# facebookresearch/Active-3D-Vision-and-Touch

Hardware: AMD Instinct MI355X
Metric: mesh-recon iters/sec (fwd+bwd, 2562-vert GCN + 10k-pt Chamfer) at bs=64 (higher is better)
Workload: dtype f32; 1 GPU; icosphere-4 template (2562 verts, 5120 faces), 3-stage GCN 20x300 cut 0.33, bs=64/GPU, 10000-pt Chamfer x3 draws, Adam, ellipsoid clouds (BASELINE.json configs[1]); global_batch=64, parallelism=dp1

## Files before the change

active-3d-vision-and-touch_amd/csrc/capi.hip:

```cpp
#include <stdarg.h>
#include <stdlib.h>
#include <string.h>

#include "../../include/a3vt.h"
#include <atomic>
#include <initializer_list>
#include <mutex>
#include <unordered_map>

#include "kernels.h"
#include "prims.h"

namespace a3vt {

static thread_local char g_err[512] = "";

void set_error(const char *fmt, ...) {
  va_list ap;
  va_start(ap, fmt);
  vsnprintf(g_err, sizeof(g_err), fmt, ap);
  va_end(ap);
}

struct PtrArg {
  const char *name;
  const void *p;
  bool required;
  unsigned align;
  const char *why;
};
static int check_ptrs(const char *who, std::initializer_list<PtrArg> ptrs) {
  for (const PtrArg &a : ptrs) {
    if (a.required && !a.p) {
      set_error("%s: %s=NULL: %s", who, a.name, a.why);
      return -1;
    }
    if (!aligned_to(a.p, a.align)) {
      set_error("%s: %s=%p is not %u-byte aligned", who, a.name, a.p, a.align);
      return -1;
    }
  }
  return 0;
}
static int check_range(const char *who, const char *name, long long v, long long lo, long long hi) {
  if (v >= lo && v <= hi) return 0;
  set_error("%s: %s=%lld outside %lld..%lld", who, name, v, lo, hi);
  return -1;
}
static int check_count(const char *who, const char *name, int v, int max) {
  if (v >= 1 && v <= max) return 0;
  set_error("%s: %s=%d (1..%d) unsupported", who, name, v, max);
  return -1;
}
static int check_grads(const char *who, const PolicyGrads &g, int n_layers) {
  for (int l = 0; l < n_layers; ++l) {
    if (!g.dw[l] || !g.db[l] || !aligned_to(g.dw[l], 4) || !aligned_to(g.db[l], 4)) {
      set_error("%s: layer %d dweight / dbias null or misaligned", who, l);
      return -1;
    }
  }
  return 0;
}
template <int N>
struct LaunchCounts {
  std::atomic<long long> n[N];
  void add(int i, long long k) { n[i].fetch_add(k, std::memory_order_relaxed); }
  int read(long long *counts, int reset) {
    for (int i = 0; i < N; ++i) {
      if (counts) counts[i] = n[i].load(std::memory_order_relaxed);
      if (reset) n[i].store(0, std::memory_order_relaxed);
    }
    return N;
  }
};

__device__ float g_zero_page[64];
static const float *zero_page() {
  static const float *ptr[64] = {};
  static std::mutex mu;
  int dev = 0;
  (void)hipGetDevice(&dev);
  std::lock_guard<std::mutex> lock(mu);
  const float *&slot = ptr[dev & 63];
  if (!slot) {
    void *p = nullptr;
    if (hipGetSymbolAddress(&p, HIP_SYMBOL(g_zero_page)) != hipSuccess) return nullptr;
    slot = static_cast<const float *>(p);
  }
  return slot;
}

static inline size_t align_up(size_t x, size_t a) { return (x + a - 1) / a * a; }

struct Arena {
  size_t off = 0;
  size_t take(size_t nfloats) {
    const size_t o = off;
    off = align_up(off + nfloats, 64);
    return o;
  }
  size_t take16(size_t nelems) { return take((nelems + 1) / 2 + 64); }
};

enum { PROF_GEMM_FWD = 0, PROF_GEMM_DX = 1, PROF_DW = 2, PROF_AGG = 3, PROF_OUT = 4, PROF_SEARCH = 5, PROF_LOSS = 6, PROF_ENC = 7,
       PROF_OPT = 8, PROF_CLASSES = 9 };
struct Prof {
  bool on = false;
  static constexpr int kMax = 8192;
  hipEvent_t ev[kMax][2];
  int cls[kMax];
  int created = 0, used = 0;
};
static Prof g_prof;

struct ProfScope {
  int slot = -1;
  hipStream_t s;
  ProfScope(int cls, hipStream_t stream, bool timed = true) : s(stream) {
    if (!timed || !g_prof.on || g_prof.used >= Prof::kMax) return;
    slot = g_prof.used++;
    if (slot >= g_prof.created) {
      (void)hipEventCreate(&g_prof.ev[slot][0]);
      (void)hipEventCreate(&g_prof.ev[slot][1]);
      g_prof.created = slot + 1;
    }
    g_prof.cls[slot] = cls;
    (void)hipEventRecord(g_prof.ev[slot][0], s);
  }
  ~ProfScope() {
    if (slot >= 0) (void)hipEventRecord(g_prof.ev[slot][1], s);
  }
};

struct StackLayout {
  size_t wt, wt_stride;
  size_t za;
  int ldza;
  size_t z3;
  size_t ping[2];
  size_t panel;
  size_t dw_slab, db_slab, thin_dw_slab, thin_db_slab;
  size_t db_layer_stride;
  size_t heavy;
  size_t gq;
  size_t ell;
  size_t total;
};

constexpr int kQuadCols = 160;
static std::atomic<long long> g_path_counts[PATH_COUNT];
void path_count(int which) { g_path_counts[which].fetch_add(1, std::memory_order_relaxed); }
static int g_csr_algo = 0;
static SplitRef split_ref(const a3vt_adj_split *sp) {
  return sp ? SplitRef{sp->rowptr, sp->col, sp->scale, sp->cls} : SplitRef{nullptr, nullptr, nullptr, nullptr};
}
static bool split_whole(const a3vt_adj_split *sp) {
  const SplitRef r = split_ref(sp);
  return !sp || (r.rowptr && r.col && r.scale && r.cls);
}
static bool split_usable(const a3vt_adj_split *sp, int n_vert, int cut_len) {
  return sp && sp->max_degree > 0 && sp->max_degree <= csrqs_max_degree() && csrqs_fits(n_vert, cut_len);
}
static bool use_csrq(int batch, int n_vert, int hidden, int cut_len, int mode, int max_degree) {
  if (mode == GEMM_BF16_OPERANDS || mode == GEMM_BF16_STORAGE) return false;
  if (g_csr_algo != 2 && (max_degree <= 0 || max_degree > csrq_max_degree())) return false;
  if (g_csr_algo == 1 || cut_len <= 0) return false;
  return hidden % 4 == 0 && hidden >= kQuadCols + 16 && csrq_fits(n_vert, cut_len) && dw_quad_major_ok(hidden, kQuadCols / 4) &&
         rowgemm_quad_major_ok(batch * n_vert, hidden, pad4(cut_len));
}
static std::mutex g_stash_mu;
static std::unordered_map<const void *, int> g_stash_layout;
static void stash_layout_record(const void *masks, bool quad) {
  if (!masks) return;
  std::lock_guard<std::mutex> lock(g_stash_mu);
  if (g_stash_layout.size() > 4096) g_stash_layout.clear();
  g_stash_layout[masks] = quad ? 1 : 0;
}
static int stash_layout_lookup(const void *masks) {
  std::lock_guard<std::mutex> lock(g_stash_mu);
  auto it = g_stash_layout.find(masks);
  return it == g_stash_layout.end() ? -1 : it->second;
}
static int reduce_bias_partials(const float *slab, size_t layer_stride, int nslab, int cpad, int cut_len, int hidden, int last,
                                float *const *grad_biases, int acc, hipStream_t s) {
  for (int i0 = 0; i0 < last; i0 += kMaxImages) {
    SlabReduceBatch b{};
    b.count = last - i0 < kMaxImages ? last - i0 : kMaxImages;
    b.slab = slab + (size_t)i0 * layer_stride;
    for (int j = 0; j < b.count; ++j) b.out[j] = grad_biases[i0 + j];
    b.layer_stride = layer_stride;
    b.stride = cpad;
    b.n = cut_len;
    b.n_out = hidden;
    b.nslab = nslab;
    b.accumulate = acc;
    if (int rc = launch_slab_reduce_batch(b, s)) return rc;
  }
  return 0;
}

static inline int mask_ld(int hidden, int cut_len) { return pad4(cut_len) / 4 + (hidden + 3) / 4; }

static int hub_rows(const int32_t *rowptr, int n_vert, int max_degree, float *slot, int32_t **heavy, hipStream_t s) {
  *heavy = nullptr;
  if (max_degree > 0 && max_degree <= csr_heavy_degree()) return 0;
  *heavy = reinterpret_cast<int32_t *>(slot);
  return launch_csr_heavy_list(rowptr, n_vert, *heavy, s);
}

static int launch_stack_images(int kind, int transpose, const float *const *weights, int i0, int i1, int in_features,
                               int hidden, int w0, int wh, float *dst, size_t stride, hipStream_t s) {
  auto ld = [&](int w) { return kind == GEMM_BF16_STORAGE ? 2 * pad16(w / 2) : pad16(w); };
  for (; i0 < i1; i0 += kMaxImages) {
    WeightImages wi{};
    wi.count = i1 - i0 < kMaxImages ? i1 - i0 : kMaxImages;
    wi.dst = dst + stride * i0;
    wi.dst_stride = stride;
    wi.n = hidden;
    wi.transpose = transpose;
    int max_rows = 0, max_ld = kind == GEMM_FP32 && transpose ? ld(wh) : 0;
    for (int j = 0; j < wi.count; ++j) {
      const int w = i0 + j == 0 ? w0 : wh;
      wi.w[j] = weights[i0 + j];
      wi.k[j] = i0 + j == 0 ? in_features : hidden;
      wi.rows[j] = rowgemm_bt_rows(transpose ? hidden : w);
      wi.ld[j] = ld(transpose ? w : wh);
      max_rows = wi.rows[j] > max_rows ? wi.rows[j] : max_rows;
      max_ld = wi.ld[j] > max_ld ? wi.ld[j] : max_ld;
    }
    const int rc = kind == GEMM_FP32X3 ? launch_weight_images3(wi, s)
                   : kind == GEMM_BF16_STORAGE ? launch_weight_images16(wi, max_rows, max_ld, s)
                                               : launch_weight_images(wi, max_rows, max_ld, s);
    if (rc) return rc;
  }
  return 0;
}

static int reduce_output_grads(const float *dw_slab, const float *db_slab, int k, float *grad_w, float *grad_b, int acc,
                               hipStream_t s) {
  const size_t n = (size_t)k * 3;
  if (int rc = launch_slab_reduce_za(dw_slab, thin_num_slabs(), n, n, n, grad_w, acc, s)) return rc;
  return launch_slab_reduce_za(db_slab, thin_num_slabs(), 3, 3, 3, grad_b, acc, s);
}

struct StackPlan {
  bool x3;
  int omode;
  bool quad;
  bool qsplit;
  int qcols;
  int rm_ld;
  size_t rm_off;
};
static StackPlan stack_plan(int mode, int batch, int n_vert, int hidden, int num_layers, int cut_len, int max_degree,
                            const a3vt_adj_split *split, int rec) {
  StackPlan p{};
  const size_t m = (size_t)batch * n_vert;
  p.x3 = mode == GEMM_FP32X3 && num_layers > 2 && rowgemm3_stack_ok((long long)m, hidden, mask_ld(hidden, cut_len));
  p.omode = mode == GEMM_BF16_OPERANDS ? GEMM_BF16_OPERANDS : GEMM_FP32;
  const bool split_ok = split_usable(split, n_vert, cut_len);
  p.quad = num_layers > 1 &&
           (rec >= 0 ? rec == 1 : use_csrq(batch, n_vert, hidden, cut_len, mode, split_ok ? csrq_max_degree() : max_degree));
  p.qsplit = p.quad && split_ok;
  p.qcols = p.quad ? kQuadCols : 0;
  p.rm_ld = hidden - p.qcols;
  p.rm_off = m * p.qcols;
  return p;
}

static int launch_stack_ell(const StackPlan &p, const a3vt_adj_split *split, const int32_t *rowptr, const int32_t *col,
                            const float *val, int n_vert, int32_t *ell, hipStream_t s) {
  if (p.qsplit) {
    const SplitRef r = split_ref(split);
    return launch_csrqs_image(r.rowptr, r.col, r.scale, r.cls, n_vert, ell, s);
  }
  return p.quad ? launch_csrq_ell(rowptr, col, val, n_vert, ell, s) : 0;
}

static StackLayout stack_layout(int batch, int n_vert, int in_features, int hidden, int num_layers, int cut_len,
                                int need_backward, int gemm_mode = 0) {
  StackLayout L{};
  const size_t m = (size_t)batch * n_vert;
  const int cpad = pad4(cut_len);
  Arena a;
  const int kmax = hidden > pad4(in_features) ? hidden : pad4(in_features);
  L.wt_stride = align_up((size_t)rowgemm_bt_rows(kmax) * pad16(kmax), 64);
  if (gemm_mode == GEMM_FP32X3 && L.wt_stride < 3 * (size_t)kX3ImageFloats) L.wt_stride = 3 * (size_t)kX3ImageFloats;
  L.wt = a.take(L.wt_stride * (num_layers > 1 ? num_layers - 1 : 1));
  L.ldza = cpad > 4 ? cpad : 4;
  L.za = a.take(m * L.ldza);
  L.z3 = a.take(2 * m * 4);
  L.ping[0] = a.take(m * hidden);
  L.ping[1] = a.take(m * hidden);
  L.heavy = a.take(csr_heavy_scratch_ints(n_vert));
  L.ell = a.take(csrq_ell_ints(n_vert));
  if (need_backward) {
    const size_t kin = kmax;
    L.panel = a.take(pad4(in_features) > 304 ? m * 300 : 0);
    L.dw_slab = a.take((size_t)dw_slab_capacity(hidden) * kin * hidden);
    const size_t nslab = (size_t)csr_bwd_num_slabs(batch, n_vert) > (size_t)batch ? csr_bwd_num_slabs(batch, n_vert) : batch;
    L.db_layer_stride = align_up(nslab * cpad, 64);
    L.db_slab = a.take(L.db_layer_stride * (num_layers > 1 ? num_layers - 1 : 1));
    L.gq = a.take(m * L.ldza);
    L.thin_dw_slab = a.take((size_t)thin_num_slabs() * kin * 3);
    L.thin_db_slab = a.take((size_t)thin_num_slabs() * 3);
  }
  L.total = a.off;
  return L;
}

static int dw_panels(DwArgs d, const float *x, int ldx, int kin, float *panel, float *grad, int acc, bool timed, hipStream_t s) {
  const int cblk = kin > 304 ? 300 : kin;
  for (int c0 = 0; c0 < kin; c0 += cblk) {
    const int w = kin - c0 < cblk ? kin - c0 : cblk;
    d.x = x;
    d.ldx = ldx;
    if (kin > 304) {
      if (pad4(w) != w) { set_error("gcn_stack: in_features=%d needs a multiple of 4 past 300", kin); return -1; }
      if (int rc = launch_copy_cols(x, ldx, c0, w, panel, (long long)d.m, s)) return rc;
      d.x = panel;
      d.ldx = w;
    }
    d.k_in = w;
    {
      ProfScope ps(PROF_DW, s, timed);
      if (int rc = launch_dw(d, s)) return rc;
    }
    const size_t n = (size_t)w * d.n_out;
    if (int rc = launch_slab_reduce_za(d.slab, dw_images(d), n, n, n, grad + (size_t)c0 * d.n_out, acc, s)) return rc;
  }
  return 0;
}

static int check_stack_dims(int ld_feats, int in_features, int num_layers, int hidden, int cut_len) {
  if (num_layers < 1) { set_error("gcn_stack: num_layers=%d", num_layers); return -1; }
  if (ld_feats != pad4(in_features)) {
    set_error("gcn_stack: ld_feats=%d must be in_features=%d rounded up to a multiple of 4", ld_feats, in_features);
    return -1;
  }
  if (num_layers > 1 && (hidden % 4 != 0 || hidden > 304 || cut_len < 0 || cut_len > hidden)) {
    set_error("gcn_stack: hidden=%d (must be a multiple of 4, <= 304) cut_len=%d unsupported", hidden, cut_len);
    return -1;
  }
  if (ld_feats > 600) { set_error("gcn_stack: in_features=%d > 600 unsupported", in_features); return -1; }
  if (num_layers == 1 && ld_feats > 320) { set_error("gcn_stack: single-layer stack with %d inputs unsupported", in_features); return -1; }
  return 0;
}


static inline int mask_ld16(int hidden, int cut_len) { return (pad8(cut_len) / 4 + (hidden + 3) / 4 + 1) & ~1; }

constexpr int kStashInputLd = 608;

struct StackStash {
  size_t act_stride;
  size_t input16;
  int mld;
  size_t sign_stride;
  size_t signq0, signq_stride;
  size_t acts_bytes, mask_bytes;
  size_t act(int i) const { return (size_t)i * act_stride; }
  size_t signs(int i) const { return (size_t)i * sign_stride; }
  size_t signq(int i) const { return signq0 + (size_t)i * signq_stride; }
};
static StackStash stack_stash(int batch, int n_vert, int hidden, int num_layers, int cut_len, int gemm_mode) {
  StackStash S{};
  const bool s16 = gemm_mode == GEMM_BF16_STORAGE;
  const size_t m = (size_t)batch * n_vert, mpad = (m + 31) / 32 * 32, nh = num_layers > 1 ? num_layers - 1 : 0;
  S.act_stride = m * (s16 ? pad8(hidden) : hidden);
  S.input16 = nh * S.act_stride;
  S.mld = s16 ? mask_ld16(hidden, cut_len) : mask_ld(hidden, cut_len);
  S.sign_stride = mpad * S.mld;
  S.signq0 = nh * S.sign_stride;
  S.signq_stride = s16 ? 0 : align_up(m * (size_t)(pad4(cut_len) / 4), 256);
  S.acts_bytes = s16 ? (S.input16 + m * (size_t)kStashInputLd) * 2 + 256 : nh * S.act_stride * sizeof(float);
  S.mask_bytes = nh * (S.sign_stride + S.signq_stride);
  return S;
}
struct Stack16Layout {
  size_t wt, wt_stride;
  size_t feats16;
  size_t za;
  size_t z3;
  size_t ping[2];
  size_t dw_slab, db_slab, thin_dw_slab, thin_db_slab, heavy, total;
  size_t db_layer_stride;
  size_t tplan;
  int ld0, ldh, cpad;
  int ldza;
};

static Stack16Layout stack16_layout(int batch, int n_vert, int in_features, int hidden, int num_layers, int cut_len,
                                    int need_backward) {
  Stack16Layout L{};
  const size_t m = (size_t)batch * n_vert;
  L.ld0 = pad8(in_features);
  L.ldh = pad8(hidden);
  L.cpad = pad8(cut_len);
  L.ldza = L.cpad > 8 ? L.cpad : 8;
  Arena a;
  const int kmax = L.ld0 > L.ldh ? L.ld0 : L.ldh;
  const int rows_f = rowgemm_bt_rows(hidden), rows_b = rowgemm_bt_rows(kmax);
  const size_t img_f = (size_t)rows_f * pad16(kmax / 2), img_b = (size_t)rows_b * pad16(L.ldh / 2);
  L.wt_stride = align_up(img_f > img_b ? img_f : img_b, 64);
  L.wt = a.take(L.wt_stride * (num_layers > 1 ? num_layers - 1 : 1));
  L.feats16 = a.take16(m * L.ld0);
  L.za = a.take16(m * L.ldza);
  L.z3 = a.take(2 * m * 4);
  L.ping[0] = a.take16(m * L.ldh);
  L.ping[1] = a.take16(m * L.ldh);
  L.heavy = a.take(csr_heavy_scratch_ints(n_vert));
  L.tplan = a.take(csr16t_plan_ints(n_vert));
  if (need_backward) {
    const size_t kin = in_features > hidden ? in_features : hidden;
    L.dw_slab = a.take((size_t)dw16_num_slabs(hidden) * (kin > 304 ? 304 : kin) * hidden);
    L.db_layer_stride = align_up((size_t)csr_bwd_num_slabs(batch, n_vert) * L.ldza, 64);
    L.db_slab = a.take(L.db_layer_stride * (num_layers > 1 ? num_layers - 1 : 1));
    L.thin_dw_slab = a.take((size_t)thin_num_slabs() * hidden * 3);
    L.thin_db_slab = a.take((size_t)thin_num_slabs() * 3);
  }
  L.total = a.off;
  return L;
}

static int check_stack16_dims(int num_layers, int hidden, int in_features) {
  if (num_layers < 2) { set_error("gcn_stack: the bf16 storage mode needs at least one hidden layer"); return -1; }
  if (num_layers - 1 > kMaxImages) { set_error("gcn_stack: bf16 storage mode supports up to %d hidden layers", kMaxImages); return -1; }
  if (hidden > 304 || hidden % 4 != 0 || hidden < 16) { set_error("gcn_stack: bf16 storage mode: hidden=%d unsupported", hidden); return -1; }
  if (in_features > 600) { set_error("gcn_stack: in_features=%d > 600 unsupported", in_features); return -1; }
  if (in_features > 304 && in_features % 8 != 0) {
    set_error("gcn_stack: bf16 storage mode: in_features=%d > 304 must be a multiple of 8", in_features);
    return -1;
  }
  return 0;
}

static int stack_fwd16(const float *feats, int ld_feats, int in_features, const float *const *weights,
                       const float *const *biases, int num_layers, int hidden, int cut_len, const int32_t *rowptr,
                       const int32_t *col, const float *val, int max_degree, const a3vt_adj_split *split, int n_vert,
                       int batch, void *acts, uint8_t *masks, float *scratch, float *update, hipStream_t s) {
  if (int rc = check_stack16_dims(num_layers, hidden, in_features)) return rc;
  const float *zeros = zero_page();
  A3VT_CHECK_ARG(zeros != nullptr);
  const Stack16Layout L = stack16_layout(batch, n_vert, in_features, hidden, num_layers, cut_len, 0);
  const StackStash S = stack_stash(batch, n_vert, hidden, num_layers, cut_len, GEMM_BF16_STORAGE);
  const size_t m = (size_t)batch * n_vert;
  int32_t *heavy;
  if (int rc = hub_rows(rowptr, n_vert, max_degree, scratch + L.heavy, &heavy, s)) return rc;
  if (int rc = launch_stack_images(GEMM_BF16_STORAGE, 1, weights, 0, num_layers - 1, in_features, hidden, L.ld0, L.ldh,
                                   scratch + L.wt, L.wt_stride, s))
    return rc;
  u16 *f16 = acts ? static_cast<u16 *>(acts) + S.input16 : reinterpret_cast<u16 *>(scratch + L.feats16);
  if (int rc = launch_cvt_rows(feats, ld_feats, in_features, f16, L.ld0, (long long)m, s)) return rc;
  const bool tiled = heavy == nullptr && cut_len > 0 && g_csr_algo != 1 && csr16t_ok(n_vert, cut_len, max_degree, (long long)m);
  int32_t *tplan = reinterpret_cast<int32_t *>(scratch + L.tplan);
  if (tiled)
    if (int rc = launch_csr16t_build(rowptr, col, val, n_vert, tplan, s)) return rc;

  const u16 *x = f16;
  int ldx = L.ld0;
  u16 *za = reinterpret_cast<u16 *>(scratch + L.za);
  for (int i = 0; i + 1 < num_layers; ++i) {
    u16 *y = acts ? static_cast<u16 *>(acts) + S.act(i) : reinterpret_cast<u16 *>(scratch + L.ping[i & 1]);
    RowGemmArgs g{};
    g.a0 = g.a1 = reinterpret_cast<const float *>(x);
    g.lda0 = g.lda1 = ldx / 2;
    g.ksplit = g.k = ldx / 2;
    g.bt = scratch + L.wt + L.wt_stride * i;
    g.ldb = pad16(ldx / 2);
    g.zeros = zeros;
    g.m = (int)m;
    g.n_store = hidden;
    g.c = reinterpret_cast<float *>(y);
    g.ldc = L.ldh;
    g.c2 = reinterpret_cast<float *>(za);
    g.ldc2 = L.ldza;
    g.csplit = cut_len;
    uint8_t *mk = masks ? masks + S.signs(i) : nullptr;
    g.maskb = mk;
    g.mld = S.mld;
    g.moff = L.cpad / 4;
    g.mode = GEMM_BF16_STORAGE;
// ... 170 lines not shown
  return 0;
}

int a3vt_adj_split_validate(const int32_t *rowptr, const int32_t *col, const float *val, int n_vert,
                            const int32_t *p_rowptr, const int32_t *p_col, const float *scale, const uint8_t *cls) {
  A3VT_CHECK_ARG(rowptr && col && val && p_rowptr && p_col && scale && cls && n_vert > 0);
  if (p_rowptr[0] != 0 || p_rowptr[n_vert] > rowptr[n_vert]) {
    set_error("adj_split: p_rowptr[0]=%d p_rowptr[n]=%d (the matrix has %d entries)", p_rowptr[0], p_rowptr[n_vert], rowptr[n_vert]);
    return -1;
  }
  for (int i = 0; i < n_vert; ++i)
    if (p_rowptr[i + 1] < p_rowptr[i]) { set_error("adj_split: p_rowptr not monotone at %d", i); return -1; }
  int ns = 0, nc = 0;
  for (int i = 0; i < n_vert; ++i) {
    if (cls[i] > 2) { set_error("adj_split: cls[%d]=%d", i, (int)cls[i]); return -1; }
    ns += cls[i] == 1;
    nc += cls[i] == 2;
  }
  if ((ns == 0) != (nc == 0)) { set_error("adj_split: %d seam vertices but %d centres", ns, nc); return -1; }
  int32_t *members = static_cast<int32_t *>(malloc(sizeof(int32_t) * (size_t)(ns + nc + 1)));
  A3VT_CHECK_ARG(members != nullptr);
  int32_t *seam = members, *centre = members + ns;
  for (int i = 0, a = 0, b = 0; i < n_vert; ++i) {
    if (cls[i] == 1) seam[a++] = i;
    if (cls[i] == 2) centre[b++] = i;
  }
  int rc = 0;
  for (int i = 0; i < n_vert && rc == 0; ++i) {
    const int e0 = rowptr[i], e1 = rowptr[i + 1], p0 = p_rowptr[i], p1 = p_rowptr[i + 1];
    const int32_t *other = cls[i] == 1 ? centre : cls[i] == 2 ? seam : nullptr;
    const int no = cls[i] == 1 ? nc : cls[i] == 2 ? ns : 0;
    if (p1 < p0 || e1 - e0 != (p1 - p0) + no) {
      set_error("adj_split: row %d has %d entries, the split gives %d + %d", i, e1 - e0, p1 - p0, no);
      rc = -1;
      break;
    }
    int a = p0, b = 0;
    for (int e = e0; e < e1; ++e) {
      const bool has_a = a < p1, has_b = b < no;
      int next;
      if (has_a && has_b && p_col[a] == other[b]) {
        set_error("adj_split: row %d: column %d is in P and in the bipartite block", i, p_col[a]);
        rc = -1;
        break;
      }
      if (has_a && (!has_b || p_col[a] < other[b])) {
        next = p_col[a++];
        if (next < 0 || next >= n_vert || (a - 1 > p0 && p_col[a - 2] >= next)) {
          set_error("adj_split: row %d of P is not ascending / in range at column %d", i, next);
          rc = -1;
          break;
        }
        int lo = p_rowptr[next], hi = p_rowptr[next + 1] - 1;
        bool found = false;
        while (lo <= hi) {
          const int mid = (lo + hi) / 2;
          if (p_col[mid] == i) { found = true; break; }
          if (p_col[mid] < i) lo = mid + 1;
          else hi = mid - 1;
        }
        if (!found) { set_error("adj_split: P has (%d, %d) but not (%d, %d)", i, next, next, i); rc = -1; break; }
      } else {
        next = other[b++];
      }
      if (col[e] != next) {
        set_error("adj_split: row %d entry %d: column %d, the split gives %d", i, e - e0, col[e], next);
        rc = -1;
        break;
      }
      if (memcmp(&val[e], &scale[i], sizeof(float)) != 0) {
        set_error("adj_split: row %d entry %d: value %.9g != scale %.9g", i, e - e0, (double)val[e], (double)scale[i]);
        rc = -1;
        break;
      }
    }
  }
  free(members);
  return rc;
}

size_t a3vt_gcn_stack_mask_bytes(int batch, int n_vert, int hidden, int num_layers, int cut_len) {
  if (num_layers < 2 || batch <= 0 || n_vert <= 0 || hidden <= 0 || cut_len < 0) return 0;
  return stack_stash(batch, n_vert, hidden, num_layers, cut_len, GEMM_FP32).mask_bytes;
}

size_t a3vt_gcn_stack_scratch_bytes(int batch, int n_vert, int in_features, int hidden, int num_layers, int cut_len,
                                    int need_backward) {
  size_t most = 0;
  for (int mode = 0; mode <= 3; ++mode) {
    if (mode == GEMM_BF16_STORAGE && num_layers < 2) continue;
    const size_t b = a3vt_gcn_stack_scratch_bytes_mode(batch, n_vert, in_features, hidden, num_layers, cut_len, need_backward, mode);
    most = b > most ? b : most;
  }
  return most;
}

size_t a3vt_gcn_stack_scratch_bytes_mode(int batch, int n_vert, int in_features, int hidden, int num_layers,
                                         int cut_len, int need_backward, int gemm_bf16) {
  if (batch <= 0 || n_vert <= 0 || in_features <= 0 || hidden <= 0 || num_layers <= 0 || cut_len < 0 || gemm_bf16 < 0 || gemm_bf16 > 3)
    return 0;
  if (gemm_bf16 == GEMM_BF16_STORAGE)
    return stack16_layout(batch, n_vert, in_features, hidden, num_layers, cut_len, need_backward).total * sizeof(float);
  return stack_layout(batch, n_vert, in_features, hidden, num_layers, cut_len, need_backward, gemm_bf16).total * sizeof(float);
}

int a3vt_gcn_stack_stash_bytes(int batch, int n_vert, int hidden, int num_layers, int cut_len, int gemm_bf16,
                               size_t *acts_bytes, size_t *mask_bytes) {
  A3VT_CHECK_ARG(acts_bytes && mask_bytes && batch > 0 && n_vert > 0 && hidden > 0 && cut_len >= 0);
  *acts_bytes = *mask_bytes = 0;
  if (num_layers < 2) return 0;
  const StackStash S = stack_stash(batch, n_vert, hidden, num_layers, cut_len, gemm_bf16);
  *acts_bytes = S.acts_bytes;
  *mask_bytes = S.mask_bytes;
  return 0;
}

int a3vt_gcn_stack_fwd(const float *feats, int ld_feats, int in_features, const float *const *weights,
                       const float *const *biases, int num_layers, int hidden, int cut_len,
                       const int32_t *rowptr, const int32_t *col, const float *val, int max_degree, int n_vert,
                       int batch, int gemm_bf16, void *acts_v, uint8_t *masks, float *scratch, float *update,
                       void *stream) {
  return a3vt_gcn_stack_fwd_adj(feats, ld_feats, in_features, weights, biases, num_layers, hidden, cut_len, rowptr, col, val,
                                max_degree, nullptr, n_vert, batch, gemm_bf16, acts_v, masks, scratch, update, stream);
}

int a3vt_gcn_stack_fwd_adj(const float *feats, int ld_feats, int in_features, const float *const *weights,
                           const float *const *biases, int num_layers, int hidden, int cut_len,
                           const int32_t *rowptr, const int32_t *col, const float *val, int max_degree,
                           const a3vt_adj_split *split, int n_vert,
                           int batch, int gemm_bf16, void *acts_v, uint8_t *masks, float *scratch, float *update,
                           void *stream) {
  float *acts = static_cast<float *>(acts_v);
  A3VT_CHECK_ARG(feats && weights && biases && rowptr && col && val && scratch && update);
  A3VT_CHECK_ARG((acts == nullptr) == (masks == nullptr) || num_layers < 2);
  A3VT_CHECK_ARG(n_vert > 0 && batch > 0 && split_whole(split));
  A3VT_CHECK_ARG(gemm_bf16 >= GEMM_FP32 && gemm_bf16 <= GEMM_FP32X3);
  if (int rc = check_stack_dims(ld_feats, in_features, num_layers, hidden, cut_len)) return rc;
  hipStream_t s = static_cast<hipStream_t>(stream);
  if (gemm_bf16 == GEMM_BF16_STORAGE)
    return stack_fwd16(feats, ld_feats, in_features, weights, biases, num_layers, hidden, cut_len, rowptr, col, val,
                       max_degree, split, n_vert, batch, acts, masks, scratch, update, s);
  const float *zeros = zero_page();
  A3VT_CHECK_ARG(zeros != nullptr);
  const StackLayout L = stack_layout(batch, n_vert, in_features, hidden, num_layers, cut_len, 0, gemm_bf16);
  const StackStash S = stack_stash(batch, n_vert, hidden, num_layers, cut_len, gemm_bf16);
  const size_t m = (size_t)batch * n_vert;
  const int cpad = pad4(cut_len);

  int32_t *heavy;
  if (int rc = hub_rows(rowptr, n_vert, max_degree, scratch + L.heavy, &heavy, s)) return rc;
  const StackPlan P = stack_plan(gemm_bf16, batch, n_vert, hidden, num_layers, cut_len, max_degree, split, -1);
  const int qcols = P.qcols, rm_ld = P.rm_ld;
  const size_t rm_off = P.rm_off;
  if (P.x3)
    if (int rc = launch_stack_images(GEMM_FP32X3, 1, weights, 1, num_layers - 1, in_features, hidden, ld_feats, hidden,
                                     scratch + L.wt, L.wt_stride, s))
      return rc;
  if (int rc = launch_stack_images(GEMM_FP32, 1, weights, 0, P.x3 ? 1 : num_layers - 1, in_features, hidden, ld_feats, hidden,
                                   scratch + L.wt, L.wt_stride, s))
    return rc;
  if (num_layers > 1) path_count(P.quad ? PATH_STACK_QUAD : PATH_STACK_ROWS);
  if (P.qsplit) path_count(PATH_STACK_SPLIT);
  if (num_layers > 1) stash_layout_record(masks, P.quad);
  int32_t *ell = reinterpret_cast<int32_t *>(scratch + L.ell);
  if (int rc = launch_stack_ell(P, split, rowptr, col, val, n_vert, ell, s)) return rc;
  const float *x = feats, *xq = nullptr;
  int ldx = ld_feats;
  for (int i = 0; i + 1 < num_layers; ++i) {
    const int k = i == 0 ? ld_feats : hidden;
    const bool l3 = P.x3 && i > 0;
    float *y = acts ? acts + S.act(i) : scratch + L.ping[i & 1];
    RowGemmArgs g{};
    g.a0 = g.a1 = x;
    g.lda0 = g.lda1 = ldx;
    g.ksplit = k;
    if (xq) {
      g.a0 = xq;
      g.ksplit = qcols;
      g.a0q_nvert = n_vert;
      g.a0q_quads = qcols / 4;
    }
    g.bt = scratch + L.wt + L.wt_stride * i;
    g.ldb = pad16(k);
    g.zeros = zeros;
    g.m = (int)m;
    g.k = k;
    g.n_store = hidden;
    g.c = y + rm_off - qcols;
    g.ldc = rm_ld;
    g.c2 = scratch + L.za;
    g.ldc2 = cpad;
    g.csplit = cut_len;
    uint8_t *mk = masks ? masks + S.signs(i) : nullptr;
    g.maskb = mk;
    g.mld = S.mld;
    g.moff = cpad / 4;
    g.mode = l3 ? GEMM_FP32X3 : P.omode;
    if (P.quad) {
      g.zq_nvert = n_vert;
      g.zq_quads = cpad / 4;
      g.yq = y;
      g.yq_quads = qcols / 4;
      g.trash = scratch + L.z3;
    }
    {
      ProfScope ps(PROF_GEMM_FWD, s);
      if (int rc = launch_rowgemm(g, EPI_FWD_HIDDEN, s)) return rc;
    }
    if (P.quad) {
      uint8_t *sq = masks ? masks + S.signq(i) : nullptr;
      ProfScope psa(PROF_AGG, s);
      if (P.qsplit) {
        if (int rc = launch_csrqs_fwd(scratch + L.za, biases[i], cut_len, ell, n_vert, batch, y, qcols / 4, sq, 1, s)) return rc;
      } else if (int rc = launch_csrq_fwd(scratch + L.za, biases[i], cut_len, rowptr, col, val, heavy, ell, n_vert, batch, y, qcols / 4, sq, 1, s)) {
        return rc;
      }
      xq = y;
    } else if (cut_len > 0) {
      ProfScope psa(PROF_AGG, s);
      if (int rc = launch_csr_fwd(scratch + L.za, L.ldza, biases[i], cut_len, rowptr, col, val, heavy, n_vert, batch, y, hidden, mk, S.mld, 1, s))
        return rc;
    }
    x = y + rm_off - qcols;
    ldx = rm_ld;
  }
  const int klast = num_layers == 1 ? in_features : hidden;
  ProfScope pso(PROF_OUT, s);
  const SplitRef sref = split_ref(split);
  return launch_thin_fwd(x, ldx, klast, weights[num_layers - 1], biases[num_layers - 1], rowptr, col, val, heavy, n_vert,
                         batch, scratch + L.z3, update, xq, qcols / 4, s, split ? &sref : nullptr);
}

int a3vt_gcn_stack_bwd(const float *feats, int ld_feats, int in_features, const float *const *weights,
                       const float *const *biases, int num_layers, int hidden, int cut_len,
                       const int32_t *rowptr, const int32_t *col, const float *val, const int32_t *rowptrT,
                       const int32_t *colT, const float *valT, int max_degreeT, int n_vert, int batch, int gemm_bf16,
                       const void *acts_v,
                       const uint8_t *masks, const float *grad_update, float *const *grad_weights, float *const *grad_biases,
                       float *grad_feats, float *scratch, void *stream) {
  return a3vt_gcn_stack_bwd_adj(feats, ld_feats, in_features, weights, biases, num_layers, hidden, cut_len, rowptr, col, val,
                                rowptrT, colT, valT, max_degreeT, nullptr, n_vert, batch, gemm_bf16, acts_v, masks, grad_update,
                                grad_weights, grad_biases, grad_feats, scratch, 0, stream);
}

int a3vt_gcn_stack_bwd_acc(const float *feats, int ld_feats, int in_features, const float *const *weights,
                           const float *const *biases, int num_layers, int hidden, int cut_len,
                           const int32_t *rowptr, const int32_t *col, const float *val, const int32_t *rowptrT,
                           const int32_t *colT, const float *valT, int max_degreeT, int n_vert, int batch, int gemm_bf16,
                           const void *acts_v,
                           const uint8_t *masks, const float *grad_update, float *const *grad_weights,
                           float *const *grad_biases, float *grad_feats, float *scratch, int accumulate, void *stream) {
  return a3vt_gcn_stack_bwd_adj(feats, ld_feats, in_features, weights, biases, num_layers, hidden, cut_len, rowptr, col, val,
                                rowptrT, colT, valT, max_degreeT, nullptr, n_vert, batch, gemm_bf16, acts_v, masks, grad_update,
                                grad_weights, grad_biases, grad_feats, scratch, accumulate, stream);
}

int a3vt_gcn_stack_bwd_adj(const float *feats, int ld_feats, int in_features, const float *const *weights,
                           const float *const *biases, int num_layers, int hidden, int cut_len,
                           const int32_t *rowptr, const int32_t *col, const float *val, const int32_t *rowptrT,
                           const int32_t *colT, const float *valT, int max_degreeT, const a3vt_adj_split *split,
                           int n_vert, int batch, int gemm_bf16, const void *acts_v,
                           const uint8_t *masks, const float *grad_update, float *const *grad_weights,
                           float *const *grad_biases, float *grad_feats, float *scratch, int accumulate, void *stream) {
  const int acc = accumulate ? 1 : 0;
  const float *acts = static_cast<const float *>(acts_v);
  (void)biases; (void)rowptr; (void)col; (void)val;
  A3VT_CHECK_ARG(feats && weights && rowptrT && colT && valT && grad_update && grad_weights && grad_biases);
  A3VT_CHECK_ARG(grad_feats && scratch && n_vert > 0 && batch > 0 && split_whole(split));
  A3VT_CHECK_ARG(gemm_bf16 >= GEMM_FP32 && gemm_bf16 <= GEMM_FP32X3);
  A3VT_CHECK_ARG(num_layers == 1 || acts != nullptr);
  A3VT_CHECK_ARG(num_layers <= 2 || masks != nullptr);
  if (int rc = check_stack_dims(ld_feats, in_features, num_layers, hidden, cut_len)) return rc;
  hipStream_t s = static_cast<hipStream_t>(stream);
  if (gemm_bf16 == GEMM_BF16_STORAGE)
    return stack_bwd16(feats, ld_feats, in_features, weights, num_layers, hidden, cut_len, rowptrT, colT, valT,
                       max_degreeT, split, n_vert, batch, acts, masks, grad_update, grad_weights, grad_biases, grad_feats,
                       scratch, acc, s);
  const float *zeros = zero_page();
  A3VT_CHECK_ARG(zeros != nullptr);
  const StackLayout L = stack_layout(batch, n_vert, in_features, hidden, num_layers, cut_len, 1, gemm_bf16);
  const StackStash S = stack_stash(batch, n_vert, hidden, num_layers, cut_len, gemm_bf16);
  const size_t m = (size_t)batch * n_vert;
  const int cpad = pad4(cut_len);
  const int last = num_layers - 1;

  const SplitRef sref = split_ref(split);
  int32_t *heavyT;
  if (int rc = hub_rows(rowptrT, n_vert, max_degreeT, scratch + L.heavy, &heavyT, s)) return rc;
  const StackPlan P = stack_plan(gemm_bf16, batch, n_vert, hidden, num_layers, cut_len, max_degreeT, split,
                                 masks ? stash_layout_lookup(masks) : 0);
  const bool quad = P.quad;
  const int qcols = P.qcols, rm_ld = P.rm_ld;
  const size_t rm_off = P.rm_off;
  int32_t *ellT = reinterpret_cast<int32_t *>(scratch + L.ell);
  if (int rc = launch_stack_ell(P, split, rowptrT, colT, valT, n_vert, ellT, s)) return rc;
  {
    const float *xl = num_layers == 1 ? feats : acts + S.act(last - 1);
    const float *x = xl + rm_off - qcols;
    const int ldx = num_layers == 1 ? ld_feats : rm_ld;
    const int k = num_layers == 1 ? in_features : hidden;
    float *gprev = num_layers == 1 ? grad_feats : scratch + L.ping[0];
    const int ldg = num_layers == 1 ? ld_feats : hidden;
    ProfScope pso(PROF_OUT, s);
    if (int rc = launch_thin_bwd(x, ldx, k, weights[last], rowptrT, colT, valT, heavyT, n_vert, batch, grad_update,
                                 scratch + L.z3, num_layers > 1, gprev, ldg, ldg, scratch + L.thin_dw_slab,
                                 scratch + L.thin_db_slab, quad ? scratch + L.gq : nullptr, cpad / 4, quad ? xl : nullptr,
                                 qcols / 4, s, split ? &sref : nullptr))
      return rc;
    if (int rc = reduce_output_grads(scratch + L.thin_dw_slab, scratch + L.thin_db_slab, k, grad_weights[last], grad_biases[last],
                                     acc, s))
      return rc;
  }

  if (P.x3)
    if (int rc = launch_stack_images(GEMM_FP32X3, 0, weights, 1, last, in_features, hidden, ld_feats, hidden, scratch + L.wt,
                                     L.wt_stride, s))
      return rc;
  if (int rc = launch_stack_images(GEMM_FP32, 0, weights, 0, P.x3 ? 1 : last, in_features, hidden, ld_feats, hidden,
                                   scratch + L.wt, L.wt_stride, s))
    return rc;

  const int db_rows = quad ? batch : csr_bwd_num_slabs(batch, n_vert);
  int cur = 0;
  for (int i = last - 1; i >= 0; --i) {
    float *g = scratch + L.ping[cur];
    float *dza = scratch + L.za;
    const float *xl = i == 0 ? feats : acts + S.act(i - 1);
    const bool xhyb = quad && i > 0;
    const float *x = xhyb ? xl + rm_off - qcols : xl;
    const int ldx = i == 0 ? ld_feats : (xhyb ? rm_ld : hidden);
    const int kin = i == 0 ? in_features : hidden;

    if (cut_len > 0 && quad) {
      const uint8_t *sq = masks + S.signq(i);
      ProfScope psa(PROF_AGG, s);
      if (P.qsplit) {
        if (int rc = launch_csrqs_bwd(scratch + L.gq, cut_len, ellT, n_vert, batch, dza, sq,
                                      scratch + L.db_slab + (size_t)i * L.db_layer_stride, s))
          return rc;
      } else if (int rc = launch_csrq_bwd(scratch + L.gq, cut_len, rowptrT, colT, valT, heavyT, ellT, n_vert, batch, dza, sq,
                                          scratch + L.db_slab + (size_t)i * L.db_layer_stride, s)) {
        return rc;
      }
    } else if (cut_len > 0) {
      ProfScope psa(PROF_AGG, s);
      if (int rc = launch_csr_bwd(g, hidden, cut_len, rowptrT, colT, valT, heavyT, n_vert, batch, dza, L.ldza,
                                  scratch + L.db_slab + (size_t)i * L.db_layer_stride, s))
        return rc;
    } else if (!acc) {
      if (int rc = launch_fill_zero(grad_biases[i], hidden, s)) return rc;
    }

    DwArgs d{};
    if (xhyb) {
      d.ldx_src = rm_ld;
      d.xq = xl;
      d.xq_nvert = n_vert;
      d.xq_quads = qcols / 4;
    }
    if (quad) {
      d.z0q_nvert = n_vert;
      d.z0q_quads = cpad / 4;
    }
    d.z0 = dza;
    d.ldz0 = L.ldza;
    d.z1 = g;
    d.ldz1 = hidden;
    d.zsplit = cpad;
    d.zeros = zeros;
    d.slab = scratch + L.dw_slab;
    d.m = (int)m;
    d.n_out = hidden;
    d.mode = P.omode;
    const int ldxw = xhyb ? hidden : ldx;
    if (P.x3 && i > 0) {
      d.mode = GEMM_FP32X3;
      d.x = x;
      d.ldx = ldxw;
      d.k_in = kin;
      if (!dw3_ok(d)) d.mode = P.omode;
    }
    if (int rc = dw_panels(d, x, ldxw, kin, scratch + L.panel, grad_weights[i], acc, true, s)) return rc;

    RowGemmArgs r{};
    r.a0 = dza;
    r.lda0 = L.ldza;
    if (quad) {
      r.a0q_nvert = n_vert;
      r.a0q_quads = cpad / 4;
    }
    r.a1 = g;
    r.lda1 = hidden;
    r.ksplit = cpad;
    r.bt = scratch + L.wt + L.wt_stride * i;
    r.ldb = pad16(hidden);
    r.zeros = zeros;
    r.m = (int)m;
    r.k = hidden;
    r.n_store = i == 0 ? ld_feats : hidden;
    r.mode = P.x3 && i > 0 ? GEMM_FP32X3 : P.omode;
    if (i == 0) {
      r.c = grad_feats;
      r.ldc = ld_feats;
      if (int rc = launch_rowgemm(r, EPI_PLAIN, s)) return rc;
    } else {
      r.c = scratch + L.ping[cur ^ 1];
      r.ldc = hidden;
      r.maskb = const_cast<uint8_t *>(masks) + S.signs(i - 1);
      r.mld = S.mld;
      r.moff = cpad / 4;
      r.csplit = cut_len;
      if (quad) {
        r.c2 = scratch + L.gq;
        r.zq_nvert = n_vert;
        r.zq_quads = cpad / 4;
        r.trash = scratch + L.z3;
      }
      {
        ProfScope ps(PROF_GEMM_DX, s);
        if (int rc = launch_rowgemm(r, EPI_DX_MASK, s)) return rc;
      }
      cur ^= 1;
    }
  }
  if (cut_len > 0)
    if (int rc = reduce_bias_partials(scratch + L.db_slab, L.db_layer_stride, db_rows, cpad, cut_len, hidden, last, grad_biases, acc, s))
      return rc;
  return 0;
}

namespace {
struct LayerLayout {
  size_t wt, za, ga, dz, panel, dw_slab, db_slab, heavy, total;
  int ldza;
};
LayerLayout layer_layout(int batch, int n_vert, int ld_x, int n_out, int cut_len, int need_backward) {
  LayerLayout L{};
  const size_t m = (size_t)batch * n_vert;
  const int cpad = pad4(cut_len), npad = pad4(n_out);
  L.ldza = cpad > 4 ? cpad : 4;
  Arena a;
  const size_t wt_fwd = (size_t)rowgemm_bt_rows(n_out) * pad16(ld_x);
  const size_t wt_bwd = (size_t)rowgemm_bt_rows(ld_x) * pad16(npad);
  L.wt = a.take(wt_fwd > wt_bwd ? wt_fwd : wt_bwd);
  L.za = a.take(m * L.ldza);
  L.heavy = a.take(csr_heavy_scratch_ints(n_vert));
  if (need_backward) {
    L.ga = a.take(m * L.ldza);
    L.dz = a.take(m * npad);
    L.panel = a.take(ld_x > 304 ? m * 300 : 0);
    const int kin = ld_x > 304 ? 300 : ld_x;
    L.dw_slab = a.take((size_t)dw_num_slabs(n_out) * kin * n_out);
    L.db_slab = a.take((size_t)csr_bwd_num_slabs(batch, n_vert) * L.ldza);
  }
  L.total = a.off;
  return L;
}
int check_layer_dims(int ld_x, int in_features, int n_out, int cut_len) {
  if (ld_x % 4 != 0 || ld_x < in_features || ld_x > 600 || in_features < 1) {
    set_error("gcn_layer: ld_x=%d must be a multiple of 4, >= in_features=%d and <= 600", ld_x, in_features);
    return -1;
  }
  if (n_out < 1 || n_out > 304 || cut_len < 0 || cut_len > n_out) {
    set_error("gcn_layer: out_features=%d (1..304) cut_len=%d unsupported", n_out, cut_len);
    return -1;
  }
  if (in_features > 304 && in_features % 4 != 0) {
    set_error("gcn_layer: in_features=%d > 304 must be a multiple of 4", in_features);
    return -1;
  }
  return 0;
}
int layer_fwd_tail(const float *za, int ldza, const float *bias, int cut_len, int relu, const int32_t *rowptr, const int32_t *col,
                   const float *val, int max_degree, int n_vert, int batch, float *y, int ld_y, float *heavy_slot, hipStream_t s) {
  if (cut_len <= 0) return 0;
  int32_t *heavy;
  if (int rc = hub_rows(rowptr, n_vert, max_degree, heavy_slot, &heavy, s)) return rc;
  return launch_csr_fwd(za, ldza, bias, cut_len, rowptr, col, val, heavy, n_vert, batch, y, ld_y, nullptr, 0, relu, s);
}
int layer_bwd_tail(const float *grad_y, int ld_gy, const float *y, int ld_y, int relu, int n_out, int cut_len,
                   const int32_t *rowptrT, const int32_t *colT, const float *valT, int max_degreeT, int n_vert, int batch, float *ga,
                   float *dz, float *db_slab, float *heavy_slot, float *grad_bias, hipStream_t s) {
  const int cpad = pad4(cut_len), npad = pad4(n_out);
  if (int rc = launch_relu_split(grad_y, ld_gy, y, ld_y, relu, n_out, cpad, npad, (long long)batch * n_vert, ga, dz, s)) return rc;
  if (int rc = launch_fill_zero(grad_bias, n_out, s)) return rc;
  if (cut_len <= 0) return 0;
  int32_t *heavyT;
  if (int rc = hub_rows(rowptrT, n_vert, max_degreeT, heavy_slot, &heavyT, s)) return rc;
  if (int rc = launch_csr_bwd(ga, cpad, cut_len, rowptrT, colT, valT, heavyT, n_vert, batch, dz, npad, db_slab, s)) return rc;
  return launch_slab_reduce(db_slab, csr_bwd_num_slabs(batch, n_vert), cpad, cut_len, grad_bias, s);
}
}

size_t a3vt_gcn_layer_scratch_bytes(int batch, int n_vert, int ld_x, int out_features, int cut_len, int need_backward) {
  return layer_layout(batch, n_vert, ld_x, out_features, cut_len, need_backward).total * sizeof(float);
}

int a3vt_gcn_layer_fwd(const float *x, int ld_x, int in_features, const float *weight, const float *bias,
                       int out_features, int cut_len, int relu, const int32_t *rowptr, const int32_t *col,
                       const float *val, int max_degree, int n_vert, int batch, int gemm_bf16, float *y, int ld_y,
                       float *scratch, void *stream) {
  A3VT_CHECK_ARG(x && weight && bias && rowptr && col && val && y && scratch && n_vert > 0 && batch > 0);
  if (int rc = check_layer_dims(ld_x, in_features, out_features, cut_len)) return rc;
  A3VT_CHECK_ARG(ld_y % 4 == 0 && ld_y >= out_features);
  hipStream_t s = static_cast<hipStream_t>(stream);
  const float *zeros = zero_page();
  A3VT_CHECK_ARG(zeros != nullptr);
  const LayerLayout L = layer_layout(batch, n_vert, ld_x, out_features, cut_len, 0);
  const size_t m = (size_t)batch * n_vert;
  float *wt = scratch + L.wt;
  if (int rc = launch_transpose_pad(weight, in_features, out_features, wt, rowgemm_bt_rows(out_features), pad16(ld_x), s))
    return rc;
  RowGemmArgs g{};
  g.a0 = g.a1 = x;
  g.lda0 = g.lda1 = ld_x;
  g.ksplit = ld_x;
  g.bt = wt;
  g.ldb = pad16(ld_x);
  g.zeros = zeros;
  g.m = (int)m;
  g.k = ld_x;
  g.n_store = out_features;
  g.c = y;
  g.ldc = ld_y;
  g.c2 = scratch + L.za;
  g.ldc2 = L.ldza;
  g.csplit = cut_len;
  g.no_relu = relu ? 0 : 1;
  g.mode = gemm_bf16 == GEMM_BF16_OPERANDS ? GEMM_BF16_OPERANDS : GEMM_FP32;
  if (int rc = launch_rowgemm(g, EPI_FWD_HIDDEN, s)) return rc;
  return layer_fwd_tail(scratch + L.za, L.ldza, bias, cut_len, relu ? 1 : 0, rowptr, col, val, max_degree, n_vert, batch, y, ld_y,
                        scratch + L.heavy, s);
}

int a3vt_gcn_layer_bwd(const float *x, int ld_x, int in_features, const float *weight, int out_features, int cut_len,
                       int relu, const int32_t *rowptrT, const int32_t *colT, const float *valT, int max_degreeT,
                       int n_vert, int batch, int gemm_bf16, const float *y, int ld_y, const float *grad_y, int ld_gy,
                       float *grad_weight, float *grad_bias, float *grad_x, float *scratch, void *stream) {
  A3VT_CHECK_ARG(x && weight && rowptrT && colT && valT && grad_y && grad_weight && grad_bias && grad_x && scratch);
  A3VT_CHECK_ARG(n_vert > 0 && batch > 0 && ld_gy >= out_features && (!relu || (y && ld_y >= out_features)));
  if (int rc = check_layer_dims(ld_x, in_features, out_features, cut_len)) return rc;
  hipStream_t s = static_cast<hipStream_t>(stream);
  const float *zeros = zero_page();
  A3VT_CHECK_ARG(zeros != nullptr);
  const LayerLayout L = layer_layout(batch, n_vert, ld_x, out_features, cut_len, 1);
  const size_t m = (size_t)batch * n_vert;
  const int npad = pad4(out_features);
  float *dz = scratch + L.dz;
  if (int rc = layer_bwd_tail(grad_y, ld_gy, y, ld_y, relu ? 1 : 0, out_features, cut_len, rowptrT, colT, valT, max_degreeT, n_vert,
                              batch, scratch + L.ga, dz, scratch + L.db_slab, scratch + L.heavy, grad_bias, s))
    return rc;
  DwArgs d{};
  d.z0 = scratch + L.za;
  d.ldz0 = 4;
  d.z1 = dz;
  d.ldz1 = npad;
  d.zsplit = 0;
  d.zeros = zeros;
  d.slab = scratch + L.dw_slab;
  d.m = (int)m;
  d.n_out = out_features;
  d.mode = gemm_bf16 == GEMM_BF16_OPERANDS ? GEMM_BF16_OPERANDS : GEMM_FP32;
  if (int rc = dw_panels(d, x, ld_x, in_features, scratch + L.panel, grad_weight, 0, false, s)) return rc;
  float *wp = scratch + L.wt;
  if (int rc = launch_copy_pad(weight, in_features, out_features, wp, rowgemm_bt_rows(ld_x), pad16(npad), s)) return rc;
  RowGemmArgs r{};
  r.a0 = scratch + L.za;
  r.lda0 = 4;
  r.ksplit = 0;
  r.a1 = dz;
  r.lda1 = npad;
  r.bt = wp;
  r.ldb = pad16(npad);
  r.zeros = zeros;
  r.m = (int)m;
// ... 760 lines not shown
  for (int k = 0; k < n; ++k) {
    A3VT_CHECK_ARG(src[k] && dst[k] && outer[k] > 0 && inner[k] > 0 && hw[k] > 0);
    A3VT_CHECK_ARG(outer[k] <= (1ll << 31) / inner[k] / hw[k]);
    b.src[k] = src[k];
    b.dst[k] = static_cast<uint16_t *>(dst[k]);
    b.inner[k] = inner[k];
    b.hw[k] = hw[k];
    b.start[k + 1] = b.start[k] + outer[k] * inner[k] * hw[k];
  }
  ProfScope psc(PROF_ENC, static_cast<hipStream_t>(stream));
  return launch_cast_weights(b, static_cast<hipStream_t>(stream));
}

int a3vt_conv5_supported(int cin, int cout, int stride) { return conv5_shape_ok(cin, cout, stride) ? 1 : 0; }

size_t a3vt_conv5_image_bytes(int cout, int cin, int flip) {
  if (cin == 3 && flip) return cout == 16 ? conv5_weight_image_bytes(16, 16) : 0;
  if (cin == 3) return cout == 3 || cout == 16 ? conv5_weight_image_bytes(cout, 3) : 0;
  if ((cin != 16 && cin != 32) || (cout != 16 && cout != 32)) return 0;
  return flip ? conv5_weight_image_bytes(cin, cout) : conv5_weight_image_bytes(cout, cin);
}

int a3vt_conv5_weight_image(const float *weight, int cout, int cin, int flip, void *image, void *stream) {
  A3VT_CHECK_ARG(weight && image && (flip == 0 || flip == 1));
  A3VT_CHECK_ARG(((cin == 16 || cin == 32) && (cout == 16 || cout == 32)) || (cin == 3 && flip == 0 && (cout == 3 || cout == 16)) ||
                 (cin == 3 && flip == 1 && cout == 16));
  A3VT_CHECK_ARG(aligned_to(image, 16));
  return launch_conv5_weight_image(weight, flip, cout, cin, image, static_cast<hipStream_t>(stream));
}

int a3vt_conv5_nhwc(const void *x, int batch, int height, int width, int cin, int cout, int stride, int pad, const void *image,
                    const float *bias, void *y, void *stream) {
  A3VT_CHECK_ARG(x && image && y);
  A3VT_CHECK_ARG(conv5_shape_ok(cin, cout, stride));
  A3VT_CHECK_ARG(batch > 0 && height > 0 && width > 0 && pad >= 0 && pad <= 4);
  A3VT_CHECK_ARG(height + 2 * pad >= 5 && width + 2 * pad >= 5);
  A3VT_CHECK_ARG((long long)batch * height * width <= (1ll << 31) / 32);
  A3VT_CHECK_ARG(aligned_to(x, cin == 3 ? 2 : 16) && aligned_to(y, cin == 3 ? 2 : 16));
  A3VT_CHECK_ARG(aligned_to(image, 16) && (cout == 3 || aligned_to(y, 16)));
  A3VT_CHECK_ARG(aligned_to(bias, cout == 3 ? 4 : 16));
  ProfScope psc(PROF_ENC, static_cast<hipStream_t>(stream));
  return launch_conv5(x, batch, height, width, cin, cout, stride, pad, image, bias, y, static_cast<hipStream_t>(stream));
}

int a3vt_conv5_input_grad_3x16s2(const void *grad_out, int batch, int out_height, int out_width, const void *image, void *grad_in,
                                 void *stream) {
  A3VT_CHECK_ARG(grad_out && image && grad_in && batch > 0 && out_height > 0 && out_width > 0);
  A3VT_CHECK_ARG((long long)batch * (2 * out_height + 2) * (2 * out_width + 2) <= (1ll << 31) / 16);
  A3VT_CHECK_ARG(aligned_to(grad_out, 16) && aligned_to(image, 16));
  A3VT_CHECK_ARG(aligned_to(grad_in, 2));
  ProfScope psc(PROF_ENC, static_cast<hipStream_t>(stream));
  return launch_conv5_up3(grad_out, batch, out_height, out_width, image, grad_in, static_cast<hipStream_t>(stream));
}

size_t a3vt_conv5_wrw_scratch_bytes(int cin, int cout) {
  return ((cin == 16 || cin == 32) && (cout == 16 || cout == 32)) || (cin == 3 && (cout == 3 || cout == 16)) ? conv5_wrw_scratch_bytes(cin, cout) : 0;
}

int a3vt_conv5_weight_grad(const void *x, const void *grad_out, int batch, int height, int width, int cin, int cout, int stride,
                           float *grad_weight, void *scratch, size_t scratch_bytes, void *stream) {
  A3VT_CHECK_ARG(x && grad_out && grad_weight && scratch);
  A3VT_CHECK_ARG(conv5_shape_ok(cin, cout, stride));
  A3VT_CHECK_ARG(batch > 0 && height >= 3 && width >= 3 && (long long)batch * height * width <= (1ll << 31) / 32);
  A3VT_CHECK_ARG(aligned_to(scratch, 16));
  A3VT_CHECK_ARG(aligned_to(x, cin == 3 ? 2 : 16) && aligned_to(grad_out, cout == 3 ? 2 : 16));
  A3VT_CHECK_ARG(scratch_bytes >= conv5_wrw_scratch_bytes(cin, cout));
  ProfScope psc(PROF_ENC, static_cast<hipStream_t>(stream));
  return launch_conv5_wrw(x, grad_out, batch, height, width, cin, cout, stride, grad_weight, scratch, static_cast<hipStream_t>(stream));
}

int a3vt_conv5f_supported(int cin, int cout, int stride) { return conv5f_shape_ok(cin, cout, stride) ? 1 : 0; }

size_t a3vt_conv5f_image_bytes(int cin, int cout) { return conv5f_weight_image_bytes(cin, cout); }

int a3vt_conv5f_weight_image(const float *weight, int cout, int cin, void *image, void *stream) {
  A3VT_CHECK_ARG(weight && image);
  A3VT_CHECK_ARG(conv5f_weight_image_bytes(cin, cout) != 0);
  A3VT_CHECK_ARG(aligned_to(weight, 4) && aligned_to(image, 16));
  return launch_conv5f_weight_image(weight, cout, cin, image, static_cast<hipStream_t>(stream));
}

int a3vt_conv5f_nhwc(const float *x, int batch, int height, int width, int cin, int cout, int stride, int pad, const void *image,
                     const float *scale, const float *shift, int relu, float *y, void *stream) {
  A3VT_CHECK_ARG(x && image && y);
  A3VT_CHECK_ARG(conv5f_shape_ok(cin, cout, stride));
  A3VT_CHECK_ARG(batch >= 1 && height >= 1 && width >= 1 && pad >= 0 && pad <= 4 && (relu == 0 || relu == 1));
  A3VT_CHECK_ARG(height + 2 * pad >= 5 && width + 2 * pad >= 5);
  A3VT_CHECK_ARG((long long)batch * height * width <= (1ll << 31) / 32);
  A3VT_CHECK_ARG(aligned_to(x, cin == 3 ? 4 : 16));
  A3VT_CHECK_ARG(aligned_to(y, 16) && aligned_to(image, 16));
  A3VT_CHECK_ARG(aligned_to(scale, 4) && aligned_to(shift, 4));
  ProfScope psc(PROF_ENC, static_cast<hipStream_t>(stream));
  return launch_conv5f(x, batch, height, width, cin, cout, stride, pad, image, scale, shift, relu, y, static_cast<hipStream_t>(stream));
}

int a3vt_adam_chunk_elems(void) { return adam_chunk_elems(); }

int a3vt_adam_step(void *const *param, const void *const *grad, void *const *exp_avg, void *const *exp_avg_sq,
                   const long long *numel, const int *chunk_tensor, const long long *chunk_off, int n_chunks, double lr, double beta1,
                   double beta2, double eps, double weight_decay, long long step, void *stream) {
  A3VT_CHECK_ARG(n_chunks >= 0 && step >= 1);
  A3VT_CHECK_ARG(n_chunks == 0 || (param && grad && exp_avg && exp_avg_sq && numel && chunk_tensor && chunk_off));
  A3VT_CHECK_ARG(lr >= 0.0 && beta1 >= 0.0 && beta1 < 1.0 && beta2 >= 0.0 && beta2 < 1.0 && eps >= 0.0 && weight_decay >= 0.0);
  ProfScope psc(PROF_OPT, static_cast<hipStream_t>(stream));
  return launch_adam(param, grad, exp_avg, exp_avg_sq, numel, chunk_tensor, chunk_off, n_chunks, lr, beta1, beta2, eps, weight_decay, step,
                     static_cast<hipStream_t>(stream));
}

int a3vt_adam_step_clamp(void *const *param, void *const *grad, void *const *exp_avg, void *const *exp_avg_sq, const long long *numel,
                         const int *chunk_tensor, const long long *chunk_off, int n_chunks, double lr, double beta1, double beta2,
                         double eps, double weight_decay, long long step, double grad_clamp, void *stream) {
  A3VT_CHECK_ARG(n_chunks >= 0 && step >= 1 && grad_clamp > 0.0);
  A3VT_CHECK_ARG(n_chunks == 0 || (param && grad && exp_avg && exp_avg_sq && numel && chunk_tensor && chunk_off));
  A3VT_CHECK_ARG(lr >= 0.0 && beta1 >= 0.0 && beta1 < 1.0 && beta2 >= 0.0 && beta2 < 1.0 && eps >= 0.0 && weight_decay >= 0.0);
  ProfScope psc(PROF_OPT, static_cast<hipStream_t>(stream));
  return launch_adam(param, const_cast<const void *const *>(grad), exp_avg, exp_avg_sq, numel, chunk_tensor, chunk_off, n_chunks, lr, beta1,
                     beta2, eps, weight_decay, step, static_cast<hipStream_t>(stream), grad_clamp);
}

int a3vt_profile_enable(int on) {
  g_prof.on = on != 0;
  g_prof.used = 0;
  return 0;
}

int a3vt_profile_read_classes(double *total_ms, int *count, int n) {
  A3VT_CHECK_ARG(total_ms && count && n >= 0);
  for (int c = 0; c < n; ++c) { total_ms[c] = 0.0; count[c] = 0; }
  for (int i = 0; i < g_prof.used; ++i) {
    if (hipEventSynchronize(g_prof.ev[i][1]) != hipSuccess) { set_error("profile_read: event sync failed"); return -2; }
    float ms = 0.f;
    if (hipEventElapsedTime(&ms, g_prof.ev[i][0], g_prof.ev[i][1]) != hipSuccess) continue;
    if (g_prof.cls[i] >= n) continue;
    total_ms[g_prof.cls[i]] += ms;
    count[g_prof.cls[i]] += 1;
  }
  g_prof.used = 0;
  return PROF_CLASSES;
}

int a3vt_profile_read(double *total_ms, int *count) {
  const int rc = a3vt_profile_read_classes(total_ms, count, 3);
  return rc < 0 ? rc : 0;
}

int a3vt_dbg_path_counts(long long *counts, int n, int reset) {
  A3VT_CHECK_ARG(n >= 0 && (counts != nullptr || n == 0));
  for (int i = 0; i < n; ++i) counts[i] = i < PATH_COUNT ? g_path_counts[i].load(std::memory_order_relaxed) : 0;
  if (reset)
    for (auto &c : g_path_counts) c.store(0, std::memory_order_relaxed);
  return PATH_COUNT;
}

int a3vt_dbg_csr_algo(int algo) {
  A3VT_CHECK_ARG(algo >= 0 && algo <= 2);
  g_csr_algo = algo;
  return 0;
}

int a3vt_split3_bf16(const float *x, size_t n, uint16_t *hi, uint16_t *mid, uint16_t *lo, void *stream) {
  A3VT_CHECK_ARG(n == 0 || (x && hi && mid && lo));
  return launch_split3(x, n, hi, mid, lo, static_cast<hipStream_t>(stream));
}

int a3vt_check_finite(const float *data, size_t n, int32_t *flag, void *stream) {
  A3VT_CHECK_ARG(data && flag);
  return launch_check_finite(data, n, flag, static_cast<hipStream_t>(stream));
}

}
```

active-3d-vision-and-touch_amd/csrc/gcn_dww.hip:

```cpp
#include <type_traits>

#include "gemm_tile.h"

namespace a3vt {

constexpr int kDK = 300, kDN = 300, kDXQ = 40, kDZQ = 25, kDXRW = 140, kDLdz = 300;
constexpr int kDStageRows = 16;
constexpr int kDwwGroupsA = 135, kDwwGroupsB = 121;
constexpr int kDXQ_off = 0, kDXR_off = 2560, kDZ_off = 2560 + 2304;
constexpr int kDZRa_off = kDZ_off + 1792;
constexpr int kDStage = kDZ_off + 2816;
constexpr int kDStages = 4;
constexpr int kDLdsFloats = kDStages * kDStage;

__device__ __forceinline__ void d_mfma(f32x4 &acc, float a, float b) {
  asm volatile("v_mfma_f32_16x16x4_f32 %0, %1, %2, %0" : "+a"(acc) : "v"(a), "v"(b));
}
__device__ __forceinline__ void d_lds(float &dst, unsigned base, int imm) {
  asm volatile("ds_read_b32 %0, %1 offset:%2" : "=v"(dst) : "v"(base), "n"(imm));
}
template <int N, int NX, int NZ>
__device__ __forceinline__ void d_wait(float (&x)[NX], float (&z)[NZ]) {
  static_assert(NX <= 5 && NZ <= 10, "operand list");
  if constexpr (NX == 5 && NZ == 10)
// ... 19 lines not shown
  const int nvert = p.xq_nvert;
  const unsigned lds0 = (unsigned)(size_t)(__attribute__((address_space(3))) float *)lds;

  const unsigned xq_lane = kDXQ_off * 4 + (unsigned)((l16 >> 2) * 256 + q * 16 + (l16 & 3) * 4);
  const unsigned xr_lane = kDXR_off * 4 + (unsigned)((q * kDXRW + l16) * 4);
  const unsigned zq_lane = kDZ_off * 4 + (unsigned)((l16 >> 2) * 256 + q * 16 + (l16 & 3) * 4);
  const unsigned zra_lane = kDZRa_off * 4 + (unsigned)((q * 60 + l16) * 4);
  const unsigned zrb_lane = kDZ_off * 4 + (unsigned)((q * kDXRW + l16) * 4);
  const bool t6q = l16 < 4;
  const unsigned z6_lane = t6q ? kDZ_off * 4 + (unsigned)(24 * 256 + q * 16 + l16 * 4) : kDZRa_off * 4 + (unsigned)((q * 60 + l16 - 4) * 4);
  const unsigned z6_step = t6q ? 64u : 960u;

  unsigned xr_off[9], zr_off[9];
  int d_bq = 0, d_vq = 0;
  unsigned xq_off = 0, zq_off = 0;
  auto locate = [&](int tile) {
    const int row = tile * kDStageRows + l16;
    d_bq = row / nvert;
    d_vq = row - d_bq * nvert;
  };
  auto refresh = [&]() {
    xq_off = ((unsigned)(d_bq * kDXQ + q) * (unsigned)nvert + (unsigned)d_vq) * 16u;
    zq_off = ((unsigned)(d_bq * kDZQ + q) * (unsigned)nvert + (unsigned)d_vq) * 16u;
  };
  auto advance = [&]() {
    d_vq += kDStageRows;
    const bool wrap = d_vq >= nvert;
    d_vq = wrap ? d_vq - nvert : d_vq;
    d_bq = wrap ? d_bq + 1 : d_bq;
  };
  if (SERVICE) {
#pragma unroll
    for (int j = 0; j < 9; ++j) {
      const int i = 64 * j + lane;
      const int rx = i / 35, px = i - rx * 35;
      xr_off[j] = i < 16 * 35 ? (unsigned)((rx * p.ldx_src + px * 4) * 4) : 0u;
      if (HALF == 0) {
        const int rz = i / 15, pz = i - rz * 15;
        zr_off[j] = (j < 4 && i < 16 * 15) ? (unsigned)((rz * kDLdz + pz * 4) * 4) : 0u;
      } else {
        zr_off[j] = i < 16 * 35 ? (unsigned)((rx * kDLdz + px * 4) * 4) : 0u;
      }
    }
  }
  constexpr int NDMA = HALF == 0 ? 10 + 9 + 7 + 4 : 10 + 9 + 9;
  auto dma = [&](int idx, int tile, int st) {
    float *sbase = lds + st * kDStage;
    const size_t row0 = (size_t)tile * kDStageRows;
    if (idx < 10) {
      glds16(reinterpret_cast<const float *>(w_at(p.xq + (size_t)idx * 4 * nvert * 4, xq_off)), sbase + kDXQ_off + idx * 256);
    } else if (idx < 19) {
      const int j = idx - 10;
      glds16(reinterpret_cast<const float *>(w_at(p.x + row0 * p.ldx_src + 160, xr_off[j])), sbase + kDXR_off + j * 256);
    } else if (HALF == 0 && idx < 26) {
      const int j = idx - 19;
      const unsigned off = j < 6 ? zq_off : zq_off - (unsigned)q * (unsigned)nvert * 16u;
      glds16(reinterpret_cast<const float *>(w_at(p.z0 + (size_t)(j < 6 ? j * 4 : 24) * nvert * 4, off)), sbase + kDZ_off + j * 256);
    } else if (HALF == 0) {
      const int j = idx - 26;
      glds16(reinterpret_cast<const float *>(w_at(p.z1 + row0 * kDLdz + 100, zr_off[j])), sbase + kDZRa_off + j * 256);
    } else {
      const int j = idx - 19;
      glds16(reinterpret_cast<const float *>(w_at(p.z1 + row0 * kDLdz + 160, zr_off[j])), sbase + kDZ_off + j * 256);
    }
  };

  if (SERVICE) {
#pragma unroll
    for (int d = 0; d < 3; ++d) {
      const int tsrc = tile0 + d < tile1 ? tile0 + d : tile1 - 1;
      locate(tsrc);
      refresh();
#pragma unroll
      for (int idx = 0; idx < NDMA; ++idx) dma(idx, tsrc, d);
    }
    locate(tile0 + 2 < tile1 ? tile0 + 2 : tile1 - 1);
    refresh();
  }
  wait_vmcnt<0>();
  wait_lgkm0();
  __builtin_amdgcn_s_barrier();

  f32x4 acc[NKT][NNT];
#pragma unroll
  for (int t = 0; t < NKT; ++t)
#pragma unroll
    for (int n = 0; n < NNT; ++n) acc[t][n] = f32x4{0.f, 0.f, 0.f, 0.f};
  int st = 0;
  auto frag = [&](int stg, auto sc, auto kc, float (&xf)[NKT], float (&zf)[NNT]) {
    constexpr int s = decltype(sc)::value, k = decltype(kc)::value;
    const unsigned sb = lds0 + (unsigned)(stg * kDStage * 4);
    if constexpr (k < NKT) {
      const unsigned xb = sb + (XROW ? xr_lane : xq_lane);
      if (XROW) d_lds(xf[k], xb, (kt0x + k) * 64 + s * 4 * kDXRW * 4);
      else d_lds(xf[k], xb, (kt0x + k) * 1024 + s * 64);
    } else if constexpr (k < NKT + NNT) {
      constexpr int n = k - NKT, T = NT0 + n;
      if (HALF == 0 && T < 6) d_lds(zf[n], sb + zq_lane, T * 1024 + s * 64);
      else if (HALF == 0 && T == 6) d_lds(zf[n], sb + z6_lane + (unsigned)s * z6_step, 0);
      else if (HALF == 0) d_lds(zf[n], sb + zra_lane, (T * 16 - 100) * 4 + s * 4 * 60 * 4);
      else d_lds(zf[n], sb + zrb_lane, (T * 16 - 160) * 4 + s * 4 * kDXRW * 4);
    }
  };
  auto dma_part = [&](int part, int dtile, int dst) {
    constexpr int PER = (NDMA + 3) / 4;
#pragma unroll
    for (int u = 0; u < PER; ++u)
      if (part * PER + u < NDMA) dma(part * PER + u, dtile < tile1 ? dtile : tile1 - 1, dst);
  };
  float xc[NKT], zc[NNT];
  [&]<int... K>(std::integer_sequence<int, K...>) {
    (frag(0, std::integral_constant<int, 0>{}, std::integral_constant<int, K>{}, xc, zc), ...);
  }(std::make_integer_sequence<int, NKT + NNT>{});
  d_wait<0>(xc, zc);
  for (int tile = tile0; tile < tile1; ++tile) {
    auto step = [&](auto sc) {
      constexpr int s = decltype(sc)::value;
      float xn[NKT], zn[NNT];
      constexpr int EVERY = (NKT * NNT) / (NKT + NNT);
      [&]<int... I>(std::integer_sequence<int, I...>) {
        ((d_mfma(acc[I / NNT][I % NNT], zc[I % NNT], xc[I / NNT]),
          (I % EVERY == 0 ? frag(s < 3 ? st : ((st + 1) & 3), std::integral_constant<int, (s + 1) & 3>{}, std::integral_constant<int, I / EVERY>{}, xn, zn)
                          : (void)0)),
         ...);
      }(std::make_integer_sequence<int, NKT * NNT>{});
      d_wait<0>(xn, zn);
#pragma unroll
      for (int t = 0; t < NKT; ++t) xc[t] = xn[t];
#pragma unroll
      for (int n = 0; n < NNT; ++n) zc[n] = zn[n];
    };
    step(std::integral_constant<int, 0>{});
    if (SERVICE && tile > tile0) dma_part(1, tile + 2, (st + 2) & 3);
    step(std::integral_constant<int, 1>{});
    if (SERVICE && tile > tile0) dma_part(2, tile + 2, (st + 2) & 3);
    step(std::integral_constant<int, 2>{});
    if (SERVICE) {
      if (tile > tile0) dma_part(3, tile + 2, (st + 2) & 3);
      wait_vmcnt<NDMA>();
    }
    wait_lgkm0();
    __builtin_amdgcn_s_barrier();
    step(std::integral_constant<int, 3>{});
    if (SERVICE) {
      if (tile + 3 < tile1) {
        advance();
        refresh();
      }
      dma_part(0, tile + 3, (st + 3) & 3);
    }
    st = (st + 1) & 3;
  }
  asm volatile("s_nop 15\n\ts_nop 3" ::: "memory");
  float *img = p.slab + (size_t)image * kDK * kDN;
#pragma unroll
  for (int t = 0; t < NKT; ++t) {
    const int k = (kt0 + t) * 16 + l16;
#pragma unroll
    for (int n = 0; n < NNT; ++n) {
      const int col = (NT0 + n) * 16 + q * 4;
      if (k < kDK && col < kDN) *reinterpret_cast<f32x4 *>(img + (size_t)k * kDN + col) = acc[t][n];
    }
  }
}

__global__ __launch_bounds__(256) __attribute__((amdgpu_waves_per_eu(1, 1))) void dww_kernel(DwArgs p) {
  extern __shared__ __attribute__((aligned(16))) float lds[];
  const int lane = threadIdx.x & 63;
  const int wave = __builtin_amdgcn_readfirstlane(threadIdx.x >> 6);
  const int half = blockIdx.x < kDwwGroupsA ? 0 : 1;
  const int group = half == 0 ? blockIdx.x : blockIdx.x - kDwwGroupsA, ngroups = half == 0 ? kDwwGroupsA : kDwwGroupsB;
  const int tiles = p.m / kDStageRows;
  const int t0 = (int)((long long)group * tiles / ngroups), t1 = (int)((long long)(group + 1) * tiles / ngroups);
  if (half == 1 && group < kDwwGroupsA - kDwwGroupsB) {
    float *img = p.slab + (size_t)(kDwwGroupsB + group) * kDK * kDN;
    for (int i = threadIdx.x; i < kDK * 35; i += 256) {
      const int k = i / 35, c = i - k * 35;
      *reinterpret_cast<f32x4 *>(img + (size_t)k * kDN + 160 + c * 4) = f32x4{0.f, 0.f, 0.f, 0.f};
    }
  }
  if (half == 0) {
    if (wave == 0) dww_wave<0, false, 5, false, 0>(p, lds, lane, t0, t1, group);
    else if (wave == 1) dww_wave<0, false, 5, false, 5>(p, lds, lane, t0, t1, group);
    else if (wave == 2) dww_wave<0, true, 5, false, 10>(p, lds, lane, t0, t1, group);
    else dww_wave<0, true, 4, true, 15>(p, lds, lane, t0, t1, group);
  } else {
    if (wave == 0) dww_wave<1, false, 5, false, 0>(p, lds, lane, t0, t1, group);
    else if (wave == 1) dww_wave<1, false, 5, false, 5>(p, lds, lane, t0, t1, group);
    else if (wave == 2) dww_wave<1, true, 5, false, 10>(p, lds, lane, t0, t1, group);
    else dww_wave<1, true, 4, true, 15>(p, lds, lane, t0, t1, group);
  }
}

bool dww_ok(const DwArgs &a) {
  if (a.mode != GEMM_FP32 || a.xq_nvert <= 0 || a.z0q_nvert != a.xq_nvert || a.xq == nullptr) return false;
  if (a.k_in != kDK || a.n_out != kDN || a.xq_quads != kDXQ || a.z0q_quads != kDZQ || a.zsplit != 4 * kDZQ) return false;
  if (a.ldx_src != kDXRW || a.ldz1 != kDLdz || a.m % a.xq_nvert != 0 || a.m % kDStageRows != 0 || a.xq_nvert < 16) return false;
  if (a.m > 3000000) return false;
  return a.m / kDStageRows >= kDwwGroupsA * 5;
}

int dww_images() { return kDwwGroupsA; }

int launch_dww(const DwArgs &a, hipStream_t s) {
  if (!dww_ok(a)) {
    set_error("dww: shape not taken (m=%d k_in=%d n_out=%d)", a.m, a.k_in, a.n_out);
    return -1;
  }
  static OncePerDevice once;
  once.run([] {
    (void)hipFuncSetAttribute((const void *)dww_kernel, hipFuncAttributeMaxDynamicSharedMemorySize, (int)(kDLdsFloats * sizeof(float)));
  });
  path_count(PATH_DWW);
  A3VT_LAUNCH(dww_kernel, dim3(kDwwGroupsA + kDwwGroupsB), dim3(256), kDLdsFloats * sizeof(float), s, a);
  A3VT_CHECK_LAUNCH();
  return 0;
}

}
```

active-3d-vision-and-touch_amd/csrc/gcn_gemm.hip:

```cpp
#include <type_traits>

#include "common.h"
#include "kernels.h"
#include "gemm_tile.h"

namespace a3vt {

template <int V>
using RgIdx = std::integral_constant<int, V>;

template <int NT, int EPI, int NSTAGE, int WAVES, int MODE, bool ADIRECT = false>
__global__ __launch_bounds__(64 * WAVES, 2) void rowgemm_kernel(RowGemmArgs p) {
  constexpr bool BF16 = MODE == 1;
  constexpr bool ST16 = MODE == 2;
  constexpr int MT = 2;
  constexpr int BROWS = ((NT * 16 + 16 * WAVES - 1) / (16 * WAVES)) * (16 * WAVES);
  constexpr int A_INSTR = MT;
  constexpr int B_INSTR = BROWS / (16 * WAVES);
  constexpr int A_FLOATS = WAVES * MT * 16 * 16;
  constexpr int STAGE = A_FLOATS + BROWS * 16;
  constexpr int PER = A_INSTR + B_INSTR;
  constexpr int DIST = NSTAGE - 1;
  constexpr int MSLOT = 1024;
  static_assert((DIST - 1) * PER <= 63, "vmcnt immediate");
// ... 401 lines not shown
              const int ur = i * 16 + rl;
              const unsigned ba = mslot[ur * p.mld + (col >> 2)];
              const unsigned bb = mslot[ur * p.mld + p.moff + (col >> 2)];
              float *dst = p.c + (size_t)row * p.ldc + col;
#pragma unroll
              for (int t = 0; t < 4; ++t) {
                const unsigned bit = ((col + t < p.csplit ? ba : bb) >> t) & 1u;
                v[t] = bit ? v[t] : 0.f;
              }
              if (full) {
                *reinterpret_cast<f32x4 *>(dst) = v;
              } else {
                for (int t = 0; t < 4; ++t)
                  if (col + t < p.n_store) dst[t] = v[t];
              }
            }
          }
        }
      }
      if (mask_rows) {
        wait_lgkm0();
        __builtin_amdgcn_wave_barrier();
        const int nbytes = 16 * nm * p.mld;
        uint8_t *dstm = p.maskb + (size_t)row0 * p.mld;
        for (int o = le * 16; o < nbytes; o += 1024)
          *reinterpret_cast<f32x4 *>(dstm + o) = *reinterpret_cast<const f32x4 *>(mslot + o);
      }
    }
    wait_lgkm0();
    __builtin_amdgcn_s_barrier();
  }
  if (p.rem_rows > 0) {
    const int ntl = min(NT, (p.n_store - col0 + 15) >> 4);
    const int units = ((p.rem_rows + 15) >> 4) * ntl;
    for (int u = wave * gridDim.x + blockIdx.x; u < units; u += WAVES * gridDim.x)
      rowtile_unit<EPI, MODE>(p, p.rem_row0, p.rem_row0 + p.rem_rows, u / ntl, col0 + (u % ntl) * 16, lane);
  }
}

template <int NT>
struct RowGemmCfg {
  static constexpr int WAVES = 8;
  static constexpr int NSTAGE = NT == 1 ? 5 : 3;
  static constexpr int WG_PER_CU = 1;
  static constexpr int BROWS = ((NT * 16 + 16 * WAVES - 1) / (16 * WAVES)) * (16 * WAVES);
};

template <int NT, int EPI>
static int launch_rowgemm_nt(const RowGemmArgs &a, int grid_y, hipStream_t s) {
  using C = RowGemmCfg<NT>;
  constexpr size_t shmem = (C::NSTAGE * (size_t)(C::WAVES * 2 * 256 + C::BROWS * 16) +
                            (EPI != EPI_PLAIN ? C::WAVES * 1024 : 0)) * sizeof(float);
  static_assert(shmem * C::WG_PER_CU <= 160 * 1024, "LDS budget");
  static OncePerDevice once;
  once.run([] {
    (void)hipFuncSetAttribute((const void *)rowgemm_kernel<NT, EPI, C::NSTAGE, C::WAVES, 0>,
                              hipFuncAttributeMaxDynamicSharedMemorySize, (int)shmem);
    (void)hipFuncSetAttribute((const void *)rowgemm_kernel<NT, EPI, C::NSTAGE, C::WAVES, 1>,
                              hipFuncAttributeMaxDynamicSharedMemorySize, (int)shmem);
    (void)hipFuncSetAttribute((const void *)rowgemm_kernel<NT, EPI, C::NSTAGE, C::WAVES, 2>,
                              hipFuncAttributeMaxDynamicSharedMemorySize, (int)shmem);
    if (NT == 19)
      (void)hipFuncSetAttribute((const void *)rowgemm_kernel<NT, EPI, C::NSTAGE, C::WAVES, 0, NT == 19>,
                                hipFuncAttributeMaxDynamicSharedMemorySize, (int)shmem);
  });
  const int tiles = cdiv(a.m, 16);
  const int max_wg = 256 * C::WG_PER_CU;
  const int grid = cdiv(tiles, C::WAVES) < max_wg ? cdiv(tiles, C::WAVES) : max_wg;
  if (a.mode == GEMM_BF16_STORAGE)
    A3VT_LAUNCH((rowgemm_kernel<NT, EPI, C::NSTAGE, C::WAVES, 2>), dim3(grid, grid_y), dim3(64 * C::WAVES), shmem, s, a);
  else if (a.mode == GEMM_BF16_OPERANDS)
    A3VT_LAUNCH((rowgemm_kernel<NT, EPI, C::NSTAGE, C::WAVES, 1>), dim3(grid, grid_y), dim3(64 * C::WAVES), shmem, s, a);
  else {
    if (NT == 19) path_count(PATH_RG_ADIRECT);
    if (NT == 19)
      A3VT_LAUNCH((rowgemm_kernel<NT, EPI, C::NSTAGE, C::WAVES, 0, NT == 19>), dim3(grid, grid_y), dim3(64 * C::WAVES), shmem, s, a);
    else
      A3VT_LAUNCH((rowgemm_kernel<NT, EPI, C::NSTAGE, C::WAVES, 0>), dim3(grid, grid_y), dim3(64 * C::WAVES), shmem, s, a);
  }
  A3VT_CHECK_LAUNCH();
  return 0;
}

template <int EPI>
static int launch_rowgemm_cols(const RowGemmArgs &a, hipStream_t s) {
  const int nt = cdiv(a.n_store, 16);
  const int row_wgs = cdiv(cdiv(a.m, 16), 8);
  if (row_wgs < 96 && nt > 4) {
    if (row_wgs * cdiv(nt, 4) >= 96) return launch_rowgemm_nt<4, EPI>(a, cdiv(nt, 4), s);
    return launch_rowgemm_nt<1, EPI>(a, nt, s);
  }
  if (nt <= 1) return launch_rowgemm_nt<1, EPI>(a, 1, s);
  if (nt <= 4) return launch_rowgemm_nt<4, EPI>(a, 1, s);
  if (nt <= 8) return launch_rowgemm_nt<8, EPI>(a, 1, s);
  if (nt <= 13) return launch_rowgemm_nt<13, EPI>(a, 1, s);
  return launch_rowgemm_nt<19, EPI>(a, cdiv(nt, 19), s);
}

static int rowgemm_main_rows(int m, int nt) {
  const int tiles = cdiv(m, 16), full = tiles / 2048 * 2048, rem = tiles - full;
  return full == 0 || rem == 0 || rem * nt > 1024 || nt < 2 ? m : full * 16;
}
template <int EPI>
static int launch_rowgemm_epi(const RowGemmArgs &a0, hipStream_t s) {
  RowGemmArgs a = a0;
  a.bt_rows = rowgemm_bt_rows(a.n_store);
  a.col0 = 0;
  const int main_m = rowgemm_main_rows(a.m, cdiv(a.n_store, 16));
  if (main_m == a.m) return launch_rowgemm_cols<EPI>(a, s);
  RowGemmArgs m = a;
  m.m = main_m;
  m.rem_row0 = main_m;
  m.rem_rows = a.m - main_m;
  return launch_rowgemm_cols<EPI>(m, s);
}

int rowgemm_bt_rows(int n_store) {
  const int nt = cdiv(n_store, 16);
  if (nt > 19) return ((n_store + 127) / 128) * 128;
  const int tnt = nt <= 1 ? 1 : nt <= 4 ? 4 : nt <= 8 ? 8 : nt <= 13 ? 13 : 19;
  return ((tnt * 16 + 127) / 128) * 128;
}

bool rowgemm_quad_major_ok(int m, int n_store, int cpad) {
  const int nt = cdiv(n_store, 16);
  if (nt < 14 || nt > 19 || cpad <= 0 || cpad > 160 || cpad % 4 != 0) return false;
  return cdiv(cdiv(rowgemm_main_rows(m, nt), 16), 8) >= 96;
}

int launch_rowgemm(const RowGemmArgs &a, int epi, hipStream_t s) {
  if (a.mode == GEMM_FP32X3) return launch_rowgemm3(a, epi, s);
  if (a.a0q_nvert > 0 && (a.mode == GEMM_BF16_STORAGE || a.m % a.a0q_nvert != 0 || a.ksplit != a.a0q_quads * 4)) {
    set_error("rowgemm: quad-major a0 needs ksplit = 4 * quads (ksplit=%d quads=%d) and whole meshes (m=%d)", a.ksplit, a.a0q_quads, a.m);
    return -1;
  }
  if (a.yq_quads > 0 && (a.zq_nvert <= 0 || a.yq == nullptr || epi != EPI_FWD_HIDDEN || a.yq_quads < a.zq_quads || a.yq_quads * 4 > 160 ||
                         a.yq_quads * 4 > a.n_store)) {
    set_error("rowgemm: quad-major activations need the quad-major forward epilogue and at most 160 columns (yq_quads=%d)", a.yq_quads);
    return -1;
  }
  if (a.zq_nvert > 0 && (epi == EPI_PLAIN || a.mode == GEMM_BF16_STORAGE || a.c2 == nullptr || a.m % a.zq_nvert != 0 ||
                         a.zq_quads * 4 != pad4(a.csplit) || !rowgemm_quad_major_ok(a.m, a.n_store, a.zq_quads * 4))) {
    set_error("rowgemm: quad-major output unsupported for m=%d n=%d csplit=%d epi=%d mode=%d", a.m, a.n_store, a.csplit, epi, a.mode);
    return -1;
  }
  if (epi == EPI_DX_MASK && (a.maskb == nullptr || 32 * a.mld > 4096)) {
    set_error("rowgemm: EPI_DX_MASK needs sign bytes with 32*mld <= 4096 (mld=%d)", a.mld);
    return -1;
  }
  if (a.k % 4 != 0 || a.ksplit % 4 != 0 || a.ldb < pad16(a.k)) {
    set_error("rowgemm: k=%d ksplit=%d ldb=%d violate alignment rules", a.k, a.ksplit, a.ldb);
    return -1;
  }
  if (rowgemmw_ok(a, epi)) return launch_rowgemmw(a, epi, s);
  if (rowgemm16_ok(a, epi)) return launch_rowgemm16(a, epi, s);
  switch (epi) {
    case EPI_PLAIN: return launch_rowgemm_epi<EPI_PLAIN>(a, s);
    case EPI_FWD_HIDDEN: return launch_rowgemm_epi<EPI_FWD_HIDDEN>(a, s);
    case EPI_DX_MASK: return launch_rowgemm_epi<EPI_DX_MASK>(a, s);
  }
  set_error("rowgemm: bad epilogue %d", epi);
  return -1;
}

__global__ void transpose_pad_kernel(const float *__restrict__ w, int k, int n, float *__restrict__ wt,
                                     int rows, int ld) {
  __shared__ float tile[32][33];
  const int bx = blockIdx.x * 32, by = blockIdx.y * 32;
  for (int i = threadIdx.y; i < 32; i += 8) {
    const int kk = bx + i, nn = by + threadIdx.x;
    tile[i][threadIdx.x] = (kk < k && nn < n) ? w[(size_t)kk * n + nn] : 0.f;
  }
  __syncthreads();
  for (int i = threadIdx.y; i < 32; i += 8) {
    const int nn = by + i, kk = bx + threadIdx.x;
    if (nn < rows && kk < ld) wt[(size_t)nn * ld + kk] = tile[threadIdx.x][i];
  }
}

int launch_transpose_pad(const float *w, int k, int n, float *wt, int rows, int ld, hipStream_t s) {
  dim3 grid(cdiv(ld, 32), cdiv(rows, 32));
  A3VT_LAUNCH(transpose_pad_kernel, grid, dim3(32, 8), 0, s, w, k, n, wt, rows, ld);
  A3VT_CHECK_LAUNCH();
  return 0;
}

__global__ void weight_images_kernel(WeightImages w) {
  const int l = blockIdx.z;
  const float *src = w.w[l];
  float *dst = w.dst + (size_t)l * w.dst_stride;
  const int k = w.k[l], n = w.n, rows = w.rows[l], ld = w.ld[l];
  if (w.transpose) {
    __shared__ float tile[32][33];
    const int bx = blockIdx.x * 32, by = blockIdx.y * 32;
    if (bx >= ld || by >= rows) return;
    for (int i = threadIdx.y; i < 32; i += 8) {
      const int kk = bx + i, nn = by + threadIdx.x;
      tile[i][threadIdx.x] = (kk < k && nn < n) ? src[(size_t)kk * n + nn] : 0.f;
    }
    __syncthreads();
    for (int i = threadIdx.y; i < 32; i += 8) {
      const int nn = by + i, kk = bx + threadIdx.x;
      if (nn < rows && kk < ld) dst[(size_t)nn * ld + kk] = tile[threadIdx.x][i];
    }
  } else {
    const int tid = threadIdx.y * 32 + threadIdx.x;
    const int nblk = gridDim.x * gridDim.y, blk = blockIdx.y * gridDim.x + blockIdx.x;
    for (int idx = blk * 256 + tid; idx < rows * ld; idx += nblk * 256) {
      const int r = idx / ld, c = idx % ld;
      dst[idx] = (r < k && c < n) ? src[(size_t)r * n + c] : 0.f;
    }
  }
}

int launch_weight_images(const WeightImages &w, int max_rows, int max_ld, hipStream_t s) {
  A3VT_LAUNCH(weight_images_kernel, dim3(cdiv(max_ld, 32), cdiv(max_rows, 32), w.count), dim3(32, 8), 0, s, w);
  A3VT_CHECK_LAUNCH();
  return 0;
}

__global__ void copy_pad_kernel(const float *__restrict__ w, int rows_in, int cols_in, float *__restrict__ out,
                                int rows, int ld) {
  const int idx = blockIdx.x * blockDim.x + threadIdx.x;
  if (idx >= rows * ld) return;
  const int r = idx / ld, c = idx % ld;
  out[idx] = (r < rows_in && c < cols_in) ? w[(size_t)r * cols_in + c] : 0.f;
}

int launch_copy_pad(const float *w, int rows_in, int cols_in, float *out, int rows, int ld, hipStream_t s) {
  A3VT_LAUNCH(copy_pad_kernel, dim3(cdiv((long long)rows * ld, 256)), dim3(256), 0, s, w, rows_in, cols_in, out,
                     rows, ld);
  A3VT_CHECK_LAUNCH();
  return 0;
}

__global__ void copy_cols_kernel(const float *__restrict__ src, int ld_src, int c0, int w, float *__restrict__ dst,
                                 long long m) {
  const long long i = (long long)blockIdx.x * blockDim.x + threadIdx.x;
  const int w4 = w >> 2;
  if (i >= m * w4) return;
  const long long r = i / w4;
  const int c = (int)(i - r * w4) * 4;
  *reinterpret_cast<f32x4 *>(dst + r * w + c) = *reinterpret_cast<const f32x4 *>(src + r * ld_src + c0 + c);
}

int launch_copy_cols(const float *src, int ld_src, int c0, int w, float *dst, long long m, hipStream_t s) {
  A3VT_LAUNCH(copy_cols_kernel, dim3(cdiv(m * (w >> 2), 256)), dim3(256), 0, s, src, ld_src, c0, w, dst, m);
  A3VT_CHECK_LAUNCH();
  return 0;
}

constexpr int DW_MAXI = 5;
constexpr int DW_MAXO = 3;

template <int NI, int NO>
__device__ __forceinline__ void dw_stage(const float *__restrict__ sb, int ldx, int ldz0, int ldz1, int offG,
                                         int xoff, const int (&zoff)[DW_MAXO], int q, int ni, int no, bool z0q, int rot,
                                         f32x4 (&acc)[DW_MAXI][DW_MAXO]) {
#pragma unroll 1
  for (int ks = 0; ks < 4; ++ks) {
    const int r = q * 4 + ks;
    const float *xr = sb + r * ldx + xoff;
    const int ra = z0q ? ((r + rot) & 15) * 4 : r * ldz0, rg = r * ldz1;
    float a[DW_MAXI], b[DW_MAXO];
#pragma unroll
    for (int i = 0; i < DW_MAXI; ++i) a[i] = xr[i * 16];
#pragma unroll
    for (int j = 0; j < DW_MAXO; ++j) b[j] = sb[zoff[j] + (zoff[j] < offG ? ra : rg)];
#pragma unroll
    for (int i = 0; i < DW_MAXI; ++i) {
      if (NI >= 0 ? i < NI : i < ni) {
#pragma unroll
        for (int j = 0; j < DW_MAXO; ++j)
          if (NO >= 0 ? j < NO : j < no)
            acc[i][j] = __builtin_amdgcn_mfma_f32_16x16x4f32(a[i], b[j], acc[i][j], 0, 0, 0);
      }
    }
  }
}

template <bool HYB, bool BLK>
__device__ __forceinline__ void dw_stage_fast(const float *__restrict__ sb, int ldx, int ldz0, int ldz1, int offG,
                                              int xoff, const int (&zoff)[DW_MAXO], int q, bool row5, bool col3,
                                              int xo, bool z0q, int rot, f32x4 (&acc)[DW_MAXI][DW_MAXO]) {
  float a[DW_MAXI], b[DW_MAXO], an[DW_MAXI], bn[DW_MAXO];
  auto load = [&](int ks, float (&av)[DW_MAXI], float (&bv)[DW_MAXO]) {
    const int r = q * 4 + ks;
    const float *xr = sb + r * ldx + xoff;
    const int rq = ((r + rot) & 15) * 4;
    const int ra = HYB && z0q ? rq : r * ldz0, rg = r * ldz1;
    (void)row5; (void)col3;
    if (HYB && BLK) {
      const float *xb = sb + xo + rq;
#pragma unroll
      for (int i = 0; i < DW_MAXI; ++i) av[i] = xb[i * 256];
    } else {
#pragma unroll
      for (int i = 0; i < DW_MAXI; ++i) av[i] = xr[i * 16];
    }
#pragma unroll
    for (int j = 0; j < DW_MAXO; ++j) bv[j] = sb[zoff[j] + (zoff[j] < offG ? ra : rg)];
  };
  load(0, a, b);
#pragma unroll
  for (int ks = 0; ks < 4; ++ks) {
    if (ks < 3) load(ks + 1, an, bn);
    __builtin_amdgcn_sched_barrier(0);
#pragma unroll
    for (int i = 0; i < 4; ++i)
#pragma unroll
      for (int j = 0; j < 2; ++j) acc[i][j] = __builtin_amdgcn_mfma_f32_16x16x4f32(a[i], b[j], acc[i][j], 0, 0, 0);
    if (row5) {
#pragma unroll
      for (int j = 0; j < 2; ++j) acc[4][j] = __builtin_amdgcn_mfma_f32_16x16x4f32(a[4], b[j], acc[4][j], 0, 0, 0);
    }
    if (col3) {
#pragma unroll
      for (int i = 0; i < 4; ++i) acc[i][2] = __builtin_amdgcn_mfma_f32_16x16x4f32(a[i], b[2], acc[i][2], 0, 0, 0);
      if (row5) acc[4][2] = __builtin_amdgcn_mfma_f32_16x16x4f32(a[4], b[2], acc[4][2], 0, 0, 0);
    }
    __builtin_amdgcn_sched_barrier(0);
#pragma unroll
    for (int i = 0; i < DW_MAXI; ++i) a[i] = an[i];
#pragma unroll
    for (int j = 0; j < DW_MAXO; ++j) b[j] = bn[j];
  }
}

__device__ __forceinline__ void dw_stage_bf16(const float *__restrict__ sb, int ldx, int ldz0, int ldz1, int offG,
                                              int xoff, const int (&zoff)[DW_MAXO], int q, int ni, int no,
                                              f32x4 (&acc)[DW_MAXI][DW_MAXO]) {
  s16x4 a[DW_MAXI], b[DW_MAXO];
#pragma unroll
  for (int i = 0; i < DW_MAXI; ++i) {
    f32x4 v = {0.f, 0.f, 0.f, 0.f};
    if (i < ni) {
#pragma unroll
      for (int ks = 0; ks < 4; ++ks) v[ks] = sb[(q * 4 + ks) * ldx + xoff + i * 16];
    }
    a[i] = cvt_bf16x4(v);
  }
#pragma unroll
  for (int j = 0; j < DW_MAXO; ++j) {
    f32x4 v = {0.f, 0.f, 0.f, 0.f};
    if (j < no) {
      const int ld = zoff[j] < offG ? ldz0 : ldz1;
#pragma unroll
      for (int ks = 0; ks < 4; ++ks) v[ks] = sb[zoff[j] + (q * 4 + ks) * ld];
    }
    b[j] = cvt_bf16x4(v);
  }
#pragma unroll
  for (int i = 0; i < DW_MAXI; ++i) {
    if (i < ni) {
#pragma unroll
      for (int j = 0; j < DW_MAXO; ++j)
// ... 68 lines not shown
  const int stage = offD + 256;

  const int units = (p.m + 15) >> 4;
  const int ubase = units / gridDim.x, urem = units % gridDim.x;
  const int u0 = blockIdx.x * ubase + (blockIdx.x < urem ? blockIdx.x : urem);
  const int nu = ubase + (blockIdx.x < urem ? 1 : 0);

  const float *sp[3];
  int sstep[3];
  int sdst[3];
  int srow[3];
  const int qn = p.xq_nvert > 0 ? p.xq_nvert : p.z0q_nvert;
  int sjq[3];
#pragma unroll
  for (int j = 0; j < 3; ++j) {
    const int s = wave * 3 + j;
    const float *img = nullptr, *imgq = nullptr;
    int ld = 0, w = 4, c0 = 0, li = 0, nquad = 0, cend = 0;
    bool blocked = false;
    sdst[j] = offD;
    if (s < nbq) {
      img = p.x; ld = p.ldx_src; c0 = 0; cend = p.ldx; li = s; sdst[j] = li * 256;
      imgq = p.xq; nquad = p.xq_quads; blocked = true;
    } else if (s < xin) {
      img = p.x; ld = p.ldx_src; w = wrm; c0 = nbq * 16; li = s - nbq; sdst[j] = s * 256;
    } else if (s < xin + ain) {
      li = s - xin; sdst[j] = offA + li * 256;
      if (z0q) { imgq = p.z0; nquad = p.z0q_quads; c0 = a0; cend = a0 + wa; blocked = true; }
      else { img = p.z0; ld = p.ldz0; w = wa; c0 = a0; }
    } else if (s < xin + ain + gin) {
      img = p.z1; ld = p.ldz1; w = wg; c0 = g0; li = s - xin - ain; sdst[j] = offG + li * 256;
    }
    int row, col;
    bool valid;
    if (blocked) {
      const int qd = lane >> 4;
      row = ((lane & 15) - qd) & 15;
      col = c0 + li * 16 + qd * 4;
      valid = col < cend && (img != nullptr || col < nquad * 4);
    } else {
      const int wq = w >> 2, f4 = li * 64 + lane;
      row = f4 / wq;
      col = c0 + (f4 - row * wq) * 4;
      valid = img != nullptr && row < 16;
    }
    const size_t grow = (size_t)u0 * 16 + row;
    sp[j] = valid && img != nullptr ? img + grow * ld + col : p.zeros;
    sstep[j] = valid ? 16 * ld : 0;
    srow[j] = valid ? row : 0x7fffffff;
    sjq[j] = (nquad - 1) * qn * 4;
    if (valid && imgq != nullptr && col < nquad * 4) {
      const int bq = (int)(grow / qn), vq = (int)(grow - (size_t)bq * qn);
      sp[j] = imgq + (((size_t)bq * nquad + (col >> 2)) * qn + vq) * 4;
      sstep[j] = 64;
    }
  }

  int next_mesh = qn > 0 ? (int)((((size_t)u0 * 16) / qn + 1) * qn) : 0x7fffffff;
  auto advance = [&](int unit) {
#pragma unroll
    for (int j = 0; j < 3; ++j) sp[j] += sstep[j];
    if (HYB && unit * 16 + 31 >= next_mesh) {
#pragma unroll
      for (int j = 0; j < 3; ++j) {
        const int g = unit * 16 + (srow[j] & 15);
        if (sstep[j] == 64 && g < next_mesh && g + 16 >= next_mesh) sp[j] += sjq[j];
      }
      if (unit * 16 + 16 >= next_mesh) next_mesh += qn;
    }
  };
  auto issue = [&](int unit, int buf) {
    float *base = lds + buf * stage;
    const int rows_left = p.m - unit * 16;
    if (rows_left >= 16) {
#pragma unroll
      for (int j = 0; j < 3; ++j) glds16(sp[j], base + sdst[j]);
    } else {
#pragma unroll
      for (int j = 0; j < 3; ++j) glds16(srow[j] < rows_left ? sp[j] : p.zeros, base + sdst[j]);
    }
    advance(unit);
  };

  f32x4 acc[MAXI][DW_MAXO];
#pragma unroll
  for (int i = 0; i < MAXI; ++i)
#pragma unroll
    for (int j = 0; j < DW_MAXO; ++j) acc[i][j] = f32x4{0.f, 0.f, 0.f, 0.f};

  int zoff[DW_MAXO];
#pragma unroll
  for (int j = 0; j < DW_MAXO; ++j) {
    const int col = (o0 + j) * 16 + l16;
    const int ca = col - a0;
    zoff[j] = col < p.zsplit ? offA + (z0q ? (ca >> 4) * 256 + ((ca & 15) >> 2) * 64 + (ca & 3) : ca) : offG + (col - g0);
  }
  const int xo = i0 < nbq ? i0 * 256 + (l16 >> 2) * 64 + (l16 & 3) : -1;
  const int rot = l16 >> 2;

  const int xoff = HYB ? nbq * 256 + (i0 - nbq) * 16 + l16 : i0 * 16 + l16;
  const int nst = p.nstage;
  for (int d = 0; d < nst - 1; ++d)
    if (d < nu) issue(u0 + d, d);
  int buf = 0;
  for (int t = 0; t < nu; ++t) {
    const int younger = min(nu - 1 - t, nst - 2);
    if (younger >= 3) wait_vmcnt<9>();
    else if (younger == 2) wait_vmcnt<6>();
    else if (younger == 1) wait_vmcnt<3>();
    else wait_vmcnt<0>();
    __builtin_amdgcn_s_barrier();
    if (t + nst - 1 < nu) issue(u0 + t + nst - 1, buf >= 1 ? buf - 1 : nst - 1);
    const float *sb = lds + buf * stage;
    if constexpr (NARROW) {
      dw_stage_narrow<HYB>(sb, p.ldx, wa, wg, offG, xoff, zoff, q, no == 3, z0q, rot, acc);
    } else {
    if (BF16) dw_stage_bf16(sb, p.ldx, wa, wg, offG, xoff, zoff, q, ni, no, acc);
    else if (FAST && HYB) {
      if (xo >= 0) dw_stage_fast<true, true>(sb, wrm, wa, wg, offG, xoff, zoff, q, true, no == 3, xo, z0q, rot, acc);
      else dw_stage_fast<true, false>(sb, wrm, wa, wg, offG, xoff, zoff, q, true, no == 3, xo, z0q, rot, acc);
    } else if (FAST) dw_stage_fast<false, false>(sb, p.ldx, wa, wg, offG, xoff, zoff, q, true, no == 3, xo, z0q, rot, acc);
    else dw_stage<-1, -1>(sb, p.ldx, wa, wg, offG, xoff, zoff, q, ni, no, z0q, rot, acc);
    }
    buf = buf == nst - 1 ? 0 : buf + 1;
  }
  wait_lgkm0();

  float *slab = p.slab + (size_t)blockIdx.x * p.k_in * p.n_out;
#pragma unroll
  for (int i = 0; i < MAXI; ++i) {
    if (i >= ni) continue;
#pragma unroll
    for (int r = 0; r < 4; ++r) {
      const int kin = (i0 + i) * 16 + q * 4 + r;
      if (kin >= p.k_in) continue;
#pragma unroll
      for (int j = 0; j < DW_MAXO; ++j) {
        if (j >= no) continue;
        const int col = (o0 + j) * 16 + l16;
        if (col < p.n_out) slab[(size_t)kin * p.n_out + col] = acc[i][j][r];
      }
    }
  }
}

bool dw_quad_major_ok(int k_in, int quads) { return quads % 4 == 0 && dw_blocked_tiles(k_in, quads) == quads / 4; }

static int dw_col_groups(int n_out) { return cdiv(cdiv(n_out, 16), 4 * DW_MAXO); }
int dw_num_slabs(int n_out) {
  const int g = dw_col_groups(n_out);
  return 256 / g > 0 ? 256 / g : 1;
}

int dw_images(const DwArgs &a) { return a.mode != GEMM_FP32X3 && dww_ok(a) ? dww_images() : dw_num_slabs(a.n_out); }
int dw_slab_capacity(int n_out) { return dw_num_slabs(n_out) > dww_images() ? dw_num_slabs(n_out) : dww_images(); }

constexpr int kDwStageUnits = 48;
bool dw_rows_fit(int ldx, int ldz0, int ldz1) {
  return (16 * ldx + 255) / 256 + (16 * ldz0 + 255) / 256 + (16 * ldz1 + 255) / 256 <= kDwStageUnits;
}

int launch_dw(const DwArgs &a0, hipStream_t s) {
  if (a0.mode == GEMM_FP32X3) return launch_dw3(a0, s);
  DwArgs a = a0;
  if (a.ldx_src == 0) a.ldx_src = a.ldx;
  if ((a.xq_nvert > 0 && (a.xq == nullptr || a.xq_quads * 4 > a.k_in || a.m % a.xq_nvert != 0)) ||
      (a.z0q_nvert > 0 && (a.z0q_quads * 4 != a.zsplit || a.m % a.z0q_nvert != 0)) ||
      (a.xq_nvert > 0 && a.z0q_nvert > 0 && a.xq_nvert != a.z0q_nvert) || a.mode == GEMM_BF16_STORAGE ||
      (a.xq_nvert > 0 && a.xq_nvert < 32) || (a.z0q_nvert > 0 && a.z0q_nvert < 32) ||
      ((a.xq_nvert > 0 || a.z0q_nvert > 0) && (a.ldx_src == 4 || a.ldz1 == 4 || a.ldz0 == 4))) {
    set_error("dw: quad-major operands unsupported (xq %d x %d, z0q %d x %d, m=%d)", a.xq_nvert, a.xq_quads, a.z0q_nvert,
              a.z0q_quads, a.m);
    return -1;
  }
  if (a.ldx % 4 || a.ldz0 % 4 || a.ldz1 % 4 || a.k_in > DW_MAXI * 64 || a.k_in > a.ldx ||
      a.n_out > a.ldz1 || a.zsplit > a.ldz0) {
    set_error("dw: unsupported dims k_in=%d n_out=%d ldx=%d ldz0=%d ldz1=%d", a.k_in, a.n_out, a.ldx, a.ldz0, a.ldz1);
    return -1;
  }
  if (dww_ok(a)) return launch_dww(a, s);
  const bool hyb = a.xq_nvert > 0 || a.z0q_nvert > 0;
  if (hyb) path_count(PATH_DW_HYBRID);
  const int nbq = a.xq_nvert > 0 ? a.xq_quads / 4 : 0, wrm = a.ldx - nbq * 16;
  if (a.xq_nvert > 0 && (a.xq_quads % 4 != 0 || dw_blocked_tiles(a.k_in, a.xq_quads) != nbq)) {
    set_error("dw: quad-major X columns (%d) must end where a wave's input tiles end (k_in=%d)", a.xq_quads * 4, a.k_in);
    return -1;
  }
  const int xin = nbq + (16 * wrm + 255) / 256, ain = (16 * a.ldz0 + 255) / 256, gin = (16 * a.ldz1 + 255) / 256;
  if (xin + ain + gin > kDwStageUnits) {
    set_error("dw: rows too wide (%d + %d + %d floats)", a.ldx, a.ldz0, a.ldz1);
    return -1;
  }
  const int tout_all = cdiv(a.n_out, 16), ngrp = dw_col_groups(a.n_out);
  int worst = 0;
  for (int gy = 0; gy < ngrp; ++gy) {
    const int gbase = tout_all / ngrp, grem = tout_all % ngrp;
    const int gt0 = gy * gbase + (gy < grem ? gy : grem), gtn = gbase + (gy < grem ? 1 : 0);
    const int c0 = gt0 * 16, c1 = (gt0 + gtn) * 16 < a.n_out ? (gt0 + gtn) * 16 : a.n_out;
    const int a0 = (c0 < a.zsplit ? c0 : a.zsplit) & ~3, a1 = ((c1 < a.zsplit ? c1 : a.zsplit) + 3) & ~3;
    const int g0 = (c0 > a.zsplit ? c0 : a.zsplit) & ~3;
    int g1 = ((c1 > a.zsplit ? c1 : a.zsplit) + 3) & ~3;
    g1 = g1 < a.ldz1 ? g1 : a.ldz1;
    const int wa = a1 > a0 ? a1 - a0 : 0, wg = g1 > g0 ? g1 - g0 : 0;
    const int units = xin + (a.z0q_nvert > 0 ? (wa + 15) / 16 : (16 * wa + 255) / 256) + (16 * wg + 255) / 256 + 1;
    worst = units > worst ? units : worst;
  }
  DwArgs args = a;
  args.nstage = (int)((160 * 1024) / ((size_t)worst * 1024));
  args.nstage = args.nstage > 5 ? 5 : args.nstage;
  if (args.nstage < 3) {
    set_error("dw: rows too wide for a 3-stage ring (%d KB per stage)", worst);
    return -1;
  }
  const size_t shmem = (size_t)args.nstage * worst * 1024;
  static OncePerDevice once;
  once.run([] {
    (void)hipFuncSetAttribute((const void *)dw_kernel<true, false, false>, hipFuncAttributeMaxDynamicSharedMemorySize, 160 * 1024);
    (void)hipFuncSetAttribute((const void *)dw_kernel<false, false, false>, hipFuncAttributeMaxDynamicSharedMemorySize, 160 * 1024);
    (void)hipFuncSetAttribute((const void *)dw_kernel<false, true, false>, hipFuncAttributeMaxDynamicSharedMemorySize, 160 * 1024);
    (void)hipFuncSetAttribute((const void *)dw_kernel<true, false, true>, hipFuncAttributeMaxDynamicSharedMemorySize, 160 * 1024);
    (void)hipFuncSetAttribute((const void *)dw_kernel<false, false, true>, hipFuncAttributeMaxDynamicSharedMemorySize, 160 * 1024);
    (void)hipFuncSetAttribute((const void *)dw_kernel<false, false, true, true>, hipFuncAttributeMaxDynamicSharedMemorySize, 160 * 1024);
    (void)hipFuncSetAttribute((const void *)dw_kernel<false, false, false, true>, hipFuncAttributeMaxDynamicSharedMemorySize, 160 * 1024);
  });
  const int tin = cdiv(a.k_in, 16), tout = cdiv(a.n_out, 16), groups = dw_col_groups(a.n_out);
  const bool fast = tin / 4 >= 4 && tin <= 20 && (tout / groups) / 4 >= 2 && cdiv(tout, groups) <= 12;
  if (hyb && (a.mode != GEMM_FP32 || (a.xq_nvert > 0 && !fast))) {
    set_error("dw: quad-major operands need the fp32 kernels (and quad-major X the 300-wide shape): k_in=%d n_out=%d mode=%d",
              a.k_in, a.n_out, a.mode);
    return -1;
  }
  const dim3 grid(dw_num_slabs(a.n_out), groups);
  const bool narrow = a.mode == GEMM_FP32 && tin <= 4 && a.xq_nvert == 0 && (tout / groups) / 4 >= 2 && cdiv(tout, groups) <= 12;
  if (narrow && hyb) A3VT_LAUNCH((dw_kernel<false, false, true, true>), grid, dim3(1024), shmem, s, args);
  else if (narrow) A3VT_LAUNCH((dw_kernel<false, false, false, true>), grid, dim3(1024), shmem, s, args);
  else if (a.mode == GEMM_BF16_OPERANDS) A3VT_LAUNCH((dw_kernel<false, true, false>), grid, dim3(1024), shmem, s, args);
  else if (fast && hyb) A3VT_LAUNCH((dw_kernel<true, false, true>), grid, dim3(1024), shmem, s, args);
  else if (fast) A3VT_LAUNCH((dw_kernel<true, false, false>), grid, dim3(1024), shmem, s, args);
  else if (hyb) A3VT_LAUNCH((dw_kernel<false, false, true>), grid, dim3(1024), shmem, s, args);
  else A3VT_LAUNCH((dw_kernel<false, false, false>), grid, dim3(1024), shmem, s, args);
  A3VT_CHECK_LAUNCH();
  return 0;
}

__global__ __launch_bounds__(1024) void slab_reduce_kernel(const float *__restrict__ slab, int nslab, size_t stride,
                                                           size_t n, size_t n_out, float *__restrict__ out, int accumulate) {
  __shared__ float part[16][64];
  const int lane = threadIdx.x & 63, grp = threadIdx.x >> 6;
  const size_t i = (size_t)blockIdx.x * 64 + lane;
  const int per = (nslab + 15) / 16;
  const int s0 = grp * per, s1 = min(s0 + per, nslab);
  float a[8] = {0.f, 0.f, 0.f, 0.f, 0.f, 0.f, 0.f, 0.f};
  if (i < n) {
    int s = s0;
    for (; s + 7 < s1; s += 8) {
#pragma unroll
      for (int u = 0; u < 8; ++u) a[u] += slab[(size_t)(s + u) * stride + i];
    }
    for (; s < s1; ++s) a[0] += slab[(size_t)s * stride + i];
  }
  part[grp][lane] = ((a[0] + a[1]) + (a[2] + a[3])) + ((a[4] + a[5]) + (a[6] + a[7]));
  __syncthreads();
  if (grp == 0 && i < n_out) {
    float t = 0.f;
#pragma unroll
    for (int g = 0; g < 16; ++g) t += part[g][lane];
    t = i < n ? t : 0.f;
    out[i] = accumulate ? out[i] + t : t;
  }
}

__global__ __launch_bounds__(1024) void slab_reduce_tall_kernel(const float *__restrict__ slab, int nslab, size_t stride,
                                                                size_t n, size_t n_out, float *__restrict__ out, int accumulate) {
  __shared__ float part[64][17];
  const int o = threadIdx.x & 15, grp = threadIdx.x >> 4;
  const size_t i = (size_t)blockIdx.x * 16 + o;
  float a[8] = {0.f, 0.f, 0.f, 0.f, 0.f, 0.f, 0.f, 0.f};
  if (i < n) {
    int sl = grp;
    for (; sl + 7 * 64 < nslab; sl += 8 * 64) {
#pragma unroll
      for (int u = 0; u < 8; ++u) a[u] += slab[(size_t)(sl + u * 64) * stride + i];
    }
    for (; sl < nslab; sl += 64) a[0] += slab[(size_t)sl * stride + i];
  }
  part[grp][o] = ((a[0] + a[1]) + (a[2] + a[3])) + ((a[4] + a[5]) + (a[6] + a[7]));
  __syncthreads();
  if (grp == 0 && i < n_out) {
    float t = 0.f;
#pragma unroll
    for (int g = 0; g < 64; ++g) t += part[g][o];
    t = i < n ? t : 0.f;
    out[i] = accumulate ? out[i] + t : t;
  }
}

__global__ __launch_bounds__(1024) void slab_reduce_batch_kernel(SlabReduceBatch b) {
  __shared__ float part[16][64];
  const int lane = threadIdx.x & 63, grp = threadIdx.x >> 6;
  const size_t i = (size_t)blockIdx.x * 64 + lane;
  const float *__restrict__ slab = b.slab + (size_t)blockIdx.y * b.layer_stride;
  const int per = (b.nslab + 15) / 16;
  const int s0 = grp * per, s1 = min(s0 + per, b.nslab);
  float a[8] = {0.f, 0.f, 0.f, 0.f, 0.f, 0.f, 0.f, 0.f};
  if (i < b.n) {
    int s = s0;
    for (; s + 7 < s1; s += 8) {
#pragma unroll
      for (int u = 0; u < 8; ++u) a[u] += slab[(size_t)(s + u) * b.stride + i];
    }
    for (; s < s1; ++s) a[0] += slab[(size_t)s * b.stride + i];
  }
  part[grp][lane] = ((a[0] + a[1]) + (a[2] + a[3])) + ((a[4] + a[5]) + (a[6] + a[7]));
  __syncthreads();
  if (grp == 0 && i < b.n_out) {
    float t = 0.f;
#pragma unroll
    for (int g = 0; g < 16; ++g) t += part[g][lane];
    t = i < b.n ? t : 0.f;
    float *out = b.out[blockIdx.y];
    out[i] = b.accumulate ? out[i] + t : t;
  }
}
__global__ __launch_bounds__(1024) void slab_reduce_tall_batch_kernel(SlabReduceBatch b) {
  __shared__ float part[64][17];
  const int o = threadIdx.x & 15, grp = threadIdx.x >> 4;
  const size_t i = (size_t)blockIdx.x * 16 + o;
  const float *__restrict__ slab = b.slab + (size_t)blockIdx.y * b.layer_stride;
  float a[8] = {0.f, 0.f, 0.f, 0.f, 0.f, 0.f, 0.f, 0.f};
  if (i < b.n) {
    int sl = grp;
    for (; sl + 7 * 64 < b.nslab; sl += 8 * 64) {
#pragma unroll
      for (int u = 0; u < 8; ++u) a[u] += slab[(size_t)(sl + u * 64) * b.stride + i];
    }
    for (; sl < b.nslab; sl += 64) a[0] += slab[(size_t)sl * b.stride + i];
  }
  part[grp][o] = ((a[0] + a[1]) + (a[2] + a[3])) + ((a[4] + a[5]) + (a[6] + a[7]));
  __syncthreads();
  if (grp == 0 && i < b.n_out) {
    float t = 0.f;
#pragma unroll
    for (int g = 0; g < 64; ++g) t += part[g][o];
    t = i < b.n ? t : 0.f;
    float *out = b.out[blockIdx.y];
    out[i] = b.accumulate ? out[i] + t : t;
  }
}
int launch_slab_reduce_batch(const SlabReduceBatch &b, hipStream_t s) {
  if (b.count <= 0) return 0;
  if (b.nslab >= 512 && b.n_out <= 1024)
    A3VT_LAUNCH(slab_reduce_tall_batch_kernel, dim3(cdiv((long long)b.n_out, 16), b.count), dim3(1024), 0, s, b);
  else
    A3VT_LAUNCH(slab_reduce_batch_kernel, dim3(cdiv((long long)b.n_out, 64), b.count), dim3(1024), 0, s, b);
  A3VT_CHECK_LAUNCH();
  return 0;
}

int launch_slab_reduce_za(const float *slab, int nslab, size_t stride, size_t n, size_t n_out, float *out, int accumulate,
                          hipStream_t s) {
  if (nslab >= 512 && n_out <= 1024)
    A3VT_LAUNCH(slab_reduce_tall_kernel, dim3(cdiv((long long)n_out, 16)), dim3(1024), 0, s, slab, nslab, stride, n, n_out, out,
                accumulate);
  else
    A3VT_LAUNCH(slab_reduce_kernel, dim3(cdiv((long long)n_out, 64)), dim3(1024), 0, s, slab, nslab, stride, n, n_out, out,
                accumulate);
  A3VT_CHECK_LAUNCH();
  return 0;
}
int launch_slab_reduce(const float *slab, int nslab, size_t stride, size_t n, float *out, hipStream_t s) {
  return launch_slab_reduce_za(slab, nslab, stride, n, n, out, 0, s);
}

}
```

active-3d-vision-and-touch_amd/csrc/gcn_gemmw.hip:

```cpp
#include <type_traits>

#include "gemm_tile.h"

namespace a3vt {

constexpr int kWChunks = 19;
constexpr int kWStage = kWChunks * 256;
constexpr int kWStages = 3;
constexpr int kWMaskSlot = 512;
constexpr int kWLdsFloats = (kWStages + 2) * kWStage + (3 + 5) * kWMaskSlot;

template <int V>
using WIdx = std::integral_constant<int, V>;

template <int EPI>
struct WShape {
  static constexpr int K = 300, N = 300, ZQ = 25;
  static constexpr int YQ = EPI == EPI_FWD_HIDDEN ? 40 : 25;
  static constexpr int KSPLIT = EPI == EPI_FWD_HIDDEN ? 160 : 100;
};

__device__ __forceinline__ void w_mfma(bool first, bool a_in_agpr, f32x4 &acc, float a, float b) {
  if (first) {
    if (a_in_agpr) asm("v_mfma_f32_16x16x4_f32 %0, %1, %2, 0" : "=a"(acc) : "a"(a), "v"(b));
    else asm("v_mfma_f32_16x16x4_f32 %0, %1, %2, 0" : "=a"(acc) : "v"(a), "v"(b));
  } else {
    if (a_in_agpr) asm("v_mfma_f32_16x16x4_f32 %0, %1, %2, %0" : "+a"(acc) : "a"(a), "v"(b));
    else asm("v_mfma_f32_16x16x4_f32 %0, %1, %2, %0" : "+a"(acc) : "v"(a), "v"(b));
  }
}
__device__ __forceinline__ void w_mfma_done() { asm volatile("s_nop 15\n\ts_nop 3" ::: "memory"); }


template <int EPI>
__device__ __forceinline__ void rowgemmw_compute(const RowGemmArgs &p, float *lds, int wave, int lane, int t0, int t1) {
  constexpr int NT = 5;
  const int l16 = lane & 15, q = lane >> 4;
  float *sA = lds, *sE = lds + kWStages * kWStage;
  constexpr int NV = 3;
  float bv[kWChunks][4][NV], ba[kWChunks][4][NT - NV];
#pragma unroll
  for (int t = 0; t < NT; ++t) {
    const float *br = p.bt + (size_t)((wave + 3 * t) * 16 + l16) * p.ldb + q * 4;
#pragma unroll
    for (int c = 0; c < kWChunks; ++c) {
      const f32x4 v = *reinterpret_cast<const f32x4 *>(br + c * 16);
#pragma unroll
      for (int sidx = 0; sidx < 4; ++sidx) {
        if (t < NV) bv[c][sidx][t] = v[sidx];
        else ba[c][sidx][t - NV] = v[sidx];
      }
    }
  }
  wait_vmcnt<0>();
  wait_lgkm0();
  __builtin_amdgcn_s_barrier();
  int st = 0;
  for (int tile = t0; tile < t1; ++tile) {
    const float *sa = sA + st * kWStage + lane * 4;
    float *se = sE + ((tile - t0) & 1) * kWStage + lane * 4;
    f32x4 acc[NT];
    f32x4 af = *reinterpret_cast<const f32x4 *>(sa);
#pragma unroll
    for (int c = 0; c < kWChunks; ++c) {
      f32x4 an = af;
      if (c + 1 < kWChunks) an = *reinterpret_cast<const f32x4 *>(sa + (c + 1) * 256);
#pragma unroll
      for (int sidx = 0; sidx < 4; ++sidx) {
#pragma unroll
        for (int t = 0; t < NT; ++t) {
          if (t < NV) w_mfma(c == 0 && sidx == 0, false, acc[t], bv[c][sidx][t], af[sidx]);
          else w_mfma(c == 0 && sidx == 0, true, acc[t], ba[c][sidx][t - NV], af[sidx]);
        }
      }
      af = an;
    }
    w_mfma_done();
#pragma unroll
    for (int t = 0; t < NT; ++t) *reinterpret_cast<f32x4 *>(se + (wave + 3 * t) * 256) = acc[t];
    wait_lgkm0();
    __builtin_amdgcn_s_barrier();
    st = st == 2 ? 0 : st + 1;
  }
  __builtin_amdgcn_s_barrier();
}

template <int EPI>
__device__ __forceinline__ void rowgemmw_service(const RowGemmArgs &p, float *lds, int lane, int t0, int t1) {
  constexpr int NT = 4, T0 = 15;
  using S = WShape<EPI>;
  const int l16 = lane & 15, q = lane >> 4;
  const int nvert = p.zq_nvert;
  const unsigned nv16 = (unsigned)nvert * 16u;
  float *sA = lds, *sE = lds + kWStages * kWStage;
  uint8_t *msout = reinterpret_cast<uint8_t *>(lds + (kWStages + 2) * kWStage);
  uint8_t *msin = reinterpret_cast<uint8_t *>(lds + (kWStages + 2) * kWStage + 3 * kWMaskSlot);
  constexpr int NV = 2;
  float bv[kWChunks][4][NV], ba[kWChunks][4][NT - NV];
#pragma unroll
  for (int t = 0; t < NT; ++t) {
    const float *br = p.bt + (size_t)((T0 + t) * 16 + l16) * p.ldb + q * 4;
#pragma unroll
    for (int c = 0; c < kWChunks; ++c) {
      const f32x4 v = *reinterpret_cast<const f32x4 *>(br + c * 16);
#pragma unroll
      for (int sidx = 0; sidx < 4; ++sidx) {
        if (t < NV) bv[c][sidx][t] = v[sidx];
        else ba[c][sidx][t - NV] = v[sidx];
      }
    }
  }
  if (EPI == EPI_FWD_HIDDEN) {
    for (int i = lane; i < 2 * kWMaskSlot; i += 64) reinterpret_cast<float *>(msout)[i] = 0.f;
  }

  int d_bq, d_vq, e_bq, e_vq;
  auto locate = [&](int tile, int &bq, int &vq) {
    const int row = tile * 16 + l16;
    bq = row / nvert;
    vq = row - bq * nvert;
  };
  auto advance = [&](int &bq, int &vq) {
    vq += 16;
    const bool wrap = vq >= nvert;
    vq = wrap ? vq - nvert : vq;
    bq = wrap ? bq + 1 : bq;
  };
  unsigned d_off0, d_off1;
  auto refresh_d = [&](int tile, bool on) {
    d_off0 = on ? ((unsigned)(d_bq * (S::KSPLIT / 4) + q) * (unsigned)nvert + (unsigned)d_vq) * 16u : 0u;
    d_off1 = on ? ((unsigned)(tile * 16 + l16) * (unsigned)p.lda1 + (unsigned)q * 4u) * 4u : 0u;
  };
  unsigned e_off0, e_off1, e_off2, e_mrow;
  auto refresh_e = [&](int tile, int mslot) {
    e_off0 = ((unsigned)(e_bq * S::ZQ + q) * (unsigned)nvert + (unsigned)e_vq) * 16u;
    e_off1 = ((unsigned)(e_bq * S::YQ + q) * (unsigned)nvert + (unsigned)e_vq) * 16u;
    e_off2 = ((unsigned)(tile * 16 + l16) * (unsigned)p.ldc + (unsigned)q * 4u) * 4u;
    e_mrow = (unsigned)((EPI == EPI_FWD_HIDDEN && p.maskb == nullptr ? 2 : mslot) * 2048 + l16 * p.mld + p.moff + q);
  };
  int sz = 0;
  auto a_issue = [&](auto cc, int stage, bool on) {
    constexpr int c = decltype(cc)::value;
    float *dst = sA + stage * kWStage + c * 256;
    const float *b0 = on ? p.a0 + (size_t)c * 4 * nvert * 4 + sz : p.zeros;
    const float *b1 = on ? p.a1 + c * 16 + sz : p.zeros;
    const char *src;
    if (c * 16 + 16 <= S::KSPLIT) {
      src = w_at(b0, d_off0);
    } else if (c * 16 >= S::KSPLIT && c * 16 + 16 <= S::K) {
      src = w_at(b1, d_off1);
    } else {
      const int k0 = c * 16 + q * 4;
      src = k0 >= S::K ? reinterpret_cast<const char *>(p.zeros) : (k0 < S::KSPLIT ? w_at(b0, d_off0) : w_at(b1, d_off1));
    }
    glds16(reinterpret_cast<const float *>(src), dst);
  };
  auto m_issue = [&](int tile, int slot, bool on) {
    const uint8_t *src0 = p.maskb + (size_t)tile * 16 * p.mld;
    const int nbytes = on ? 16 * p.mld : 0;
#pragma unroll
    for (int o = 0; o < 2048; o += 1024) {
      const int b = o + lane * 16;
      const void *src = b < nbytes ? (const void *)(src0 + b) : (const void *)p.zeros;
      glds16(reinterpret_cast<const float *>(src), reinterpret_cast<float *>(msin + (on ? slot : 4) * 2048 + o));
    }
  };
  auto m_flush = [&](int tile, int mslot) {
    const int nbytes = 16 * p.mld;
    uint8_t *dstm = p.maskb + (size_t)tile * 16 * p.mld;
#pragma unroll
    for (int o = 0; o < 2048; o += 1024) {
      const int b = o + lane * 16;
      if (b < nbytes) *reinterpret_cast<f32x4 *>(dstm + b) = *reinterpret_cast<const f32x4 *>(msout + mslot * 2048 + b);
    }
  };
  auto relu_bits = [](f32x4 &v) {
    float o0, o1, o2, o3;
    unsigned b0, b1, b2, b3;
    asm("v_max_f32 %0, 0, %8\n\tv_max_f32 %1, 0, %9\n\tv_max_f32 %2, 0, %10\n\tv_max_f32 %3, 0, %11\n\t"
        "v_min_u32 %4, 1, %0\n\tv_min_u32 %5, 1, %1\n\tv_min_u32 %6, 1, %2\n\tv_min_u32 %7, 1, %3\n\t"
        "v_lshl_or_b32 %4, %5, 1, %4\n\tv_lshl_or_b32 %4, %6, 2, %4\n\tv_lshl_or_b32 %4, %7, 3, %4"
        : "=&v"(o0), "=&v"(o1), "=&v"(o2), "=&v"(o3), "=&v"(b0), "=&v"(b1), "=&v"(b2), "=&v"(b3)
        : "v"(v[0]), "v"(v[1]), "v"(v[2]), "v"(v[3]));
    v = f32x4{o0, o1, o2, o3};
    return b0;
  };
  auto mask4 = [](f32x4 &v, unsigned byte) {
    float o0, o1, o2, o3;
    asm("v_bfe_i32 %0, %8, 0, 1\n\tv_bfe_i32 %1, %8, 1, 1\n\tv_bfe_i32 %2, %8, 2, 1\n\tv_bfe_i32 %3, %8, 3, 1\n\t"
        "v_and_b32 %0, %0, %4\n\tv_and_b32 %1, %1, %5\n\tv_and_b32 %2, %2, %6\n\tv_and_b32 %3, %3, %7"
        : "=&v"(o0), "=&v"(o1), "=&v"(o2), "=&v"(o3)
        : "v"(v[0]), "v"(v[1]), "v"(v[2]), "v"(v[3]), "v"(byte));
    v = f32x4{o0, o1, o2, o3};
  };
  auto epi_fetch = [&](auto tc, int eslot, int mslot_in, f32x4 &v, unsigned &byte) {
    constexpr int T = decltype(tc)::value;
    v = *reinterpret_cast<const f32x4 *>(sE + eslot * kWStage + T * 256 + lane * 4);
    byte = EPI == EPI_DX_MASK ? msin[mslot_in * 2048 + (e_mrow & 2047u) + 4 * T] : 0u;
  };
  auto epi = [&](auto tc, f32x4 v, unsigned byte) {
    constexpr int T = decltype(tc)::value;
    const int lo = 4 * T, hi = 4 * T + 3;
    if (hi < S::ZQ) {
      *reinterpret_cast<f32x4 *>(const_cast<char *>(w_at(p.c2 + (size_t)T * 4 * nvert * 4 + sz, e_off0))) = v;
    } else if (EPI == EPI_FWD_HIDDEN && lo >= S::ZQ && hi < S::YQ) {
      const unsigned bits = relu_bits(v);
      *reinterpret_cast<f32x4 *>(const_cast<char *>(w_at(p.yq + (size_t)T * 4 * nvert * 4 + sz, e_off1))) = v;
      msout[e_mrow + 4 * T] = (uint8_t)bits;
    } else if (lo >= S::YQ && hi * 4 + 3 < S::N) {
      if (EPI == EPI_FWD_HIDDEN) {
        const unsigned bits = relu_bits(v);
        msout[e_mrow + 4 * T] = (uint8_t)bits;
      } else {
        mask4(v, byte);
      }
      *reinterpret_cast<f32x4 *>(const_cast<char *>(w_at(p.c + T * 16 + sz, e_off2))) = v;
    } else {
      const int c4 = lo + q;
      const bool valid = c4 * 4 < S::N, act = c4 >= S::ZQ;
      if (valid && !act) {
        *reinterpret_cast<f32x4 *>(const_cast<char *>(w_at(p.c2 + (size_t)T * 4 * nvert * 4 + sz, e_off0))) = v;
      } else if (valid) {
        if (EPI == EPI_FWD_HIDDEN) {
          const unsigned bits = relu_bits(v);
          msout[e_mrow + 4 * T] = (uint8_t)bits;
          if (c4 < S::YQ) *reinterpret_cast<f32x4 *>(const_cast<char *>(w_at(p.yq + (size_t)T * 4 * nvert * 4 + sz, e_off1))) = v;
          else *reinterpret_cast<f32x4 *>(const_cast<char *>(w_at(p.c + T * 16 + sz, e_off2))) = v;
        } else {
          mask4(v, byte);
          *reinterpret_cast<f32x4 *>(const_cast<char *>(w_at(p.c + T * 16 + sz, e_off2))) = v;
        }
      }
    }
  };

#pragma unroll
  for (int d = 0; d < 2; ++d) {
    locate(t0 + d, d_bq, d_vq);
    refresh_d(t0 + d, t0 + d < t1);
    if (EPI == EPI_DX_MASK) m_issue(t0 + d, (t0 + d) & 3, t0 + d < t1);
    [&]<int... C>(std::integer_sequence<int, C...>) { (a_issue(WIdx<C>{}, d, t0 + d < t1), ...); }(std::make_integer_sequence<int, kWChunks>{});
  }
  locate(t0 + 2, d_bq, d_vq);
  refresh_d(t0 + 2, t0 + 2 < t1);
  locate(t0, e_bq, e_vq);
  wait_vmcnt<0>();
  wait_lgkm0();
  __builtin_amdgcn_s_barrier();

  int st = 0;
  auto tile_body = [&](int tile, auto firstc) {
    constexpr bool have_prev = !decltype(firstc)::value;
    const int par = (tile - t0) & 1;
    const bool have_next = tile + 2 < t1;
    const int nst = st == 0 ? 2 : st - 1;
    const float *sa = sA + st * kWStage + lane * 4;
    asm volatile("s_mov_b32 %0, 0" : "=s"(sz));
    if (have_prev) refresh_e(tile - 1, EPI == EPI_FWD_HIDDEN ? (par ^ 1) : 0);
    if (EPI == EPI_DX_MASK) m_issue(tile + 2, (tile + 2) & 3, have_next);
    if (EPI == EPI_FWD_HIDDEN && p.maskb && tile - 2 >= t0) m_flush(tile - 2, par);
    f32x4 acc[NT];
    f32x4 af = *reinterpret_cast<const f32x4 *>(sa);
    auto chunk = [&](auto cc) {
      constexpr int c = decltype(cc)::value;
      f32x4 an = af, ev = {0.f, 0.f, 0.f, 0.f};
      unsigned eb = 0;
      if (c + 1 < kWChunks) an = *reinterpret_cast<const f32x4 *>(sa + (c + 1) * 256);
      if (have_prev) epi_fetch(cc, par ^ 1, (tile - 1) & 3, ev, eb);
      __builtin_amdgcn_sched_barrier(0);
#pragma unroll
      for (int sidx = 0; sidx < 4; ++sidx) {
#pragma unroll
        for (int t = 0; t < NT; ++t) {
          if (t < NV) w_mfma(c == 0 && sidx == 0, false, acc[t], bv[c][sidx][t], af[sidx]);
          else w_mfma(c == 0 && sidx == 0, true, acc[t], ba[c][sidx][t - NV], af[sidx]);
        }
      }
      __builtin_amdgcn_sched_barrier(0);
      asm volatile("s_mov_b32 %0, 0" : "=s"(sz));
      a_issue(cc, nst, have_next);
      if (have_prev) epi(cc, ev, eb);
      __builtin_amdgcn_sched_barrier(0);
      af = an;
    };
    [&]<int... C>(std::integer_sequence<int, C...>) { (chunk(WIdx<C>{}), ...); }(std::make_integer_sequence<int, kWChunks>{});
    {
      float *se = sE + par * kWStage + lane * 4;
      w_mfma_done();
#pragma unroll
      for (int t = 0; t < NT; ++t) *reinterpret_cast<f32x4 *>(se + (T0 + t) * 256) = acc[t];
    }
    advance(d_bq, d_vq);
    refresh_d(tile + 3, tile + 3 < t1);
    if (have_prev) advance(e_bq, e_vq);
    wait_vmcnt<24>();
    wait_lgkm0();
    __builtin_amdgcn_s_barrier();
    st = st == 2 ? 0 : st + 1;
  };
  if (t1 > t0) tile_body(t0, std::true_type{});
  for (int tile = t0 + 1; tile < t1; ++tile) tile_body(tile, std::false_type{});
  if (t1 > t0) {
    const int last = t1 - 1, lpar = (last - t0) & 1;
    asm volatile("s_mov_b32 %0, 0" : "=s"(sz));
    refresh_e(last, EPI == EPI_FWD_HIDDEN ? lpar : 0);
    [&]<int... C>(std::integer_sequence<int, C...>) {
      ((void)[&] {
        f32x4 ev;
        unsigned eb;
        epi_fetch(WIdx<C>{}, lpar, last & 3, ev, eb);
        epi(WIdx<C>{}, ev, eb);
      }(), ...);
    }(std::make_integer_sequence<int, kWChunks>{});
    wait_lgkm0();
    if (EPI == EPI_FWD_HIDDEN && p.maskb) {
      if (last - 1 >= t0) m_flush(last - 1, lpar ^ 1);
      m_flush(last, lpar);
    }
  }
  __builtin_amdgcn_s_barrier();
}

template <int EPI>
__global__ __launch_bounds__(256) __attribute__((amdgpu_waves_per_eu(1, 1))) void rowgemmw_kernel(RowGemmArgs p) {
  extern __shared__ __attribute__((aligned(16))) float lds[];
  const int lane = threadIdx.x & 63;
  const int wave = __builtin_amdgcn_readfirstlane(threadIdx.x >> 6);
  const int per = (p.m >> 4) / (int)gridDim.x;
  const int t0 = blockIdx.x * per, t1 = t0 + per;
  if (wave < 3) rowgemmw_compute<EPI>(p, lds, wave, lane, t0, t1);
  else rowgemmw_service<EPI>(p, lds, lane, t0, t1);
  if (p.rem_rows > 0) {
    const int ntl = (p.n_store + 15) >> 4;
    const int units = ((p.rem_rows + 15) >> 4) * ntl;
    for (int u = wave * gridDim.x + blockIdx.x; u < units; u += 4 * gridDim.x)
      rowtile_unit<EPI, 0>(p, p.rem_row0, p.rem_row0 + p.rem_rows, u / ntl, (u % ntl) * 16, lane);
  }
}

bool rowgemmw_ok(const RowGemmArgs &a, int epi) {
  if (a.mode != GEMM_FP32 || (epi != EPI_FWD_HIDDEN && epi != EPI_DX_MASK)) return false;
  if (a.zq_nvert <= 0 || a.a0q_nvert != a.zq_nvert || a.c2 == nullptr || a.m % a.zq_nvert != 0 || a.m % 16 != 0) return false;
  if (a.k <= 288 || a.k > 304 || a.n_store <= 288 || a.n_store > 304 || a.n_store % 4 != 0 || a.k % 4 != 0) return false;
  if (a.ksplit != a.a0q_quads * 4 || a.ldc % 4 != 0 || a.lda1 % 4 != 0 || a.ldb < 304) return false;
  if (a.mld > 128 || a.mld % 4 != 0 || a.zq_quads * 4 > a.n_store) return false;
  if (epi == EPI_FWD_HIDDEN && (a.yq_quads < a.zq_quads || (a.yq_quads > a.zq_quads && a.yq == nullptr))) return false;
  if (epi == EPI_DX_MASK && a.maskb == nullptr) return false;
  if (a.trash == nullptr || a.zq_nvert < 16 || a.m > 3000000) return false;
  if (a.k != 300 || a.n_store != 300 || a.zq_quads != 25 || a.no_relu) return false;
  if (epi == EPI_FWD_HIDDEN && (a.yq_quads != 40 || a.ksplit != 160)) return false;
  if (epi == EPI_DX_MASK && a.ksplit != 100) return false;
  return (a.m >> 4) >= 768;
}

template <int EPI>
static int launch_rowgemmw_epi(const RowGemmArgs &a0, hipStream_t s) {
  RowGemmArgs a = a0;
  a.bt_rows = rowgemm_bt_rows(a.n_store);
  a.col0 = 0;
  const int ncu = (a.m >> 4) >= 4 * 256 ? 256 : (a.m >> 4) / 4;
  static OncePerDevice once;
  once.run([] {
    (void)hipFuncSetAttribute((const void *)rowgemmw_kernel<EPI>, hipFuncAttributeMaxDynamicSharedMemorySize,
                              (int)(kWLdsFloats * sizeof(float)));
  });
  const int tiles = a.m >> 4, per = tiles / ncu;
  a.rem_row0 = per * ncu * 16;
  a.rem_rows = a.m - a.rem_row0;
  path_count(PATH_RGW);
  A3VT_LAUNCH((rowgemmw_kernel<EPI>), dim3(ncu), dim3(256), kWLdsFloats * sizeof(float), s, a);
  A3VT_CHECK_LAUNCH();
  return 0;
}

int launch_rowgemmw(const RowGemmArgs &a, int epi, hipStream_t s) {
  if (!rowgemmw_ok(a, epi)) {
    set_error("rowgemmw: shape not taken (m=%d k=%d n=%d epi=%d)", a.m, a.k, a.n_store, epi);
    return -1;
  }
  return epi == EPI_FWD_HIDDEN ? launch_rowgemmw_epi<EPI_FWD_HIDDEN>(a, s) : launch_rowgemmw_epi<EPI_DX_MASK>(a, s);
}

}
```

active-3d-vision-and-touch_amd/csrc/gemm_tile.h:

```cpp
#pragma once
#include "kernels.h"
#include "prims.h"

namespace a3vt {

template <int EPI, int MODE>
__device__ __forceinline__ void rowtile_unit(const RowGemmArgs &p, int row_base, int row_end, int mt, int n0, int lane) {
  constexpr int KB = 19;
  const int l16 = lane & 15, q = lane >> 4;
  const int ar = min(row_base + mt * 16 + l16, row_end - 1);
  const int br = min(n0 + l16, p.bt_rows - 1);
  const float *a1r = p.a1 + (size_t)ar * p.lda1;
  const float *a0r = p.a0 + (size_t)ar * p.lda0;
  size_t a0mul = 1;
  if (p.a0q_nvert > 0) {
    const int bq = ar / p.a0q_nvert;
    a0r = p.a0 + ((size_t)bq * p.a0q_quads * p.a0q_nvert + (size_t)(ar - bq * p.a0q_nvert)) * 4;
    a0mul = (size_t)p.a0q_nvert;
  }
  const float *btr = p.bt + (size_t)br * p.ldb;
  const int nch = (p.k + 15) >> 4;
  f32x4 acc = {0.f, 0.f, 0.f, 0.f};
  for (int c0 = 0; c0 < nch; c0 += KB) {
    f32x4 af[KB], bf[KB];
#pragma unroll
    for (int c = 0; c < KB; ++c) {
      const int kk = (c0 + c) * 16 + q * 4;
      const bool on = c0 + c < nch && kk < p.k;
      af[c] = on ? *reinterpret_cast<const f32x4 *>(kk < p.ksplit ? a0r + (size_t)kk * a0mul : a1r + kk) : f32x4{0.f, 0.f, 0.f, 0.f};
      bf[c] = on ? *reinterpret_cast<const f32x4 *>(btr + kk) : f32x4{0.f, 0.f, 0.f, 0.f};
    }
#pragma unroll
    for (int c = 0; c < KB; ++c) {
      if (MODE == 2) {
        acc = mfma_bf16x32(af[c], bf[c], acc);
      } else if (MODE == 1) {
        acc = __builtin_amdgcn_mfma_f32_16x16x16bf16_1k(cvt_bf16x4(af[c]), cvt_bf16x4(bf[c]), acc, 0, 0, 0);
      } else {
#pragma unroll
        for (int t = 0; t < 4; ++t) acc = __builtin_amdgcn_mfma_f32_16x16x4f32(af[c][t], bf[c][t], acc, 0, 0, 0);
      }
    }
  }
  const int col = n0 + l16;
  const bool col_ok = col < p.n_store;
#pragma unroll
  for (int r = 0; r < 4; ++r) {
    const int row = row_base + mt * 16 + q * 4 + r;
    const bool row_ok = row < row_end;
    float v = acc[r];
    if (EPI == EPI_PLAIN) {
      if (p.plain_relu) v = v > 0.f ? v : 0.f;
      if (row_ok && col_ok) p.c[(size_t)row * p.ldc + col] = v;
    } else if (EPI == EPI_FWD_HIDDEN) {
      const unsigned mybit = (col_ok && col >= p.csplit && v > 0.f) ? 1u << (l16 & 3) : 0u;
      unsigned bits = mybit;
      bits |= __shfl_xor(bits, 1, 64);
      bits |= __shfl_xor(bits, 2, 64);
      if (row_ok && p.maskb && (l16 & 3) == 0 && (col | 3) >= p.csplit && col < ((p.n_store + 3) & ~3))
        p.maskb[(size_t)row * p.mld + p.moff + (col >> 2)] = (uint8_t)bits;
      if (MODE == 2) {
        if (row_ok && col < p.ldc) {
          if (col < p.csplit) reinterpret_cast<u16 *>(p.c2)[(size_t)row * p.ldc2 + col] = bf16_round(v);
          else reinterpret_cast<u16 *>(p.c)[(size_t)row * p.ldc + col] = bf16_round((v > 0.f || p.no_relu) ? v : 0.f);
        }
      } else if (row_ok && col_ok) {
        if (p.zq_nvert > 0 && col < p.zq_quads * 4) {
          const int bq = row / p.zq_nvert;
          p.c2[(((size_t)bq * p.zq_quads + (col >> 2)) * p.zq_nvert + (row - bq * p.zq_nvert)) * 4 + (col & 3)] = v;
        } else if (p.zq_nvert > 0 && col < p.yq_quads * 4) {
          const int bq = row / p.zq_nvert;
          p.yq[(((size_t)bq * p.yq_quads + (col >> 2)) * p.zq_nvert + (row - bq * p.zq_nvert)) * 4 + (col & 3)] =
              (v > 0.f || p.no_relu) ? v : 0.f;
        } else if (p.zq_nvert == 0 && col < p.csplit) {
          p.c2[(size_t)row * p.ldc2 + col] = v;
        } else {
          p.c[(size_t)row * p.ldc + col] = (v > 0.f || p.no_relu) ? v : 0.f;
        }
      }
    } else {
      if (MODE == 2) {
        if (row_ok && col < p.ldc) {
          const unsigned byte = col_ok ? p.maskb[(size_t)row * p.mld + (col < p.csplit ? 0 : p.moff) + (col >> 2)] : 0u;
          reinterpret_cast<u16 *>(p.c)[(size_t)row * p.ldc + col] = bf16_round(((byte >> (col & 3)) & 1u) ? v : 0.f);
        }
      } else if (row_ok && col_ok) {
        if (p.zq_nvert > 0 && col < p.zq_quads * 4) {
          const int bq = row / p.zq_nvert;
          p.c2[(((size_t)bq * p.zq_quads + (col >> 2)) * p.zq_nvert + (row - bq * p.zq_nvert)) * 4 + (col & 3)] = v;
        } else {
          const unsigned byte = p.maskb[(size_t)row * p.mld + (col < p.csplit ? 0 : p.moff) + (col >> 2)];
          p.c[(size_t)row * p.ldc + col] = ((byte >> (col & 3)) & 1u) ? v : 0.f;
        }
      }
    }
  }
}

__device__ __forceinline__ const char *w_at(const void *base, unsigned off) { return reinterpret_cast<const char *>(base) + (size_t)off; }

}
```

active-3d-vision-and-touch_amd/csrc/kernels.h:

```cpp
#pragma once
#include <hip/hip_runtime.h>
#include <stddef.h>
#include <stdint.h>

namespace a3vt {

enum { EPI_PLAIN = 0, EPI_FWD_HIDDEN = 1, EPI_DX_MASK = 2 };
enum GemmMode { GEMM_FP32 = 0, GEMM_BF16_OPERANDS = 1, GEMM_BF16_STORAGE = 2, GEMM_FP32X3 = 3 };

struct RowGemmArgs {
  const float *a0;
  const float *a1;
  const float *bt;
  const float *zeros;
  uint8_t *maskb;
  float *c;
  float *c2;
  int lda0, lda1, ksplit, ldb;
  int bt_rows;
  int col0;
  int m, k, n_store;
  int ldc, ldc2, csplit, mld, moff;
  int no_relu;
  int plain_relu;
  int mode;
  int rem_row0, rem_rows;
  int zq_nvert, zq_quads;
  float *yq;
  int yq_quads;
  int a0q_nvert, a0q_quads;
  float *trash;
};
int rowgemm_bt_rows(int n_store);
int launch_rowgemm(const RowGemmArgs &a, int epi, hipStream_t s);
bool rowgemmw_ok(const RowGemmArgs &a, int epi);
int launch_rowgemmw(const RowGemmArgs &a, int epi, hipStream_t s);
bool rowgemm16_ok(const RowGemmArgs &a, int epi);
int launch_rowgemm16(const RowGemmArgs &a, int epi, hipStream_t s);
int launch_transpose_pad(const float *w, int k, int n, float *wt, int rows, int ld, hipStream_t s);
int launch_copy_pad(const float *w, int rows_in, int cols_in, float *out, int rows, int ld, hipStream_t s);
constexpr int kMaxImages = 32;
struct WeightImages {
  const float *w[kMaxImages];
  float *dst;
  size_t dst_stride;
  int k[kMaxImages], rows[kMaxImages], ld[kMaxImages];
  int n, count, transpose;
};
int launch_weight_images(const WeightImages &w, int max_rows, int max_ld, hipStream_t s);

struct SlabReduceBatch {
  const float *slab;
  float *out[kMaxImages];
  size_t layer_stride, stride, n, n_out;
  int count, nslab, accumulate;
};
int launch_slab_reduce_batch(const SlabReduceBatch &b, hipStream_t s);

constexpr int kX3ImageRows = 320;
constexpr int kX3ImageLd = 160;
constexpr int kX3ImageFloats = kX3ImageRows * kX3ImageLd;
bool rowgemm3_dims_ok(long long m, int k, int n_store);
bool rowgemm3_stack_ok(long long m, int hidden, int mld);
bool rowgemm3_ok(const RowGemmArgs &a, int epi);
int launch_rowgemm3(const RowGemmArgs &a, int epi, hipStream_t s);
int launch_weight_images3(const WeightImages &w, hipStream_t s);
int launch_split3(const float *x, size_t n, unsigned short *hi, unsigned short *mid, unsigned short *lo, hipStream_t s);

struct DwArgs {
  const float *x;
  const float *z0;
  const float *z1;
  const float *zeros;
  float *slab;
  int ldx, ldz0, ldz1, zsplit;
  int m, k_in, n_out;
  int mode;
  int nstage;
  const float *xq;
  int ldx_src, xq_nvert, xq_quads, z0q_nvert, z0q_quads;
};
int dw_num_slabs(int n_out);
int dw_images(const DwArgs &a);
int dw_slab_capacity(int n_out);
bool dw3_ok(const DwArgs &a);
int launch_dw3(const DwArgs &a, hipStream_t s);
bool dw_quad_major_ok(int k_in, int quads);
bool dw_rows_fit(int ldx, int ldz0, int ldz1);
int launch_dw(const DwArgs &a, hipStream_t s);
bool dww_ok(const DwArgs &a);
int dww_images();
int launch_dww(const DwArgs &a, hipStream_t s);
int launch_copy_cols(const float *src, int ld_src, int c0, int w, float *dst, long long m, hipStream_t s);
int launch_slab_reduce(const float *slab, int nslab, size_t stride, size_t n, float *out, hipStream_t s);
int launch_slab_reduce_za(const float *slab, int nslab, size_t stride, size_t n, size_t n_out, float *out, int accumulate,
                          hipStream_t s);

int launch_csr_fwd(const float *za, int ldza, const float *bias, int c, const int32_t *rowptr, const int32_t *col,
                   const float *val, const int32_t *heavy, int n_vert, int batch, float *y, int ldy, uint8_t *maskb,
                   int mld, int relu, hipStream_t s);
size_t csr_heavy_scratch_ints(int n_vert);
int csr_heavy_degree();
int launch_csr_heavy_list(const int32_t *rowptr, int n_vert, int32_t *heavy, hipStream_t s);
int launch_relu_split(const float *gy, int ldgy, const float *y, int ldy, int relu, int n_out, int cpad, int npad,
                      long long m, float *ga, float *dz, hipStream_t s);
int csr_bwd_num_slabs(int batch, int n_vert);
int launch_csr_bwd(const float *g, int ldg, int c, const int32_t *rowptrT, const int32_t *colT, const float *valT,
                   const int32_t *heavyT, int n_vert, int batch, float *dza, int lddza, float *db_slab, hipStream_t s);

bool csrq_fits(int n_vert, int cut_len);
int csrq_max_degree();
size_t csrq_ell_ints(int n_vert);
int launch_csrq_ell(const int32_t *rowptr, const int32_t *col, const float *val, int n_vert, int32_t *ell, hipStream_t s);
int launch_csrq_fwd(const float *zq, const float *bias, int c, const int32_t *rowptr, const int32_t *col,
                    const float *val, const int32_t *heavy, const int32_t *ell, int n_vert, int batch, float *yq,
                    int yq_quads ,
                    uint8_t *signq, int relu, hipStream_t s);
int launch_csrq_bwd(const float *gq, int c, const int32_t *rowptrT, const int32_t *colT, const float *valT,
                    const int32_t *heavyT, const int32_t *ellT, int n_vert, int batch, float *dzaq, const uint8_t *signq,
                    float *db_slab, hipStream_t s);
struct SplitRef {
  const int32_t *rowptr, *col;
  const float *scale;
  const uint8_t *cls;
};
bool csrqs_fits(int n_vert, int cut_len);
int csrqs_max_degree();
int launch_csrqs_image(const int32_t *rowptr, const int32_t *col, const float *scale, const uint8_t *cls, int n_vert,
                       int32_t *img, hipStream_t s);
int launch_csrqs_fwd(const float *zq, const float *bias, int c, const int32_t *img, int n_vert, int batch, float *yq,
                     int yq_quads, uint8_t *signq, int relu, hipStream_t s);
int launch_csrqs_bwd(const float *gq, int c, const int32_t *img, int n_vert, int batch, float *dzaq, const uint8_t *signq,
                     float *db_slab, hipStream_t s);
bool rowgemm_quad_major_ok(int m, int n_store, int cpad);

int thin_num_slabs();
int launch_thin_fwd(const float *x, int ldx, int k, const float *w , const float *bias ,
                    const int32_t *rowptr, const int32_t *col, const float *val, const int32_t *heavy, int n_vert,
                    int batch, float *z3 , float *update ,
                    const float *xq , int xq_quads,
                    hipStream_t s, const SplitRef *sp = nullptr);
int launch_thin_bwd(const float *x, int ldx, int k, const float *w, const int32_t *rowptrT, const int32_t *colT,
                    const float *valT, const int32_t *heavyT, int n_vert, int batch,
                    const float *grad_update , float *dz3 , int apply_mask,
                    float *g_prev , int ldg, int n_store, float *dw_slab ,
                    float *db_slab , float *gq , int nq,
                    const float *xq , int xq_quads, hipStream_t s, const SplitRef *sp = nullptr);

int launch_vertex_update(const float *vin, const float *upd, int batch, int n_vert, int n_vision, float *vout,
                         hipStream_t s);
int launch_check_finite(const float *d, size_t n, int32_t *flag, hipStream_t s);
int launch_fill_zero(float *d, size_t n, hipStream_t s);

int launch_cvt_rows(const float *in, int ld_in, int n, void *out, int ld_out, long long m, hipStream_t s);
int launch_weight_images16(const WeightImages &w, int max_rows, int max_ld, hipStream_t s);
struct Dw16Args {
  const unsigned short *x;
  const unsigned short *z0;
  const unsigned short *z1;
  const float *zeros;
  float *slab;
  int ldx, xc0, xw, ldz0, ldz1, zsplit;
  int m, k_in, n_out;
  int nstage;
};
int dw16_num_slabs(int n_out);
int launch_dw16(const Dw16Args &a, hipStream_t s);
int launch_csr16_fwd(const void *za, int ldza, const float *bias, int c, const int32_t *rowptr, const int32_t *col,
                     const float *val, const int32_t *heavy, int n_vert, int batch, void *y, int ldy, uint8_t *maskb,
                     int mld, int relu, hipStream_t s);
int launch_csr16_bwd(const void *g, int ldg, int c, int cpad, const int32_t *rowptrT, const int32_t *colT,
                     const float *valT, const int32_t *heavyT, int n_vert, int batch, void *dza, int lddza,
                     float *db_slab, hipStream_t s);
size_t csr16t_plan_ints(int n_vert);
bool csr16t_ok(int n_vert, int c, int max_degree, long long m);
int launch_csr16t_build(const int32_t *rowptr, const int32_t *col, const float *val, int n_vert, int32_t *plan, hipStream_t s);
int launch_csr16t_fwd(const void *za, int ldza, const float *bias, int c, const int32_t *plan, const int32_t *rowptr,
                      const int32_t *col, const float *val, int n_vert, int batch, void *y, int ldy, uint8_t *maskb, int mld,
                      int relu, hipStream_t s);
int launch_csr16t_bwd(const void *g, int ldg, int c, int cpad, const int32_t *planT, const int32_t *rowptrT,
                      const int32_t *colT, const float *valT, int n_vert, int batch, void *dza, int lddza, float *db_slab,
                      hipStream_t s);
int launch_thin16_fwd_product(const void *x, int ldx, int k, const float *w, long long m, float *z3, hipStream_t s);
int launch_thin16_bwd_main(const void *x, int ldx, int k, const float *w, const float *dz3, const float *du, long long m,
                           int apply_mask, void *gprev, int ldg, float *dw_slab, float *db_slab, hipStream_t s);
int launch_csr3(const float *z, const float *bias, const int32_t *rowptr, const int32_t *col, const float *val,
                const int32_t *heavy, int n_vert, int batch, float *out, int ldo, hipStream_t s,
                const SplitRef *sp = nullptr ,
                bool transposed = false);
int launch_pad3to4(const float *in, long long m, float *out, hipStream_t s);

size_t posenc_param_count(int input_size);
int posenc_num_slabs(int m);
int launch_posenc_fwd(const float *verts, const float *mask, int m, int input_size, const float *params, float *feats,
                      int ld, hipStream_t s);
int launch_posenc_bwd(const float *verts, const float *mask, int m, int input_size, const float *params,
                      const float *gfeats, int ld, float *gverts, float *gparams, float *scratch, hipStream_t s);

bool posenc_wide_supported(int input_size);
size_t posenc_wide_acts_floats(int m, int input_size);
size_t posenc_wide_scratch_floats(int m, int input_size, int need_backward);
int launch_posenc_wide_fwd(const float *verts, const float *mask, int m, int input_size, const float *params, float *feats,
                           int ld, float *acts, float *scratch, const float *zeros, int gemm_bf16, hipStream_t s);
int launch_posenc_wide_bwd(const float *verts, const float *mask, int m, int input_size, const float *params,
                           const float *gfeats, int ld, const float *acts, float *gverts, float *gparams, float *scratch,
                           const float *zeros, int gemm_bf16, hipStream_t s);

int launch_face_cdf(const float *verts, const int32_t *faces, int batch, int n_vert, int n_faces, float *cdf,
                    hipStream_t s);
int launch_sample_fwd(const float *verts, const int32_t *faces, const float *cdf, int batch, int n_vert, int n_faces,
                      int draws, int num, const int32_t *fi_in, const float *u_in, const float *v_in, uint64_t seed,
                      uint64_t offset, float *points, int32_t *fi_out, float *u_out, float *v_out, hipStream_t s);
int launch_sample_bwd(const int32_t *faces, int batch, int n_vert, int n_faces, int draws, int num,
                      const int32_t *fi, const float *u, const float *v, const float *gpoints, float *gverts,
                      hipStream_t s);

constexpr int kMaxMaps = 4;
struct PoolArgs {
  const float *verts;
  float proj[12];
  int batch, n_vert, n_maps;
  const float *maps[kMaxMaps];
  float *gmaps[kMaxMaps];
  int C[kMaxMaps], H[kMaxMaps], W[kMaxMaps], off[kMaxMaps];
  float *feats;
  const float *base;
  const float *gfeats;
  int ld;
  float *gverts;
};
int launch_pool_fwd(PoolArgs a, hipStream_t s);
int launch_pool_bwd(PoolArgs a, hipStream_t s);

int bias_grad_wgs(long long n_elem, int c);
int launch_bias_grad(const void *g, int bf16, long long rows, int c, float *out, float *slab, hipStream_t s);

int bnrelu_wgs(long long n_elem, int c, int per_thread, int cap);
size_t bnrelu_scratch_bytes(int c);
int launch_bnrelu_fwd(const void *x, long long rows, int c, const float *gamma, const float *beta, const float *pre_bias, float eps,
                      float momentum, float *running_mean, float *running_var, long long *num_batches, void *y, float *save,
                      void *scratch, hipStream_t s);
int launch_bnrelu_bwd(const void *dy, const void *x, long long rows, int c, const float *save, void *dx, float *dgamma,
                      float *dbeta, float *dx_colsum, void *scratch, hipStream_t s);

// ... 145 lines not shown
```

include/a3vt.h:

```cpp
#ifndef A3VT_H
#define A3VT_H
#include <stddef.h>
#include <stdint.h>

#ifdef __cplusplus
extern "C" {
#endif

#define A3VT_VERSION 163

int a3vt_version(void);
const char *a3vt_last_error(void);

int a3vt_csr_validate(const int32_t *rowptr_host, const int32_t *col_host, int n_vert, int nnz);

size_t a3vt_gcn_stack_scratch_bytes(int batch, int n_vert, int in_features, int hidden, int num_layers,
                                    int cut_len, int need_backward);
size_t a3vt_gcn_stack_mask_bytes(int batch, int n_vert, int hidden, int num_layers, int cut_len);
size_t a3vt_gcn_stack_scratch_bytes_mode(int batch, int n_vert, int in_features, int hidden, int num_layers,
                                         int cut_len, int need_backward, int gemm_bf16);
int a3vt_gcn_stack_stash_bytes(int batch, int n_vert, int hidden, int num_layers, int cut_len, int gemm_bf16,
                               size_t *acts_bytes, size_t *mask_bytes);

int a3vt_gcn_stack_fwd(const float *feats, int ld_feats, int in_features,
// ... 22 lines not shown
                           const void *acts, const uint8_t *masks, const float *grad_update,
                           float *const *grad_weights, float *const *grad_biases, float *grad_feats,
                           float *scratch, int accumulate, void *stream);

typedef struct a3vt_adj_split {
  const int32_t *rowptr;
  const int32_t *col;
  const float *scale;
  const uint8_t *cls;
  int32_t max_degree;
  int32_t n_seam, n_centre;
} a3vt_adj_split;

int a3vt_adj_split_validate(const int32_t *csr_rowptr, const int32_t *csr_col, const float *csr_val, int n_vert,
                            const int32_t *p_rowptr, const int32_t *p_col, const float *scale, const uint8_t *cls);

int a3vt_gcn_stack_fwd_adj(const float *feats, int ld_feats, int in_features,
                           const float *const *weights, const float *const *biases,
                           int num_layers, int hidden, int cut_len,
                           const int32_t *csr_rowptr, const int32_t *csr_col, const float *csr_val, int csr_max_degree,
                           const a3vt_adj_split *split,
                           int n_vert, int batch, int gemm_bf16,
                           void *acts, uint8_t *masks, float *scratch, float *update, void *stream);
int a3vt_gcn_stack_bwd_adj(const float *feats, int ld_feats, int in_features,
                           const float *const *weights, const float *const *biases,
                           int num_layers, int hidden, int cut_len,
                           const int32_t *csr_rowptr, const int32_t *csr_col, const float *csr_val,
                           const int32_t *csrT_rowptr, const int32_t *csrT_col, const float *csrT_val, int csrT_max_degree,
                           const a3vt_adj_split *split,
                           int n_vert, int batch, int gemm_bf16,
                           const void *acts, const uint8_t *masks, const float *grad_update,
                           float *const *grad_weights, float *const *grad_biases, float *grad_feats,
                           float *scratch, int accumulate, void *stream);

size_t a3vt_gcn_layer_scratch_bytes(int batch, int n_vert, int ld_x, int out_features, int cut_len,
                                    int need_backward);
int a3vt_gcn_layer_fwd(const float *x, int ld_x, int in_features, const float *weight, const float *bias,
                       int out_features, int cut_len, int relu,
                       const int32_t *csr_rowptr, const int32_t *csr_col, const float *csr_val, int csr_max_degree,
                       int n_vert, int batch, int gemm_bf16, float *y, int ld_y, float *scratch, void *stream);
int a3vt_gcn_layer_bwd(const float *x, int ld_x, int in_features, const float *weight,
                       int out_features, int cut_len, int relu,
                       const int32_t *csrT_rowptr, const int32_t *csrT_col, const float *csrT_val, int csrT_max_degree,
                       int n_vert, int batch, int gemm_bf16, const float *y, int ld_y, const float *grad_y, int ld_gy,
                       float *grad_weight, float *grad_bias, float *grad_x, float *scratch, void *stream);

int a3vt_wt_rows(int n_out);
int a3vt_wt_ld(int k);
int a3vt_transpose_weight(const float *w, int k, int n_out, float *wt, void *stream);
int a3vt_rowgemm(const float *a, int lda, int m, int k, const float *wt, int n_out, int gemm_bf16,
                 float *c, int ldc, void *stream);

size_t a3vt_posenc_param_count(int input_size);
size_t a3vt_posenc_scratch_bytes(int m, int input_size);
int a3vt_posenc_mask_fwd(const float *verts, const float *mask, int m, int input_size,
                         const float *pe_params, float *feats, int ld_feats, void *stream);
int a3vt_posenc_mask_bwd(const float *verts, const float *mask, int m, int input_size,
                         const float *pe_params, const float *grad_feats, int ld_feats,
                         float *grad_verts, float *grad_params, float *scratch, void *stream);

int a3vt_posenc_wide_supported(int input_size);
size_t a3vt_posenc_wide_acts_bytes(int m, int input_size);
size_t a3vt_posenc_wide_scratch_bytes(int m, int input_size, int need_backward);
int a3vt_posenc_wide_fwd(const float *verts, const float *mask, int m, int input_size, const float *pe_params,
                         float *feats, int ld_feats, float *acts, float *scratch, int gemm_bf16, void *stream);
int a3vt_posenc_wide_bwd(const float *verts, const float *mask, int m, int input_size, const float *pe_params,
                         const float *grad_feats, int ld_feats, const float *acts, float *grad_verts,
                         float *grad_params, float *scratch, int gemm_bf16, void *stream);

int a3vt_image_pool_fwd(const float *verts, int batch, int n_vert, const float *proj_host, int n_maps,
                        const float *const *maps, const int *chans, const int *heights, const int *widths,
                        float *feats, int ld_feats, void *stream);
int a3vt_image_pool_fwd_add(const float *verts, int batch, int n_vert, const float *proj_host, int n_maps,
                            const float *const *maps, const int *chans, const int *heights, const int *widths,
                            const float *base, float *feats, int ld_feats, void *stream);
int a3vt_image_pool_bwd(const float *verts, int batch, int n_vert, const float *proj_host, int n_maps,
                        const float *const *maps, const int *chans, const int *heights, const int *widths,
                        const float *grad_feats, int ld_feats, float *const *grad_maps, float *grad_verts,
                        void *stream);

size_t a3vt_bias_grad_scratch_bytes(long long rows, int channels);
int a3vt_bias_grad_nhwc(const void *grad, int bf16, long long rows, int channels, float *out, void *scratch,
                        size_t scratch_bytes, void *stream);

size_t a3vt_bnrelu_scratch_bytes(int channels);
int a3vt_bnrelu_fwd(const void *x, long long rows, int channels, const float *gamma, const float *beta, const float *pre_bias,
                    float eps, float momentum, float *running_mean, float *running_var, long long *num_batches_tracked, void *y,
                    float *save, void *scratch, size_t scratch_bytes, void *stream);
int a3vt_bnrelu_bwd(const void *dy, const void *x, long long rows, int channels, const float *save, void *dx, float *dgamma,
                    float *dbeta, float *dx_colsum, void *scratch, size_t scratch_bytes, void *stream);

int a3vt_cast_weights_bf16(int n, const float *const *src, void *const *dst, const long long *outer, const int *inner,
                           const int *hw, void *stream);

int a3vt_conv5_supported(int cin, int cout, int stride);
size_t a3vt_conv5_image_bytes(int cout, int cin, int flip);
int a3vt_conv5_weight_image(const float *weight, int cout, int cin, int flip, void *image, void *stream);
int a3vt_conv5_nhwc(const void *x, int batch, int height, int width, int cin, int cout, int stride, int pad, const void *image,
                    const float *bias, void *y, void *stream);

int a3vt_conv5_input_grad_3x16s2(const void *grad_out, int batch, int out_height, int out_width, const void *image, void *grad_in,
                                 void *stream);

size_t a3vt_conv5_wrw_scratch_bytes(int cin, int cout);
int a3vt_conv5_weight_grad(const void *x, const void *grad_out, int batch, int height, int width, int cin, int cout, int stride,
                           float *grad_weight, void *scratch, size_t scratch_bytes, void *stream);

int a3vt_conv5f_supported(int cin, int cout, int stride);
size_t a3vt_conv5f_image_bytes(int cin, int cout);
int a3vt_conv5f_weight_image(const float *weight, int cout, int cin, void *image, void *stream);
int a3vt_conv5f_nhwc(const float *x, int batch, int height, int width, int cin, int cout, int stride, int pad, const void *image,
                     const float *scale, const float *shift, int relu, float *y, void *stream);

int a3vt_adam_chunk_elems(void);
int a3vt_adam_step(void *const *param, const void *const *grad, void *const *exp_avg, void *const *exp_avg_sq,
                   const long long *numel, const int *chunk_tensor, const long long *chunk_off, int n_chunks, double lr, double beta1,
                   double beta2, double eps, double weight_decay, long long step, void *stream);
int a3vt_adam_step_clamp(void *const *param, void *const *grad, void *const *exp_avg, void *const *exp_avg_sq, const long long *numel,
                         const int *chunk_tensor, const long long *chunk_off, int n_chunks, double lr, double beta1, double beta2,
                         double eps, double weight_decay, long long step, double grad_clamp, void *stream);

int a3vt_vertex_update(const float *verts_in, const float *update, int batch, int n_vert, int n_vision,
                       float *verts_out, void *stream);

int a3vt_face_cdf(const float *verts, const int32_t *faces, int batch, int n_vert, int n_faces,
                  float *cdf, void *stream);
int a3vt_sample_points_fwd(const float *verts, const int32_t *faces, const float *cdf,
                           int batch, int n_vert, int n_faces, int draws, int num,
                           const int32_t *face_idx_in, const float *u_in, const float *v_in,
                           uint64_t seed, uint64_t offset,
                           float *points, int32_t *face_idx_out, float *u_out, float *v_out, void *stream);
int a3vt_sample_points_bwd(const int32_t *faces, int batch, int n_vert, int n_faces, int draws, int num,
                           const int32_t *face_idx, const float *u, const float *v,
                           const float *grad_points, float *grad_verts, void *stream);

size_t a3vt_chamfer_scratch_bytes(int draws, int batch, int p, int q);
int a3vt_chamfer_fwd(const float *x, const float *y, int draws, int batch, int p, int q,
                     float *dist_xy, int32_t *idx_xy, float *dist_yx, int32_t *idx_yx, float *cd,
                     void *scratch, void *stream);
size_t a3vt_chamfer_workspace_bytes(int draws, int batch, int p, int q);
int a3vt_chamfer_fwd_ws(const float *x, const float *y, int draws, int batch, int p, int q,
                        float *dist_xy, int32_t *idx_xy, float *dist_yx, int32_t *idx_yx, float *cd,
                        void *workspace, size_t workspace_bytes, int algo, void *stream);
int a3vt_chamfer_fwd_shared(const float *x, const float *y, int draws, int batch, int y_batch, int p, int q,
                            float *dist_xy, int32_t *idx_xy, float *dist_yx, int32_t *idx_yx, float *cd,
                            void *workspace, size_t workspace_bytes, int algo, void *stream);
int a3vt_chamfer_bwd(const float *x, const float *y, int draws, int batch, int p, int q,
                     const int32_t *idx_xy, const int32_t *idx_yx, const float *grad_cd,
                     float *grad_x, float *grad_y, void *stream);

int a3vt_dbg_csr_algo(int algo);

int a3vt_dbg_path_counts(long long *counts, int n, int reset);

int a3vt_dbg_nn_work(int enable, unsigned long long *out8);

int a3vt_split3_bf16(const float *x, size_t n, uint16_t *hi, uint16_t *mid, uint16_t *lo, void *stream);

size_t a3vt_fold_workspace_bytes(int batch, int points, int backward);
int a3vt_fold_fwd(const float *bias_s, const float *g, int k, const float *w1g, const float *w2, const float *b2, const float *w3,
                  const float *b3, int batch, int points, int width, float *y, void *workspace, size_t workspace_bytes, void *stream);
int a3vt_fold_bwd(const float *bias_s, const float *g, int k, const float *w1g, const float *w2, const float *b2, const float *w3,
                  const float *dy, int batch, int points, int width, float *d_bias_s, float *dg, float *dw1g, float *dw2, float *db2,
                  float *dw3, float *db3, void *workspace, size_t workspace_bytes, void *stream);

int a3vt_ddqn_td(const float *q_cur, const float *q_next_online, const float *q_next_target, const float *mask, const float *actions,
                 const float *rewards, const float *denom, int batch, int num_actions, int budget, float gamma, float *loss,
                 float *diff, int32_t *best_next, float *target, void *stream);
int a3vt_ddqn_td_bwd(const float *diff, const float *actions, const float *grad_loss, int batch, int num_actions, float *dq_cur,
                     void *stream);

size_t a3vt_latent_nearest_scratch_bytes(int n_queries, int bank_rows, int k);
int a3vt_latent_nearest(const float *bank, const int32_t *bank_actions, int bank_rows, int dim, const float *queries, const float *taken,
                        int n_queries, int num_actions, int k, int32_t *idx, float *dist, int32_t *action, int32_t *rank, void *scratch,
                        void *stream);
int a3vt_latent_nn_tile(void);
int a3vt_latent_nn_query_floats(void);
int a3vt_latent_nn_cached_rows(void);

int a3vt_candidate_tally(const float *scores, const int32_t *candidates, const float *first_score, const float *taken, int K, int E, int A,
                         double unvisited, double *sums, double *checks, double *votes, int32_t *best, float *best_score, void *stream);

int a3vt_touch_render(const float *verts, int V, const int32_t *faces, int F, const int32_t *face_offset, int M, const int32_t *image_mesh,
                      const float *cam_pos, const float *cam_rot, int I, float max_depth, float yfov, float znear, float zfar, float *depth,
                      float *touch, float *points, int32_t *count, int32_t *status, void *stream);
int a3vt_touch_finish(const float *depth, const float *cam_pos, const float *cam_rot, int I, float max_depth, float yfov, float *touch,
                      float *points, int32_t *count, int32_t *status, void *stream);

int a3vt_voxel_surface(const float *verts, int V, const int32_t *faces, int F, const int32_t *vert_offset, const int32_t *face_offset, int M,
                       int dim, uint8_t *occupancy, int32_t *depth_maps, int32_t *counts, void *stream);
int a3vt_voxel_depth_maps(const uint8_t *voxels, int M, int dim, int32_t *depth_maps, void *stream);
int a3vt_voxel_points(int M, int dim, long long total, int32_t *surface, float *aligned, const long long *index, int num_points, float *cloud,
                      void *stream);
int a3vt_voxel_launches(long long *counts , int reset);

typedef struct a3vt_mlp_layer {
  const float *weight, *bias;
  int32_t in, out, relu, reserved;
} a3vt_mlp_layer;
typedef struct a3vt_mlp {
  a3vt_mlp_layer layer[16];
  int32_t n_layers, concat_at, latent_size, transform;
  float scale, offset;
} a3vt_mlp;
typedef struct a3vt_mlp_grads {
  float *dweight[16], *dbias[16];
} a3vt_mlp_grads;
int a3vt_latent_policy_limit(int which);
int a3vt_latent_policy_stash_floats(const a3vt_mlp *net);
int a3vt_latent_policy_fwd(const a3vt_mlp *net, const float *mask, const float *latent, const float *first_latent, const float *taken,
                           int rows, float *values, int32_t *action, float *stash, void *stream);
int a3vt_action_value_loss(const float *values, const int32_t *actions, const float *targets, int steps, int rows, int num_actions,
                           float *loss, float *dvalues, void *stream);
int a3vt_latent_policy_bwd(const a3vt_mlp *net, const a3vt_mlp_grads *grads, const float *mask, const float *latent,
                           const float *first_latent, const float *dvalues, const float *stash, float *delta, int rows, int accumulate,
                           void *stream);
int a3vt_latent_policy_launches(long long *counts , int reset);

size_t a3vt_ddqn_latent_scratch_bytes(const a3vt_mlp *online, int batch);
int a3vt_ddqn_latent_q(const a3vt_mlp *net, const float *mask, const float *latent, const float *first_latent, const float *mask_penalty,
                       int rows, float *q, int32_t *action, void *stream);
int a3vt_ddqn_latent_update(const a3vt_mlp *online, const a3vt_mlp *target_net, const a3vt_mlp_grads *grads, const float *mask,
                            const float *mask_n, const float *latent, const float *latent_n, const float *first_latent,
                            const float *actions, const float *rewards, const float *denom, int batch, int budget, float gamma,
                            float *q_cur, int32_t *best_next, float *target_out, float *diff, float *loss, void *scratch, void *stream);
int a3vt_ddqn_latent_launches(long long *counts , int reset);

size_t a3vt_qnet_input_scratch_bytes(int batch, int n_vert, int hidden, int cut_len, int backward);
int a3vt_qnet_input_fwd(const float *mesh, const float *w1, const float *b1, const float *w2, const float *b2, const float *comp_s,
                        const float *comp_t, const float *comp_c, const float *bias, int hidden, int cut_len, const int32_t *rowptr,
                        const int32_t *col, const float *val, int max_degree, int n_vert, int batch, float *y, int ld_y,
                        float *scratch, void *stream);
int a3vt_qnet_input_bwd(const float *mesh, const float *w1, const float *b1, const float *w2, const float *b2, const float *comp_c,
                        int hidden, int cut_len, const int32_t *rowptrT, const int32_t *colT, const float *valT, int max_degreeT,
                        int n_vert, int batch, const float *y, int ld_y, const float *grad_y, int ld_gy, float *d_s, float *d_t,
                        float *d_c, float *dw1, float *db1, float *dw2, float *db2, float *grad_bias, float *scratch, void *stream);

int a3vt_check_finite(const float *data, size_t n, int32_t *flag, void *stream);

int a3vt_profile_enable(int on);
int a3vt_profile_read(double *total_ms , int *count );
int a3vt_profile_read_classes(double *total_ms, int *count, int n);

#ifdef __cplusplus
}
#endif
#endif
```

Before: 22.04 iters/s.

## Store GCN weight images and dW slabs in MFMA fragment order

Adds a fragment-order layout (19x19 tiles of 16x16, laid out per lane) for the weight images that the rowgemmw kernel consumes. Each lane can then load its B fragment contiguously rather than through strided row-major rows. The dww backward kernel also writes its per-group dW images in fragment order, and a templated slab reducer maps them back to row-major while reducing. This aims to cut uncoalesced and strided global loads and stores in the hidden-layer GEMMs. In exchange, the image-building and reduce kernels take on index remapping, and rowgemmw is now gated on a bt_frag flag.

```diff
diff --git a/active-3d-vision-and-touch_amd/csrc/capi.hip b/active-3d-vision-and-touch_amd/csrc/capi.hip
--- a/active-3d-vision-and-touch_amd/csrc/capi.hip
+++ b/active-3d-vision-and-touch_amd/csrc/capi.hip
@@ -10,6 +10,7 @@
 
 #include "kernels.h"
 #include "prims.h"
+#include "gemm_tile.h"
 
 namespace a3vt {
 
@@ -208,8 +209,9 @@
   return launch_csr_heavy_list(rowptr, n_vert, *heavy, s);
 }
 
+template <class Frag>
 static int launch_stack_images(int kind, int transpose, const float *const *weights, int i0, int i1, int in_features,
-                               int hidden, int w0, int wh, float *dst, size_t stride, hipStream_t s) {
+                               int hidden, int w0, int wh, float *dst, size_t stride, hipStream_t s, Frag frag) {
   auto ld = [&](int w) { return kind == GEMM_BF16_STORAGE ? 2 * pad16(w / 2) : pad16(w); };
   for (; i0 < i1; i0 += kMaxImages) {
     WeightImages wi{};
@@ -225,6 +227,7 @@
       wi.k[j] = i0 + j == 0 ? in_features : hidden;
       wi.rows[j] = rowgemm_bt_rows(transpose ? hidden : w);
       wi.ld[j] = ld(transpose ? w : wh);
+      wi.frag[j] = kind == GEMM_FP32 && frag(i0 + j);
       max_rows = wi.rows[j] > max_rows ? wi.rows[j] : max_rows;
       max_ld = wi.ld[j] > max_ld ? wi.ld[j] : max_ld;
     }
@@ -234,6 +237,10 @@
     if (rc) return rc;
   }
   return 0;
+}
+static int launch_stack_images(int kind, int transpose, const float *const *weights, int i0, int i1, int in_features,
+                               int hidden, int w0, int wh, float *dst, size_t stride, hipStream_t s) {
+  return launch_stack_images(kind, transpose, weights, i0, i1, in_features, hidden, w0, wh, dst, stride, s, [](int) { return false; });
 }
 
 static int reduce_output_grads(const float *dw_slab, const float *db_slab, int k, float *grad_w, float *grad_b, int acc,
@@ -297,7 +304,7 @@
   if (need_backward) {
     const size_t kin = kmax;
     L.panel = a.take(pad4(in_features) > 304 ? m * 300 : 0);
-    L.dw_slab = a.take((size_t)dw_slab_capacity(hidden) * kin * hidden);
+    L.dw_slab = a.take(dw_slab_floats((int)kin, hidden));
     const size_t nslab = (size_t)csr_bwd_num_slabs(batch, n_vert) > (size_t)batch ? csr_bwd_num_slabs(batch, n_vert) : batch;
     L.db_layer_stride = align_up(nslab * cpad, 64);
     L.db_slab = a.take(L.db_layer_stride * (num_layers > 1 ? num_layers - 1 : 1));
@@ -326,8 +333,7 @@
       ProfScope ps(PROF_DW, s, timed);
       if (int rc = launch_dw(d, s)) return rc;
     }
-    const size_t n = (size_t)w * d.n_out;
-    if (int rc = launch_slab_reduce_za(d.slab, dw_images(d), n, n, n, grad + (size_t)c0 * d.n_out, acc, s)) return rc;
+    if (int rc = launch_dw_reduce(d, grad + (size_t)c0 * d.n_out, acc, s)) return rc;
   }
   return 0;
 }
@@ -804,30 +810,24 @@
   const StackPlan P = stack_plan(gemm_bf16, batch, n_vert, hidden, num_layers, cut_len, max_degree, split, -1);
   const int qcols = P.qcols, rm_ld = P.rm_ld;
   const size_t rm_off = P.rm_off;
-  if (P.x3)
-    if (int rc = launch_stack_images(GEMM_FP32X3, 1, weights, 1, num_layers - 1, in_features, hidden, ld_feats, hidden,
-                                     scratch + L.wt, L.wt_stride, s))
-      return rc;
-  if (int rc = launch_stack_images(GEMM_FP32, 1, weights, 0, P.x3 ? 1 : num_layers - 1, in_features, hidden, ld_feats, hidden,
-                                   scratch + L.wt, L.wt_stride, s))
-    return rc;
-  if (num_layers > 1) path_count(P.quad ? PATH_STACK_QUAD : PATH_STACK_ROWS);
-  if (P.qsplit) path_count(PATH_STACK_SPLIT);
-  if (num_layers > 1) stash_layout_record(masks, P.quad);
-  int32_t *ell = reinterpret_cast<int32_t *>(scratch + L.ell);
-  if (int rc = launch_stack_ell(P, split, rowptr, col, val, n_vert, ell, s)) return rc;
-  const float *x = feats, *xq = nullptr;
-  int ldx = ld_feats;
-  for (int i = 0; i + 1 < num_layers; ++i) {
+  auto out_of = [&](int i) -> float * { return acts ? acts + S.act(i) : scratch + L.ping[i & 1]; };
+  struct In { const float *x, *xq; int ldx; };
+  auto in_of = [&](int i) -> In {
+    if (i == 0) return {feats, nullptr, ld_feats};
+    const float *yp = out_of(i - 1);
+    return {yp + rm_off - qcols, P.quad ? yp : nullptr, rm_ld};
+  };
+  auto product = [&](int i) {
     const int k = i == 0 ? ld_feats : hidden;
     const bool l3 = P.x3 && i > 0;
-    float *y = acts ? acts + S.act(i) : scratch + L.ping[i & 1];
+    const In in = in_of(i);
+    float *y = out_of(i);
     RowGemmArgs g{};
-    g.a0 = g.a1 = x;
-    g.lda0 = g.lda1 = ldx;
+    g.a0 = g.a1 = in.x;
+    g.lda0 = g.lda1 = in.ldx;
     g.ksplit = k;
-    if (xq) {
-      g.a0 = xq;
+    if (in.xq) {
+      g.a0 = in.xq;
       g.ksplit = qcols;
       g.a0q_nvert = n_vert;
       g.a0q_quads = qcols / 4;
@@ -843,8 +843,7 @@
     g.c2 = scratch + L.za;
     g.ldc2 = cpad;
     g.csplit = cut_len;
-    uint8_t *mk = masks ? masks + S.signs(i) : nullptr;
-    g.maskb = mk;
+    g.maskb = masks ? masks + S.signs(i) : nullptr;
     g.mld = S.mld;
     g.moff = cpad / 4;
     g.mode = l3 ? GEMM_FP32X3 : P.omode;
@@ -855,6 +854,25 @@
       g.yq_quads = qcols / 4;
       g.trash = scratch + L.z3;
     }
+    g.bt_frag = rowgemmw_shape_ok(g, EPI_FWD_HIDDEN);
+    return g;
+  };
+  if (P.x3)
+    if (int rc = launch_stack_images(GEMM_FP32X3, 1, weights, 1, num_layers - 1, in_features, hidden, ld_feats, hidden,
+                                     scratch + L.wt, L.wt_stride, s))
+      return rc;
+  if (int rc = launch_stack_images(GEMM_FP32, 1, weights, 0, P.x3 ? 1 : num_layers - 1, in_features, hidden, ld_feats, hidden,
+                                   scratch + L.wt, L.wt_stride, s, [&](int i) { return product(i).bt_frag != 0; }))
+    return rc;
+  if (num_layers > 1) path_count(P.quad ? PATH_STACK_QUAD : PATH_STACK_ROWS);
+  if (P.qsplit) path_count(PATH_STACK_SPLIT);
+  if (num_layers > 1) stash_layout_record(masks, P.quad);
+  int32_t *ell = reinterpret_cast<int32_t *>(scratch + L.ell);
+  if (int rc = launch_stack_ell(P, split, rowptr, col, val, n_vert, ell, s)) return rc;
+  for (int i = 0; i + 1 < num_layers; ++i) {
+    float *y = out_of(i);
+    const RowGemmArgs g = product(i);
+    uint8_t *mk = g.maskb;
     {
       ProfScope ps(PROF_GEMM_FWD, s);
       if (int rc = launch_rowgemm(g, EPI_FWD_HIDDEN, s)) return rc;
@@ -867,20 +885,18 @@
       } else if (int rc = launch_csrq_fwd(scratch + L.za, biases[i], cut_len, rowptr, col, val, heavy, ell, n_vert, batch, y, qcols / 4, sq, 1, s)) {
         return rc;
       }
-      xq = y;
     } else if (cut_len > 0) {
       ProfScope psa(PROF_AGG, s);
       if (int rc = launch_csr_fwd(scratch + L.za, L.ldza, biases[i], cut_len, rowptr, col, val, heavy, n_vert, batch, y, hidden, mk, S.mld, 1, s))
         return rc;
     }
-    x = y + rm_off - qcols;
-    ldx = rm_ld;
   }
   const int klast = num_layers == 1 ? in_features : hidden;
+  const In in = in_of(num_layers - 1);
   ProfScope pso(PROF_OUT, s);
   const SplitRef sref = split_ref(split);
-  return launch_thin_fwd(x, ldx, klast, weights[num_layers - 1], biases[num_layers - 1], rowptr, col, val, heavy, n_vert,
-                         batch, scratch + L.z3, update, xq, qcols / 4, s, split ? &sref : nullptr);
+  return launch_thin_fwd(in.x, in.ldx, klast, weights[num_layers - 1], biases[num_layers - 1], rowptr, col, val, heavy, n_vert,
+                         batch, scratch + L.z3, update, in.xq, qcols / 4, s, split ? &sref : nullptr);
 }
 
 int a3vt_gcn_stack_bwd(const float *feats, int ld_feats, int in_features, const float *const *weights,
@@ -964,18 +980,56 @@
       return rc;
   }
 
+  auto cur_of = [&](int i) { return (last - 1 - i) & 1; };
+  auto dx_product = [&](int i) {
+    RowGemmArgs r{};
+    r.a0 = scratch + L.za;
+    r.lda0 = L.ldza;
+    if (quad) {
+      r.a0q_nvert = n_vert;
+      r.a0q_quads = cpad / 4;
+    }
+    r.a1 = scratch + L.ping[cur_of(i)];
+    r.lda1 = hidden;
+    r.ksplit = cpad;
+    r.bt = scratch + L.wt + L.wt_stride * i;
+    r.ldb = pad16(hidden);
+    r.zeros = zeros;
+    r.m = (int)m;
+    r.k = hidden;
+    r.n_store = i == 0 ? ld_feats : hidden;
+    r.mode = P.x3 && i > 0 ? GEMM_FP32X3 : P.omode;
+    if (i == 0) {
+      r.c = grad_feats;
+      r.ldc = ld_feats;
+    } else {
+      r.c = scratch + L.ping[cur_of(i) ^ 1];
+      r.ldc = hidden;
+      r.maskb = const_cast<uint8_t *>(masks) + S.signs(i - 1);
+      r.mld = S.mld;
+      r.moff = cpad / 4;
+      r.csplit = cut_len;
+      if (quad) {
+        r.c2 = scratch + L.gq;
+        r.zq_nvert = n_vert;
+        r.zq_quads = cpad / 4;
+        r.trash = scratch + L.z3;
+      }
+      r.bt_frag = rowgemmw_shape_ok(r, EPI_DX_MASK);
+    }
+    return r;
+  };
   if (P.x3)
     if (int rc = launch_stack_images(GEMM_FP32X3, 0, weights, 1, last, in_features, hidden, ld_feats, hidden, scratch + L.wt,
                                      L.wt_stride, s))
       return rc;
   if (int rc = launch_stack_images(GEMM_FP32, 0, weights, 0, P.x3 ? 1 : last, in_features, hidden, ld_feats, hidden,
-                                   scratch + L.wt, L.wt_stride, s))
+                                   scratch + L.wt, L.wt_stride, s, [&](int i) { return dx_product(i).bt_frag != 0; }))
     return rc;
 
   const int db_rows = quad ? batch : csr_bwd_num_slabs(batch, n_vert);
-  int cur = 0;
   for (int i = last - 1; i >= 0; --i) {
-    float *g = scratch + L.ping[cur];
+    float *g = scratch + L.ping[cur_of(i)];
     float *dza = scratch + L.za;
     const float *xl = i == 0 ? feats : acts + S.act(i - 1);
     const bool xhyb = quad && i > 0;
@@ -1034,45 +1088,12 @@
     }
     if (int rc = dw_panels(d, x, ldxw, kin, scratch + L.panel, grad_weights[i], acc, true, s)) return rc;
 
-    RowGemmArgs r{};
-    r.a0 = dza;
-    r.lda0 = L.ldza;
-    if (quad) {
-      r.a0q_nvert = n_vert;
-      r.a0q_quads = cpad / 4;
-    }
-    r.a1 = g;
-    r.lda1 = hidden;
-    r.ksplit = cpad;
-    r.bt = scratch + L.wt + L.wt_stride * i;
-    r.ldb = pad16(hidden);
-    r.zeros = zeros;
-    r.m = (int)m;
-    r.k = hidden;
-    r.n_store = i == 0 ? ld_feats : hidden;
-    r.mode = P.x3 && i > 0 ? GEMM_FP32X3 : P.omode;
+    const RowGemmArgs r = dx_product(i);
     if (i == 0) {
-      r.c = grad_feats;
-      r.ldc = ld_feats;
       if (int rc = launch_rowgemm(r, EPI_PLAIN, s)) return rc;
     } else {
-      r.c = scratch + L.ping[cur ^ 1];
-      r.ldc = hidden;
-      r.maskb = const_cast<uint8_t *>(masks) + S.signs(i - 1);
-      r.mld = S.mld;
-      r.moff = cpad / 4;
-      r.csplit = cut_len;
-      if (quad) {
-        r.c2 = scratch + L.gq;
-        r.zq_nvert = n_vert;
-        r.zq_quads = cpad / 4;
-        r.trash = scratch + L.z3;
-      }
-      {
-        ProfScope ps(PROF_GEMM_DX, s);
-        if (int rc = launch_rowgemm(r, EPI_DX_MASK, s)) return rc;
-      }
-      cur ^= 1;
+      ProfScope ps(PROF_GEMM_DX, s);
+      if (int rc = launch_rowgemm(r, EPI_DX_MASK, s)) return rc;
     }
   }
   if (cut_len > 0)
@@ -2139,6 +2160,11 @@
   return PATH_COUNT;
 }
 
+int a3vt_dbg_fragment_offset(int tile, int chunk, int lane, int elem) {
+  A3VT_CHECK_ARG(tile >= 0 && tile < kFragTiles && chunk >= 0 && chunk < kFragChunks && lane >= 0 && lane < 64 && elem >= 0 && elem < 4);
+  return frag_offset(tile, chunk, lane, elem);
+}
+
 int a3vt_dbg_csr_algo(int algo) {
   A3VT_CHECK_ARG(algo >= 0 && algo <= 2);
   g_csr_algo = algo;
diff --git a/active-3d-vision-and-touch_amd/csrc/gcn_dww.hip b/active-3d-vision-and-touch_amd/csrc/gcn_dww.hip
--- a/active-3d-vision-and-touch_amd/csrc/gcn_dww.hip
+++ b/active-3d-vision-and-touch_amd/csrc/gcn_dww.hip
@@ -195,15 +195,11 @@
     st = (st + 1) & 3;
   }
   asm volatile("s_nop 15\n\ts_nop 3" ::: "memory");
-  float *img = p.slab + (size_t)image * kDK * kDN;
+  float *img = p.slab + (size_t)image * kFragFloats;
 #pragma unroll
   for (int t = 0; t < NKT; ++t) {
-    const int k = (kt0 + t) * 16 + l16;
-#pragma unroll
-    for (int n = 0; n < NNT; ++n) {
-      const int col = (NT0 + n) * 16 + q * 4;
-      if (k < kDK && col < kDN) *reinterpret_cast<f32x4 *>(img + (size_t)k * kDN + col) = acc[t][n];
-    }
+#pragma unroll
+    for (int n = 0; n < NNT; ++n) *reinterpret_cast<f32x4 *>(img + frag_offset(kt0 + t, NT0 + n, lane, 0)) = acc[t][n];
   }
 }
 
@@ -216,10 +212,11 @@
   const int tiles = p.m / kDStageRows;
   const int t0 = (int)((long long)group * tiles / ngroups), t1 = (int)((long long)(group + 1) * tiles / ngroups);
   if (half == 1 && group < kDwwGroupsA - kDwwGroupsB) {
-    float *img = p.slab + (size_t)(kDwwGroupsB + group) * kDK * kDN;
-    for (int i = threadIdx.x; i < kDK * 35; i += 256) {
-      const int k = i / 35, c = i - k * 35;
-      *reinterpret_cast<f32x4 *>(img + (size_t)k * kDN + 160 + c * 4) = f32x4{0.f, 0.f, 0.f, 0.f};
+    float *img = p.slab + (size_t)(kDwwGroupsB + group) * kFragFloats;
+    constexpr int kHalfB = (kFragTiles - 10) * 64;
+    for (int i = threadIdx.x; i < kFragTiles * kHalfB; i += 256) {
+      const int tk = i / kHalfB, r = i - tk * kHalfB;
+      *reinterpret_cast<f32x4 *>(img + frag_offset(tk, 10, 0, 0) + r * 4) = f32x4{0.f, 0.f, 0.f, 0.f};
     }
   }
   if (half == 0) {
@@ -244,6 +241,8 @@
 }
 
 int dww_images() { return kDwwGroupsA; }
+size_t dww_image_floats() { return kFragFloats; }
+size_t dww_slab_floats(int k_max, int n_out) { return k_max >= kDK && n_out == kDN ? (size_t)kDwwGroupsA * kFragFloats : 0; }
 
 int launch_dww(const DwArgs &a, hipStream_t s) {
   if (!dww_ok(a)) {
diff --git a/active-3d-vision-and-touch_amd/csrc/gcn_gemm.hip b/active-3d-vision-and-touch_amd/csrc/gcn_gemm.hip
--- a/active-3d-vision-and-touch_amd/csrc/gcn_gemm.hip
+++ b/active-3d-vision-and-touch_amd/csrc/gcn_gemm.hip
@@ -577,6 +577,10 @@
     set_error("rowgemm: k=%d ksplit=%d ldb=%d violate alignment rules", a.k, a.ksplit, a.ldb);
     return -1;
   }
+  if (a.bt_frag && !rowgemmw_ok(a, epi)) {
+    set_error("rowgemm: fragment-order weight image on a shape rowgemmw does not take (m=%d k=%d n=%d epi=%d)", a.m, a.k, a.n_store, epi);
+    return -1;
+  }
   if (rowgemmw_ok(a, epi)) return launch_rowgemmw(a, epi, s);
   if (rowgemm16_ok(a, epi)) return launch_rowgemm16(a, epi, s);
   switch (epi) {
@@ -615,6 +619,9 @@
   const float *src = w.w[l];
   float *dst = w.dst + (size_t)l * w.dst_stride;
   const int k = w.k[l], n = w.n, rows = w.rows[l], ld = w.ld[l];
+  const bool frag = w.frag[l] != 0;
+  auto at = [&](int r, int c) { return frag ? (size_t)frag_offset(r >> 4, c >> 4, ((c >> 2) & 3) * 16 + (r & 15), c & 3) : (size_t)r * ld + c; };
+  const int rows_w = frag ? min(rows, 16 * kFragTiles) : rows, ld_w = frag ? min(ld, 16 * kFragChunks) : ld;
   if (w.transpose) {
     __shared__ float tile[32][33];
     const int bx = blockIdx.x * 32, by = blockIdx.y * 32;
@@ -625,8 +632,18 @@
     }
     __syncthreads();
     for (int i = threadIdx.y; i < 32; i += 8) {
-      const int nn = by + i, kk = bx + threadIdx.x;
-      if (nn < rows && kk < ld) dst[(size_t)nn * ld + kk] = tile[threadIdx.x][i];
+      const int j = i * 32 + threadIdx.x;
+      const int tn = frag ? (j >> 2) & 31 : i, tk = frag ? (j >> 7) * 4 + (j & 3) : threadIdx.x;
+      const int nn = by + tn, kk = bx + tk;
+      if (nn < rows_w && kk < ld_w) dst[at(nn, kk)] = tile[tk][tn];
+    }
+  } else if (frag) {
+    const int tid = threadIdx.y * 32 + threadIdx.x;
+    const int nblk = gridDim.x * gridDim.y, blk = blockIdx.y * gridDim.x + blockIdx.x;
+    for (int idx = blk * 256 + tid; idx < kFragFloats; idx += nblk * 256) {
+      int r, c;
+      frag_row_col(idx, r, c);
+      dst[idx] = (r < k && c < n) ? src[(size_t)r * n + c] : 0.f;
     }
   } else {
     const int tid = threadIdx.y * 32 + threadIdx.x;
@@ -1001,8 +1018,12 @@
   return 256 / g > 0 ? 256 / g : 1;
 }
 
-int dw_images(const DwArgs &a) { return a.mode != GEMM_FP32X3 && dww_ok(a) ? dww_images() : dw_num_slabs(a.n_out); }
-int dw_slab_capacity(int n_out) { return dw_num_slabs(n_out) > dww_images() ? dw_num_slabs(n_out) : dww_images(); }
+static bool dw_takes_dww(const DwArgs &a) { return a.mode != GEMM_FP32X3 && dww_ok(a); }
+int dw_images(const DwArgs &a) { return dw_takes_dww(a) ? dww_images() : dw_num_slabs(a.n_out); }
+size_t dw_slab_floats(int k_max, int n_out) {
+  const size_t rows = (size_t)dw_num_slabs(n_out) * k_max * n_out, frag = dww_slab_floats(k_max, n_out);
+  return rows > frag ? rows : frag;
+}
 
 constexpr int kDwStageUnits = 48;
 bool dw_rows_fit(int ldx, int ldz0, int ldz1) {
@@ -1092,8 +1113,10 @@
   return 0;
 }
 
+template <bool FRAG>
 __global__ __launch_bounds__(1024) void slab_reduce_kernel(const float *__restrict__ slab, int nslab, size_t stride,
-                                                           size_t n, size_t n_out, float *__restrict__ out, int accumulate) {
+                                                           size_t n, size_t n_out, float *__restrict__ out, int accumulate,
+                                                           int rows, int cols) {
   __shared__ float part[16][64];
   const int lane = threadIdx.x & 63, grp = threadIdx.x >> 6;
   const size_t i = (size_t)blockIdx.x * 64 + lane;
@@ -1115,7 +1138,14 @@
 #pragma unroll
     for (int g = 0; g < 16; ++g) t += part[g][lane];
     t = i < n ? t : 0.f;
-    out[i] = accumulate ? out[i] + t : t;
+    size_t o = i;
+    if (FRAG) {
+      int k, c;
+      frag_row_col((int)i, k, c);
+      if (k >= rows || c >= cols) return;
+      o = (size_t)k * cols + c;
+    }
+    out[o] = accumulate ? out[o] + t : t;
   }
 }
 
@@ -1212,11 +1242,20 @@
     A3VT_LAUNCH(slab_reduce_tall_kernel, dim3(cdiv((long long)n_out, 16)), dim3(1024), 0, s, slab, nslab, stride, n, n_out, out,
                 accumulate);
   else
-    A3VT_LAUNCH(slab_reduce_kernel, dim3(cdiv((long long)n_out, 64)), dim3(1024), 0, s, slab, nslab, stride, n, n_out, out,
-                accumulate);
+    A3VT_LAUNCH(slab_reduce_kernel<false>, dim3(cdiv((long long)n_out, 64)), dim3(1024), 0, s, slab, nslab, stride, n, n_out, out,
+                accumulate, 0, 0);
   A3VT_CHECK_LAUNCH();
   return 0;
 }
+int launch_dw_reduce(const DwArgs &a, float *out, int accumulate, hipStream_t s) {
+  const size_t n = (size_t)a.k_in * a.n_out;
+  if (!dw_takes_dww(a)) return launch_slab_reduce_za(a.slab, dw_images(a), n, n, n, out, accumulate, s);
+  const size_t nf = dww_image_floats();
+  A3VT_LAUNCH(slab_reduce_kernel<true>, dim3(cdiv((long long)nf, 64)), dim3(1024), 0, s, a.slab, dww_images(), nf, nf, nf, out, accumulate,
+              a.k_in, a.n_out);
+  A3VT_CHECK_LAUNCH();
+  return 0;
+}
 int launch_slab_reduce(const float *slab, int nslab, size_t stride, size_t n, float *out, hipStream_t s) {
   return launch_slab_reduce_za(slab, nslab, stride, n, n, out, 0, s);
 }
diff --git a/active-3d-vision-and-touch_amd/csrc/gcn_gemmw.hip b/active-3d-vision-and-touch_amd/csrc/gcn_gemmw.hip
--- a/active-3d-vision-and-touch_amd/csrc/gcn_gemmw.hip
+++ b/active-3d-vision-and-touch_amd/csrc/gcn_gemmw.hip
@@ -41,10 +41,10 @@
   float bv[kWChunks][4][NV], ba[kWChunks][4][NT - NV];
 #pragma unroll
   for (int t = 0; t < NT; ++t) {
-    const float *br = p.bt + (size_t)((wave + 3 * t) * 16 + l16) * p.ldb + q * 4;
+    const float *br = p.bt + frag_offset(wave + 3 * t, 0, lane, 0);
 #pragma unroll
     for (int c = 0; c < kWChunks; ++c) {
-      const f32x4 v = *reinterpret_cast<const f32x4 *>(br + c * 16);
+      const f32x4 v = *reinterpret_cast<const f32x4 *>(br + frag_offset(0, c, 0, 0));
 #pragma unroll
       for (int sidx = 0; sidx < 4; ++sidx) {
         if (t < NV) bv[c][sidx][t] = v[sidx];
@@ -99,10 +99,10 @@
   float bv[kWChunks][4][NV], ba[kWChunks][4][NT - NV];
 #pragma unroll
   for (int t = 0; t < NT; ++t) {
-    const float *br = p.bt + (size_t)((T0 + t) * 16 + l16) * p.ldb + q * 4;
+    const float *br = p.bt + frag_offset(T0 + t, 0, lane, 0);
 #pragma unroll
     for (int c = 0; c < kWChunks; ++c) {
-      const f32x4 v = *reinterpret_cast<const f32x4 *>(br + c * 16);
+      const f32x4 v = *reinterpret_cast<const f32x4 *>(br + frag_offset(0, c, 0, 0));
 #pragma unroll
       for (int sidx = 0; sidx < 4; ++sidx) {
         if (t < NV) bv[c][sidx][t] = v[sidx];
@@ -334,11 +334,13 @@
     const int ntl = (p.n_store + 15) >> 4;
     const int units = ((p.rem_rows + 15) >> 4) * ntl;
     for (int u = wave * gridDim.x + blockIdx.x; u < units; u += 4 * gridDim.x)
-      rowtile_unit<EPI, 0>(p, p.rem_row0, p.rem_row0 + p.rem_rows, u / ntl, (u % ntl) * 16, lane);
-  }
-}
-
-bool rowgemmw_ok(const RowGemmArgs &a, int epi) {
+      rowtile_unit<EPI, 0, true>(p, p.rem_row0, p.rem_row0 + p.rem_rows, u / ntl, (u % ntl) * 16, lane);
+  }
+}
+
+static_assert(kWChunks == kFragTiles && kWChunks == kFragChunks, "the fragment-order image is this kernel's 19 x 19 tiles");
+
+bool rowgemmw_shape_ok(const RowGemmArgs &a, int epi) {
   if (a.mode != GEMM_FP32 || (epi != EPI_FWD_HIDDEN && epi != EPI_DX_MASK)) return false;
   if (a.zq_nvert <= 0 || a.a0q_nvert != a.zq_nvert || a.c2 == nullptr || a.m % a.zq_nvert != 0 || a.m % 16 != 0) return false;
   if (a.k <= 288 || a.k > 304 || a.n_store <= 288 || a.n_store > 304 || a.n_store % 4 != 0 || a.k % 4 != 0) return false;
@@ -352,6 +354,8 @@
   if (epi == EPI_DX_MASK && a.ksplit != 100) return false;
   return (a.m >> 4) >= 768;
 }
+
+bool rowgemmw_ok(const RowGemmArgs &a, int epi) { return a.bt_frag != 0 && rowgemmw_shape_ok(a, epi); }
 
 template <int EPI>
 static int launch_rowgemmw_epi(const RowGemmArgs &a0, hipStream_t s) {
@@ -375,7 +379,7 @@
 
 int launch_rowgemmw(const RowGemmArgs &a, int epi, hipStream_t s) {
   if (!rowgemmw_ok(a, epi)) {
-    set_error("rowgemmw: shape not taken (m=%d k=%d n=%d epi=%d)", a.m, a.k, a.n_store, epi);
+    set_error("rowgemmw: shape not taken or no fragment-order image (m=%d k=%d n=%d epi=%d bt_frag=%d)", a.m, a.k, a.n_store, epi, a.bt_frag);
     return -1;
   }
   return epi == EPI_FWD_HIDDEN ? launch_rowgemmw_epi<EPI_FWD_HIDDEN>(a, s) : launch_rowgemmw_epi<EPI_DX_MASK>(a, s);
diff --git a/active-3d-vision-and-touch_amd/csrc/gemm_tile.h b/active-3d-vision-and-touch_amd/csrc/gemm_tile.h
--- a/active-3d-vision-and-touch_amd/csrc/gemm_tile.h
+++ b/active-3d-vision-and-touch_amd/csrc/gemm_tile.h
@@ -4,7 +4,15 @@
 
 namespace a3vt {
 
-template <int EPI, int MODE>
+constexpr int kFragTiles = 19, kFragChunks = 19, kFragFloats = kFragTiles * kFragChunks * 256;
+__host__ __device__ constexpr int frag_offset(int T, int c, int lane, int e) { return ((T * kFragChunks + c) * 64 + lane) * 4 + e; }
+__host__ __device__ inline void frag_row_col(int off, int &row, int &col) {
+  const int tile = off >> 8, lane = (off >> 2) & 63;
+  row = (tile / kFragChunks) * 16 + (lane & 15);
+  col = (tile % kFragChunks) * 16 + (lane >> 4) * 4 + (off & 3);
+}
+
+template <int EPI, int MODE, bool BFRAG = false>
 __device__ __forceinline__ void rowtile_unit(const RowGemmArgs &p, int row_base, int row_end, int mt, int n0, int lane) {
   constexpr int KB = 19;
   const int l16 = lane & 15, q = lane >> 4;
@@ -28,7 +36,8 @@
       const int kk = (c0 + c) * 16 + q * 4;
       const bool on = c0 + c < nch && kk < p.k;
       af[c] = on ? *reinterpret_cast<const f32x4 *>(kk < p.ksplit ? a0r + (size_t)kk * a0mul : a1r + kk) : f32x4{0.f, 0.f, 0.f, 0.f};
-      bf[c] = on ? *reinterpret_cast<const f32x4 *>(btr + kk) : f32x4{0.f, 0.f, 0.f, 0.f};
+      const float *bsrc = BFRAG ? p.bt + frag_offset(n0 >> 4, c0 + c, lane, 0) : btr + kk;
+      bf[c] = on ? *reinterpret_cast<const f32x4 *>(bsrc) : f32x4{0.f, 0.f, 0.f, 0.f};
     }
 #pragma unroll
     for (int c = 0; c < KB; ++c) {
diff --git a/active-3d-vision-and-touch_amd/csrc/kernels.h b/active-3d-vision-and-touch_amd/csrc/kernels.h
--- a/active-3d-vision-and-touch_amd/csrc/kernels.h
+++ b/active-3d-vision-and-touch_amd/csrc/kernels.h
@@ -30,9 +30,11 @@
   int yq_quads;
   int a0q_nvert, a0q_quads;
   float *trash;
+  int bt_frag;
 };
 int rowgemm_bt_rows(int n_store);
 int launch_rowgemm(const RowGemmArgs &a, int epi, hipStream_t s);
+bool rowgemmw_shape_ok(const RowGemmArgs &a, int epi);
 bool rowgemmw_ok(const RowGemmArgs &a, int epi);
 int launch_rowgemmw(const RowGemmArgs &a, int epi, hipStream_t s);
 bool rowgemm16_ok(const RowGemmArgs &a, int epi);
@@ -46,6 +48,7 @@
   size_t dst_stride;
   int k[kMaxImages], rows[kMaxImages], ld[kMaxImages];
   int n, count, transpose;
+  unsigned char frag[kMaxImages];
 };
 int launch_weight_images(const WeightImages &w, int max_rows, int max_ld, hipStream_t s);
 
@@ -82,7 +85,8 @@
 };
 int dw_num_slabs(int n_out);
 int dw_images(const DwArgs &a);
-int dw_slab_capacity(int n_out);
+size_t dw_slab_floats(int k_max, int n_out);
+int launch_dw_reduce(const DwArgs &a, float *out, int accumulate, hipStream_t s);
 bool dw3_ok(const DwArgs &a);
 int launch_dw3(const DwArgs &a, hipStream_t s);
 bool dw_quad_major_ok(int k_in, int quads);
@@ -90,6 +94,8 @@
 int launch_dw(const DwArgs &a, hipStream_t s);
 bool dww_ok(const DwArgs &a);
 int dww_images();
+size_t dww_image_floats();
+size_t dww_slab_floats(int k_max, int n_out);
 int launch_dww(const DwArgs &a, hipStream_t s);
 int launch_copy_cols(const float *src, int ld_src, int c0, int w, float *dst, long long m, hipStream_t s);
 int launch_slab_reduce(const float *slab, int nslab, size_t stride, size_t n, float *out, hipStream_t s);
diff --git a/include/a3vt.h b/include/a3vt.h
--- a/include/a3vt.h
+++ b/include/a3vt.h
@@ -198,6 +198,8 @@
 int a3vt_dbg_csr_algo(int algo);
 
 int a3vt_dbg_path_counts(long long *counts, int n, int reset);
+
+int a3vt_dbg_fragment_offset(int tile, int chunk, int lane, int elem);
 
 int a3vt_dbg_nn_work(int enable, unsigned long long *out8);
 
```

Result: no change. 22.10 iters/s, median of 6 (+0.3%).
